# UBC-AWP/vision-sam3-yolo-lameless

Hardware: AMD Instinct MI355X
Metric: frames/sec (whole node) for YOLO+SAM3+DINOv3 feature extraction, 1080p clips (higher is better)
Workload: dtype f16; 1 GPU; BASELINE cfg#5, dense schedule: fused per-frame path on a synthetic 5 s @ 30 fps 1080p clip (150 unique BGR frames resident in HBM): YOLOv8-l detect (letterbox 384x640, NMS, scale_boxes; f16 plan) -> SAM (Hiera-B+ image encoder + FPN at 1024x1024, box-prompted mask decoder, 1080p mask + statistics + contour features) + DINOv3 ViT-L/16 embed (224x224) on EVERY frame; per-frame records packed, gathe; parallelism=one clip per GPU, 1 GPU(s), one gather per step, streams=7

## Files before the change

include/lmx.h:

```cpp
#ifndef LMX_H
#define LMX_H
#include <stdint.h>
#ifdef __cplusplus
extern "C" {
#endif

#define LMX_VERSION 100

#define LMX_OK 0
#define LMX_EINVAL (-1)
#define LMX_EHIP (-2)

typedef void* lmx_stream_t;

int lmx_version(void);
const char* lmx_last_error(void);
int lmx_device_count(void);

enum { LMX_F16 = 0, LMX_F32 = 1 };
enum { LMX_ACT_NONE = 0, LMX_ACT_SILU = 1, LMX_ACT_GELU = 2 , LMX_ACT_RELU = 3 };

typedef struct {
  const void* A;
  const void* W;
  const float* bias;
  const float* scale;
  const void* res;
  void* C;
  int64_t lda, ldc, ldr;
  int32_t M, N, K;
  int32_t act;
  int32_t out_dtype;
  int32_t a_mode;
  int32_t H, W_, Cin, conv_stride, Ho, Wo;
  int32_t res_rows;
  int32_t a_rep;
  int32_t split_k;
  int64_t split_stride;
} lmx_gemm_desc;
int lmx_k_gemm(const lmx_gemm_desc* d, lmx_stream_t stream);
void lmx_dbg_set_gemm2_variant(int v);

int lmx_k_layernorm(const void* x, int in_dtype, int64_t ldx, const float* gamma, const float* beta,
                    void* y, int out_dtype, int64_t ldy, int rows, int D, float eps, int act, lmx_stream_t stream);

int lmx_k_hiera_attn8(const void* h, float* x, int64_t ldx, const float* gamma, const float* beta, float eps, const void* wqkv_p,
                      const float* bqkv_p, const void* wo_p, const float* bo, int n_img, int Gh, int Gw, int D, int heads, float scale,
                      lmx_stream_t stream);

int lmx_k_hiera_attn4(const void* h, float* x, int64_t ldx, const void* w_img, const float* bias, int n_img, int Gh, int Gw, int D,
                      int heads, float scale, lmx_stream_t stream);

int lmx_k_hiera_attn_pool(const void* h, float* out, const void* w_img, const float* bias, int n_img, int Gh, int Gw, int Din, int Dout,
                          int heads, float scale, lmx_stream_t stream);

int lmx_k_ln_mlp(float* x, int64_t ldx, const float* gamma, const float* beta, const void* w1, const float* b1,
                 const void* w2, const float* b2, int64_t rows, int D, float eps, void* workspace, void* x16,
                 const float* gamma_next, const float* beta_next, void* h_next, lmx_stream_t stream);
int lmx_k_ln_mlp_img(float* x, int64_t ldx, const void* w_img, const float* bias, int64_t rows, int D, float eps, void* x16, void* h_next,
                     lmx_stream_t stream);

typedef struct {
  const void* Q; const void* K; const void* V; void* O;
  int64_t ldq, ldk, ldv, ldo;
  int32_t B, H, Tq, Tk, hd;
  float scale;
  int32_t mode;
  int32_t Gh, Gw, ws, q_stride;
  const void* pad_k; const void* pad_v;
  const void* rel; int32_t rel_S;
} lmx_attn_desc;
int lmx_k_attention(const lmx_attn_desc* d, lmx_stream_t stream);
int lmx_k_relpos_tables(const lmx_attn_desc* d, const float* rel_pos_h, const float* rel_pos_w, int S, void* out,
                        lmx_stream_t stream);

int lmx_k_rope(void* x, int64_t ld, int B, int T, int H, int hd, int n_prefix, const float* cos_t,
               const float* sin_t, lmx_stream_t stream);

int lmx_k_pil_resize_h(const uint8_t* src, uint8_t* dst, int n, int sh, int sw, int dw, const int32_t* bounds,
                       const int32_t* kk, int ksize, int swap_rb, lmx_stream_t stream);
int lmx_k_pil_resize_v(const uint8_t* src, uint8_t* dst, int n, int sh, int dh, int w, const int32_t* bounds,
                       const int32_t* kk, int ksize, lmx_stream_t stream);

int lmx_k_patchify_norm(const uint8_t* img, void* out, int n, int ih, int iw, int top, int left, int gh, int gw,
                        int P, int64_t ldo, const float* lut, lmx_stream_t stream);

int lmx_k_assemble_tokens(const void* patch_f16, const float* prefix, const float* pos, float* out, int B, int np,
                          int n_prefix, int D, lmx_stream_t stream);

int lmx_k_token_mean(const void* x, int in_dtype, float* out, int B, int T, int D, lmx_stream_t stream);

int64_t lmx_nms_workspace_bytes(int n, int A);
int lmx_k_nms(const float* pred, int n, int A, int nc, float conf, double iou, int max_det, float max_wh,
              float* boxes, float* scores, int32_t* cls, int32_t* src, int32_t* counts, void* workspace,
              lmx_stream_t stream);

int lmx_k_letterbox(const uint8_t* src, uint8_t* dst, int n, int sh, int sw, int rh, int rw, int top, int left,
                    int oh, int ow, const int32_t* xofs, const int16_t* ialpha, const int32_t* yofs,
                    const int16_t* ibeta, int swap_rb, lmx_stream_t stream);
int lmx_k_stem_conv(const uint8_t* img, const float* w, const float* bias, void* out, int n, int H, int W, int Cout,
                    lmx_stream_t stream);
int lmx_k_maxpool5(const void* src, int64_t lds, void* dst, int64_t ldd, int n, int H, int W, int C,
                   lmx_stream_t stream);
int lmx_k_upsample2(const void* src, int64_t lds, void* dst, int64_t ldd, int n, int H, int W, int C,
                    lmx_stream_t stream);
int lmx_k_detect_decode(const float* head, int64_t ldh, float* pred, int n, int H, int W, int nc, float stride,
                        int a_off, int A, lmx_stream_t stream);
int lmx_k_scale_boxes(float* boxes, int total, float padx, float pady, float gain, float w, float h,
                      lmx_stream_t stream);

int lmx_k_split3(const float* x, int64_t ldx, int act, const void* res3, int64_t ldr, void* out3, int64_t ldo, int64_t rows,
                 int N, int g, int nsum, int64_t sum_stride, lmx_stream_t stream);
int lmx_k_maxpool5_x3(const void* src3, int64_t lds, void* dst3, int64_t ldd, int n, int H, int W, int C, lmx_stream_t stream);
int lmx_k_stem_conv_x3(const uint8_t* img, const float* w, const float* bias, void* out3, int n, int H, int W, int Cout,
                       lmx_stream_t stream);
int lmx_k_attention_f32(const float* q, int64_t ldq, const float* k, int64_t ldk, const float* v, int64_t ldv, float* o,
                        int64_t ldo, int B, int H, int Tq, int Tk, int hd, float scale, lmx_stream_t stream);
int lmx_k_hyper_mask_f32(const float* up, const float* hyper, float* logits, int n, int G, int C, int act, lmx_stream_t stream);

int lmx_k_pose_gather(const float* raw0, const float* raw1, const float* raw2, int64_t ldk, const int32_t* hw,
                      const float* strides, const int32_t* src, const int32_t* counts, int n, int max_det, int K, int ndim,
                      float padx, float pady, float gain, float w, float h, float* out, lmx_stream_t stream);

int lmx_k_im2col_u8(const uint8_t* img, const float* lut, void* out, int n, int rh, int rw, int IH, int IW, int KH,
                    int KW, int stride, int pad, int64_t ldo, lmx_stream_t stream);
int lmx_k_maxpool2(const void* src, int64_t lds, void* dst, int64_t ldd, int dtype, int n, int H, int W, int C,
                   lmx_stream_t stream);
int lmx_k_cast_f32_f16(const float* src, int64_t lds, void* dst, int64_t ldd, int64_t rows, int cols,
                       lmx_stream_t stream);

int lmx_k_add_bcast(const void* a, int a_dtype, int64_t lda, const float* b, int64_t ldb, int b_rows, void* out,
                    int out_dtype, int64_t ldo, int64_t rows, int D, lmx_stream_t stream);
int lmx_k_prompt_box(const float* boxes, int64_t ldb, float* sparse, int n, double sx, double sy, float S,
                     const float* gauss, const float* corner, int F, lmx_stream_t stream);
int lmx_k_hyper_mask(const void* up, const float* hyper, float* logits, int n, int G, int C, lmx_stream_t stream);
int lmx_k_mask_post(const float* logits, int n, int L, int T, int nh, int nw, int h, int w, uint8_t* mask,
                    int64_t* stats, float* workspace, lmx_stream_t stream);
int lmx_k_prompt_points(const float* points, const int32_t* labels, int Np, const float* boxes, int64_t ldb, float* sparse, int n,
                        double sx, double sy, float S, const float* gauss, const float* point_embed, const float* not_a_point,
                        const float* corner, int F, lmx_stream_t stream);
#define LMX_MASK_EMBED_PARAMS 4684
int lmx_k_mask_embed(const float* mask_input, const void* emb, int emb_dtype, int64_t lde, const float* params, float* keys,
                     int64_t ldk, int n, int G, lmx_stream_t stream);
int lmx_k_hyper_mask_multi(const void* up, const float* hyper, float* logits, int n, int M, int G, int C, lmx_stream_t stream);
int lmx_k_hyper_mask_multi_f32(const float* up, const float* hyper, float* logits, int n, int M, int G, int C, int act,
                               lmx_stream_t stream);
int lmx_k_mask_logits(const float* logits, int n, int L, int T, int nh, int nw, int h, int w, float* out, lmx_stream_t stream);
int lmx_k_pack_bits(const uint8_t* src, int64_t rows, int w, uint8_t* dst, lmx_stream_t stream);

int64_t lmx_contour_workspace_bytes(int n, int h, int w);
int lmx_k_contour_features(const uint8_t* mask, int n, int h, int w, int64_t* out, void* workspace, lmx_stream_t stream);

int lmx_h_mask_features(const uint8_t* mask_host, int h, int w, double* out_host);

int lmx_h_iou_matrix(const double* a, int n, const double* b, int m, double* out);
int lmx_h_assign(const double* cost, int n, int m, int* row_to_col, int* col_to_row);

#ifdef __cplusplus
}
#endif
#endif
```

vision-sam3-yolo-lameless_amd/csrc/common.h:

```cpp
#pragma once
#include <hip/hip_runtime.h>
#include <stdint.h>
#include <stdio.h>
#include <stdarg.h>
#include "../../include/lmx.h"

typedef _Float16 half_t;
typedef _Float16 half2_t __attribute__((ext_vector_type(2)));
typedef _Float16 half4_t __attribute__((ext_vector_type(4)));
typedef _Float16 half8_t __attribute__((ext_vector_type(8)));
typedef float f32x4 __attribute__((ext_vector_type(4)));
typedef float f32x16 __attribute__((ext_vector_type(16)));
typedef unsigned int u32x4 __attribute__((ext_vector_type(4)));
typedef unsigned int u32x2 __attribute__((ext_vector_type(2)));

void lmx_set_error(const char* fmt, ...);

#define LMX_REQUIRE(cond, ...)            \
  do {                                    \
    if (!(cond)) {                        \
      lmx_set_error(__VA_ARGS__);         \
      return LMX_EINVAL;                  \
    }                                     \
  } while (0)

#define LMX_HIP(call)                                                                   \
  do {                                                                                  \
    hipError_t e_ = (call);                                                             \
    if (e_ != hipSuccess) {                                                             \
      lmx_set_error("%s failed: %s (%s:%d)", #call, hipGetErrorString(e_), __FILE__, __LINE__); \
      return LMX_EHIP;                                                                  \
    }                                                                                   \
  } while (0)

static inline int lmx_launch_check(const char* what) {
  hipError_t e = hipGetLastError();
  if (e != hipSuccess) {
    lmx_set_error("launch of %s failed: %s", what, hipGetErrorString(e));
    return LMX_EHIP;
  }
  return LMX_OK;
}

typedef float f32x2 __attribute__((ext_vector_type(2)));

__device__ __forceinline__ f32x2 gelu_pk(f32x2 v) {
  f32x2 vc;
  vc[0] = __builtin_amdgcn_fmed3f(v[0], -4.5f, 4.5f);
  vc[1] = __builtin_amdgcn_fmed3f(v[1], -4.5f, 4.5f);
  const f32x2 u = vc * vc;
  f32x2 p = {-1.223331157e-12f, -1.223331157e-12f};
  p = p * u + 1.524351007e-10f;
  p = p * u + -8.481037793e-09f;
  p = p * u + 2.798429583e-07f;
  p = p * u + -6.151207192e-06f;
  p = p * u + 9.615961466e-05f;
  p = p * u + -1.114801972e-03f;
  p = p * u + 9.814679350e-03f;
  p = p * u + -6.632144717e-02f;
  p = p * u + 3.988863025e-01f;
  const f32x2 g = vc * p;
  return v * g + 0.5f * v;
}
__device__ __forceinline__ float gelu_1(float v) {
  const f32x2 r = gelu_pk(f32x2{v, v});
  return r[0];
}

__device__ __forceinline__ float lmx_act(float v, int act) {
  if (act == LMX_ACT_SILU) return v * __builtin_amdgcn_rcpf(1.0f + __builtin_amdgcn_exp2f(-v * 1.44269504088896340736f));
  if (act == LMX_ACT_GELU) return gelu_1(v);
  if (act == LMX_ACT_RELU) return fmaxf(v, 0.0f);
  return v;
}

typedef __attribute__((address_space(3))) void* lds_ptr_t;

__device__ __forceinline__ void lds_dma16(__amdgpu_buffer_rsrc_t rs, char* dst_lds, unsigned voffset, int soffset) {
  __builtin_amdgcn_raw_ptr_buffer_load_lds(rs, (lds_ptr_t)dst_lds, 16, voffset, soffset, 0, 0);
}

#define LMX_WAIT_CASE(n) \
  if constexpr (N == n) asm volatile("s_waitcnt vmcnt(" #n ")" ::: "memory")
template <int N>
__device__ __forceinline__ void wait_vmcnt() {
  static_assert(N == 0 || N == 1 || N == 2 || N == 3 || N == 4 || N == 6 || N == 8 || N == 9 || N == 12 || N == 16 || N == 18 || N == 24 ||
                    N == 32,
                "add the literal for this count");
  LMX_WAIT_CASE(0);
  LMX_WAIT_CASE(1);
  LMX_WAIT_CASE(2);
  LMX_WAIT_CASE(3);
  LMX_WAIT_CASE(4);
  LMX_WAIT_CASE(6);
  LMX_WAIT_CASE(8);
  LMX_WAIT_CASE(9);
  LMX_WAIT_CASE(12);
  LMX_WAIT_CASE(16);
  LMX_WAIT_CASE(18);
  LMX_WAIT_CASE(24);
  LMX_WAIT_CASE(32);
}
#undef LMX_WAIT_CASE
template <int PT>
__device__ __forceinline__ void wait_tiles(int y) {
  if (y >= 4)
    wait_vmcnt<4 * PT>();
  else if (y == 3)
    wait_vmcnt<3 * PT>();
  else if (y == 2)
    wait_vmcnt<2 * PT>();
  else if (y == 1)
    wait_vmcnt<PT>();
  else
    wait_vmcnt<0>();
}

static inline bool aligned16(const void* p) { return (((uintptr_t)p) & 15) == 0; }

__device__ __forceinline__ float wave_sum(float v) {
#pragma unroll
  for (int o = 32; o > 0; o >>= 1) v += __shfl_xor(v, o, 64);
  return v;
}
__device__ __forceinline__ float wave_max(float v) {
#pragma unroll
  for (int o = 32; o > 0; o >>= 1) v = fmaxf(v, __shfl_xor(v, o, 64));
  return v;
}

__device__ __forceinline__ float act_exact(float v, int act) {
  if (act == LMX_ACT_SILU) return v / (1.0f + expf(-v));
  if (act == LMX_ACT_RELU) return fmaxf(v, 0.0f);
  if (act == LMX_ACT_GELU) return 0.5f * v * (1.0f + erff(v * 0.70710678118654752440f));
  return v;
}

__device__ __forceinline__ void bil_idx(float scale, int dst, int in_size, int& i0, int& i1, float& l1) {
  float src = scale * ((float)dst + 0.5f) - 0.5f;
  src = src < 0.f ? 0.f : src;
  i0 = (int)src;
  i1 = i0 + (i0 < in_size - 1 ? 1 : 0);
  l1 = src - (float)i0;
}

__device__ __forceinline__ float sample_mid(const float* __restrict__ lg, int L, int T, float sLT, int Y, int X) {
  int y0, y1, x0, x1;
  float ly, lx;
  bil_idx(sLT, Y, L, y0, y1, ly);
  bil_idx(sLT, X, L, x0, x1, lx);
  const float t0 = (1.f - lx) * lg[y0 * L + x0] + lx * lg[y0 * L + x1];
  const float t1 = (1.f - lx) * lg[y1 * L + x0] + lx * lg[y1 * L + x1];
  return (1.f - ly) * t0 + ly * t1;
}
```

vision-sam3-yolo-lameless_amd/csrc/gemm.hip:

```cpp
#include "common.h"
#include <stdlib.h>

namespace {

constexpr int BK = 64;

template <int BM, int BN, int AMODE, int OUT_DT>
__global__ __launch_bounds__(256, 2) void gemm_kernel(const lmx_gemm_desc p) {
  extern __shared__ __attribute__((aligned(16))) char smem[];
  half_t* As = reinterpret_cast<half_t*>(smem);
  half_t* Ws = As + 2 * BM * BK;
  constexpr int FM = BM / 32;
  constexpr int FN = BN / 32;
  constexpr int AI = BM / 32;
  constexpr int WI = BN / 32;

  const int tid = threadIdx.x;
  const int lane = tid & 63;
  const int wave = tid >> 6;
  const int wm = wave & 1, wn = wave >> 1;

  const int nwg = gridDim.x;
  const int bid = blockIdx.x;
  const int q = nwg >> 3, r = nwg & 7, xcd = bid & 7;
  const int swz = (xcd < r ? xcd * (q + 1) : r * (q + 1) + (xcd - r) * q) + (bid >> 3);
  const int NT = (p.N + BN - 1) / BN;
  const int mt = swz / NT, nt = swz - mt * NT;
  const int m0 = mt * BM, n0 = nt * BN;

  const int c = tid & 7;
  const int r0 = tid >> 3;

  const half_t* A = reinterpret_cast<const half_t*>(p.A);
  const half_t* W = reinterpret_cast<const half_t*>(p.W);

  int64_t a_off[AI];
  int a_iy[AI], a_ix[AI];
  bool a_ok[AI];
#pragma unroll
  for (int i = 0; i < AI; ++i) {
    const int m = m0 + r0 + 32 * i;
    a_ok[i] = m < p.M;
    if (AMODE == 0) {
      a_off[i] = (int64_t)m * p.lda;
      a_iy[i] = a_ix[i] = 0;
    } else {
      const int hw = p.Ho * p.Wo;
      const int img = m / hw;
      const int rem = m - img * hw;
      const int oy = rem / p.Wo;
      const int ox = rem - oy * p.Wo;
      a_off[i] = (int64_t)img * p.H * p.W_ * p.lda;
      a_iy[i] = oy * p.conv_stride - 1;
      a_ix[i] = ox * p.conv_stride - 1;
    }
  }
  int64_t w_off[WI];
  bool w_ok[WI];
#pragma unroll
  for (int i = 0; i < WI; ++i) {
    const int n = n0 + r0 + 32 * i;
    w_ok[i] = n < p.N;
    w_off[i] = (int64_t)n * p.K;
  }

  half8_t a_st[AI], w_st[WI];
  const half8_t zero8 = {0, 0, 0, 0, 0, 0, 0, 0};

  auto load_tile = [&](int kt) {
    const int k = kt * BK + c * 8;
    const bool k_ok = k < p.K;
    if (AMODE == 0) {
#pragma unroll
      for (int i = 0; i < AI; ++i)
        a_st[i] = (a_ok[i] && k_ok) ? *reinterpret_cast<const half8_t*>(A + a_off[i] + k) : zero8;
    } else {
      const int tap = k / p.Cin;
      const int ci = k - tap * p.Cin;
      const int ky = tap / 3;
      const int kx = tap - 3 * ky;
#pragma unroll
      for (int i = 0; i < AI; ++i) {
        const int iy = a_iy[i] + ky, ix = a_ix[i] + kx;
        const bool ok = a_ok[i] && k_ok && (unsigned)iy < (unsigned)p.H && (unsigned)ix < (unsigned)p.W_;
        a_st[i] = ok ? *reinterpret_cast<const half8_t*>(A + a_off[i] + ((int64_t)iy * p.W_ + ix) * p.lda + ci)
                     : zero8;
      }
    }
#pragma unroll
    for (int i = 0; i < WI; ++i)
      w_st[i] = (w_ok[i] && k_ok) ? *reinterpret_cast<const half8_t*>(W + w_off[i] + k) : zero8;
  };
  auto store_tile = [&](int buf) {
    half_t* as = As + buf * BM * BK;
    half_t* ws = Ws + buf * BN * BK;
#pragma unroll
    for (int i = 0; i < AI; ++i) {
      const int row = r0 + 32 * i;
      *reinterpret_cast<half8_t*>(as + row * BK + ((c ^ (row & 7)) << 3)) = a_st[i];
    }
#pragma unroll
    for (int i = 0; i < WI; ++i) {
      const int row = r0 + 32 * i;
      *reinterpret_cast<half8_t*>(ws + row * BK + ((c ^ (row & 7)) << 3)) = w_st[i];
    }
  };

  f32x4 acc[FM][FN];
#pragma unroll
  for (int i = 0; i < FM; ++i)
#pragma unroll
    for (int j = 0; j < FN; ++j) acc[i][j] = f32x4{0.f, 0.f, 0.f, 0.f};

  const int nk = (p.K + BK - 1) / BK;
  load_tile(0);
  store_tile(0);
  __syncthreads();

  const int frow = lane & 15;
  const int fq = lane >> 4;
  for (int kt = 0; kt < nk; ++kt) {
    const int buf = kt & 1;
    if (kt + 1 < nk) load_tile(kt + 1);
    const half_t* as = As + buf * BM * BK + (wm * (BM / 2) + frow) * BK;
    const half_t* ws = Ws + buf * BN * BK + (wn * (BN / 2) + frow) * BK;
#pragma unroll
    for (int ks = 0; ks < 2; ++ks) {
      const int coff = (((ks << 2) + fq) ^ (frow & 7)) << 3;
      half8_t af[FM], wf[FN];
#pragma unroll
      for (int i = 0; i < FM; ++i) af[i] = *reinterpret_cast<const half8_t*>(as + i * 16 * BK + coff);
#pragma unroll
      for (int j = 0; j < FN; ++j) wf[j] = *reinterpret_cast<const half8_t*>(ws + j * 16 * BK + coff);
#pragma unroll
      for (int i = 0; i < FM; ++i)
#pragma unroll
        for (int j = 0; j < FN; ++j)
          acc[i][j] = __builtin_amdgcn_mfma_f32_16x16x32_f16(wf[j], af[i], acc[i][j], 0, 0, 0);
    }
    if (kt + 1 < nk) store_tile(buf ^ 1);
    __syncthreads();
  }

#pragma unroll
  for (int i = 0; i < FM; ++i) {
    const int m = m0 + wm * (BM / 2) + i * 16 + frow;
    if (m >= p.M) continue;
    const int mr = p.res_rows > 0 ? m % p.res_rows : m;
#pragma unroll
    for (int j = 0; j < FN; ++j) {
      const int n = n0 + wn * (BN / 2) + j * 16 + fq * 4;
      if (n >= p.N) continue;
      f32x4 v = acc[i][j];
      if (p.bias) {
        const f32x4 b = *reinterpret_cast<const f32x4*>(p.bias + n);
        v += b;
      }
      if (p.act != LMX_ACT_NONE) {
#pragma unroll
        for (int e = 0; e < 4; ++e) v[e] = lmx_act(v[e], p.act);
      }
      if (p.scale) {
        const f32x4 s = *reinterpret_cast<const f32x4*>(p.scale + n);
#pragma unroll
        for (int e = 0; e < 4; ++e) v[e] = __fmul_rn(v[e], s[e]);
      }
      if (OUT_DT == LMX_F32) {
        float* C = reinterpret_cast<float*>(p.C);
        if (p.res) {
          const f32x4 rr = *reinterpret_cast<const f32x4*>(reinterpret_cast<const float*>(p.res) + (int64_t)mr * p.ldr + n);
#pragma unroll
          for (int e = 0; e < 4; ++e) v[e] = __fadd_rn(v[e], rr[e]);
        }
        *reinterpret_cast<f32x4*>(C + (int64_t)m * p.ldc + n) = v;
      } else {
        half_t* C = reinterpret_cast<half_t*>(p.C);
        if (p.res) {
          const half4_t rr =
              *reinterpret_cast<const half4_t*>(reinterpret_cast<const half_t*>(p.res) + (int64_t)mr * p.ldr + n);
#pragma unroll
          for (int e = 0; e < 4; ++e) v[e] = __fadd_rn((float)(half_t)v[e], (float)rr[e]);
        }
        half4_t o;
#pragma unroll
        for (int e = 0; e < 4; ++e) o[e] = (half_t)v[e];
        *reinterpret_cast<half4_t*>(C + (int64_t)m * p.ldc + n) = o;
      }
    }
  }
}

template <int BM, int BN, int AMODE, int OUT_DT>
int launch(const lmx_gemm_desc& d, hipStream_t st) {
  const int MT = (d.M + BM - 1) / BM, NT = (d.N + BN - 1) / BN;
  const size_t smem = (size_t)2 * (BM + BN) * BK * sizeof(half_t);
  static bool attr_set = false;
  if (!attr_set) {
    LMX_HIP(hipFuncSetAttribute(reinterpret_cast<const void*>(&gemm_kernel<BM, BN, AMODE, OUT_DT>),
                                hipFuncAttributeMaxDynamicSharedMemorySize, (int)smem));
    attr_set = true;
  }
  hipLaunchKernelGGL((gemm_kernel<BM, BN, AMODE, OUT_DT>), dim3(MT * NT), dim3(256), smem, st, d);
  return lmx_launch_check("gemm_kernel");
}

template <int AMODE, int OUT_DT>
int dispatch_tile(const lmx_gemm_desc& d, hipStream_t st) {
  if (d.N <= 64 || (d.N < 128 && d.N % 128 != 0)) return launch<128, 64, AMODE, OUT_DT>(d, st);
  return launch<128, 128, AMODE, OUT_DT>(d, st);
}

}

int lmx_gemm2_launch(const lmx_gemm_desc& d, hipStream_t st);

static bool force_v1() {
  static int v = -1;
  if (v < 0) {
    const char* e = getenv("LMX_GEMM_V1");
    v = (e && e[0] == '1') ? 1 : 0;
  }
  return v == 1;
}

extern "C" int lmx_k_gemm(const lmx_gemm_desc* dp, lmx_stream_t stream) {
  LMX_REQUIRE(dp != nullptr, "lmx_k_gemm: null descriptor");
  const lmx_gemm_desc& d = *dp;
  LMX_REQUIRE(d.A && d.W && d.C, "lmx_k_gemm: null A/W/C");
  LMX_REQUIRE(d.M > 0 && d.N > 0 && d.K > 0, "lmx_k_gemm: empty problem M=%d N=%d K=%d", d.M, d.N, d.K);
  LMX_REQUIRE(d.K % 8 == 0, "lmx_k_gemm: K=%d must be a multiple of 8", d.K);
  LMX_REQUIRE(d.N % 4 == 0, "lmx_k_gemm: N=%d must be a multiple of 4", d.N);
  LMX_REQUIRE(d.lda % 8 == 0, "lmx_k_gemm: lda=%lld must be a multiple of 8", (long long)d.lda);
  LMX_REQUIRE(d.ldc % 4 == 0 && d.ldc >= d.N, "lmx_k_gemm: bad ldc=%lld", (long long)d.ldc);
  LMX_REQUIRE(aligned16(d.A) && aligned16(d.W), "lmx_k_gemm: A/W must be 16-byte aligned");
  LMX_REQUIRE((((uintptr_t)d.C) & 7) == 0, "lmx_k_gemm: C must be 8-byte aligned");
  LMX_REQUIRE(d.out_dtype == LMX_F16 || d.out_dtype == LMX_F32, "lmx_k_gemm: bad out_dtype %d", d.out_dtype);
  LMX_REQUIRE(d.out_dtype == LMX_F16 || aligned16(d.C), "lmx_k_gemm: f32 C must be 16-byte aligned");
  LMX_REQUIRE(d.act >= LMX_ACT_NONE && d.act <= LMX_ACT_RELU, "lmx_k_gemm: bad act %d", d.act);
  if (d.bias) LMX_REQUIRE(aligned16(d.bias), "lmx_k_gemm: bias must be 16-byte aligned");
  if (d.scale) LMX_REQUIRE(aligned16(d.scale), "lmx_k_gemm: scale must be 16-byte aligned");
  if (d.res) LMX_REQUIRE(d.ldr % 4 == 0 && d.ldr >= d.N, "lmx_k_gemm: bad ldr=%lld", (long long)d.ldr);
  LMX_REQUIRE(d.res_rows >= 0, "lmx_k_gemm: res_rows");
  if (d.a_mode == 0) {
    LMX_REQUIRE(d.a_rep > 1 || d.lda >= d.K, "lmx_k_gemm: lda=%lld < K=%d", (long long)d.lda, d.K);
  } else if (d.a_mode == 1) {
    LMX_REQUIRE(d.Cin > 0 && d.Cin % 8 == 0, "lmx_k_gemm: conv Cin=%d must be a multiple of 8", d.Cin);
    LMX_REQUIRE(d.K == 9 * d.Cin, "lmx_k_gemm: conv K=%d != 9*Cin=%d", d.K, 9 * d.Cin);
    LMX_REQUIRE(d.conv_stride == 1 || d.conv_stride == 2, "lmx_k_gemm: conv stride %d", d.conv_stride);
    LMX_REQUIRE(d.H > 0 && d.W_ > 0, "lmx_k_gemm: conv H/W");
    LMX_REQUIRE(d.Ho == (d.H + 2 - 3) / d.conv_stride + 1 && d.Wo == (d.W_ + 2 - 3) / d.conv_stride + 1,
                "lmx_k_gemm: conv Ho/Wo (%d,%d) inconsistent with H/W (%d,%d) stride %d", d.Ho, d.Wo, d.H, d.W_,
                d.conv_stride);
    LMX_REQUIRE(d.M % (d.Ho * d.Wo) == 0, "lmx_k_gemm: conv M=%d not a multiple of Ho*Wo", d.M);
    LMX_REQUIRE(d.lda >= d.Cin, "lmx_k_gemm: conv pixel stride lda=%lld < Cin=%d", (long long)d.lda, d.Cin);
  } else if (d.a_mode == 2) {
    LMX_REQUIRE(d.lda >= d.K, "lmx_k_gemm: lda=%lld < K=%d", (long long)d.lda, d.K);
    LMX_REQUIRE(d.H > 0 && d.W_ > 0 && d.H % 2 == 0 && d.W_ % 2 == 0 && d.M % (d.H * d.W_) == 0,
                "lmx_k_gemm: pooled rows need an even H x W token grid that divides M (H=%d W=%d M=%d)", d.H, d.W_, d.M);
    LMX_REQUIRE(!d.res && !d.scale && d.act == LMX_ACT_NONE, "lmx_k_gemm: pooled rows: no residual / scale / activation");
    LMX_REQUIRE(((int64_t)d.M * d.lda + d.K) * 2 < 0x7fffffffll, "lmx_k_gemm: pooled rows: A must be smaller than 2 GB");
    LMX_REQUIRE(d.M >= 512 && d.N >= 96 && d.N % 8 == 0 && d.ldc % 8 == 0 && aligned16(d.C),
                "lmx_k_gemm: pooled rows are built for the LDS-DMA kernel (M >= 512, N >= 96, N %% 8 == 0): use GEMM + maxpool2 for M=%d N=%d", d.M, d.N);
  } else {
    LMX_REQUIRE(false, "lmx_k_gemm: bad a_mode %d", d.a_mode);
  }
  LMX_REQUIRE(d.a_rep >= 0 && d.a_rep <= 3, "lmx_k_gemm: a_rep=%d (0..3)", d.a_rep);
  LMX_REQUIRE(d.split_k >= 0 && d.split_k <= 64, "lmx_k_gemm: split_k=%d (0..64)", d.split_k);
  if (d.split_k > 1) {
    LMX_REQUIRE(d.out_dtype == LMX_F32 && d.act == LMX_ACT_NONE && d.a_mode != 2 && d.a_rep <= 1, "lmx_k_gemm: split_k needs f32 output, no activation, a_mode 0 or 1");
    LMX_REQUIRE(d.split_stride >= (int64_t)(d.M - 1) * d.ldc + d.N && d.split_stride % 4 == 0, "lmx_k_gemm: split_stride=%lld", (long long)d.split_stride);
    LMX_REQUIRE((d.K + 63) / 64 >= d.split_k, "lmx_k_gemm: split_k=%d exceeds the k-tiles of K=%d", d.split_k, d.K);
    const bool conv_ok2 = d.a_mode == 1 && d.Cin % 32 == 0 && d.H < 32768 && d.W_ < 32768;
    LMX_REQUIRE((d.a_mode == 0 || conv_ok2) && d.N >= 64 && d.N % 8 == 0 && d.ldc % 8 == 0 && (!d.res || d.ldr % 8 == 0) &&
                    aligned16(d.C) && (!d.res || aligned16(d.res)),
                "lmx_k_gemm: split_k is built into the LDS-DMA kernel only (N >= 64, N %% 8 == 0; conv: Cin %% 32 == 0); M=%d N=%d", d.M, d.N);
    return lmx_gemm2_launch(d, reinterpret_cast<hipStream_t>(stream));
  }
  if (d.a_rep > 1) {
    LMX_REQUIRE(d.a_mode == 0 && d.K % d.a_rep == 0 && (d.K / d.a_rep) % 64 == 0, "lmx_k_gemm: a_rep=%d needs a_mode 0 and K / a_rep a multiple of 64 (K=%d)", d.a_rep, d.K);
    LMX_REQUIRE(d.lda >= d.K / d.a_rep, "lmx_k_gemm: lda=%lld < K / a_rep", (long long)d.lda);
    LMX_REQUIRE(d.M >= 512 && d.N >= 96 && d.N % 8 == 0 && d.ldc % 8 == 0 && (!d.res || d.ldr % 8 == 0) && aligned16(d.C) && (!d.res || aligned16(d.res)),
                "lmx_k_gemm: a_rep is built into the LDS-DMA kernel only (M >= 512, N >= 96, N %% 8 == 0); M=%d N=%d", d.M, d.N);
    return lmx_gemm2_launch(d, reinterpret_cast<hipStream_t>(stream));
  }
  hipStream_t st = reinterpret_cast<hipStream_t>(stream);
  const bool conv_ok = d.a_mode == 1 && d.Cin % 32 == 0 && d.H < 32768 && d.W_ < 32768;
  if (d.a_mode == 2) return lmx_gemm2_launch(d, st);
  static int n64 = -1;
  if (n64 < 0) n64 = (getenv("LMX_GEMM_N64") && getenv("LMX_GEMM_N64")[0] == '0') ? 0 : 1;
  const int n_min = (conv_ok && n64 && d.M >= 65536) ? 64 : 96;
  if ((d.a_mode == 0 || conv_ok) && d.M >= 512 && d.N >= n_min && d.N % 8 == 0 && d.ldc % 8 == 0 && (!d.res || d.ldr % 8 == 0) &&
      aligned16(d.C) && (!d.res || aligned16(d.res)) && !force_v1())
    return lmx_gemm2_launch(d, st);
  if (d.a_mode == 0) {
    return d.out_dtype == LMX_F16 ? dispatch_tile<0, LMX_F16>(d, st) : dispatch_tile<0, LMX_F32>(d, st);
  }
  return d.out_dtype == LMX_F16 ? dispatch_tile<1, LMX_F16>(d, st) : dispatch_tile<1, LMX_F32>(d, st);
}
```

vision-sam3-yolo-lameless_amd/csrc/gemm2.hip:

```cpp
#include "common.h"
#include <stdlib.h>
#include <type_traits>

#ifdef LMX_DBG_TIMELINE
__device__ unsigned long long lmx_tl[8 * 16384];
extern "C" int lmx_dbg_get_timeline(void* host, int64_t bytes) { return (int)hipMemcpyFromSymbol(host, HIP_SYMBOL(lmx_tl), bytes); }
#define TL(i, v) if (threadIdx.x == 0 && swz < 16384) lmx_tl[swz * 8 + (i)] = (v)
#else
#define TL(i, v)
#endif
namespace lmx_gemm2 {

__device__ __forceinline__ float act_apply(float v, int act) { return lmx_act(v, act); }

constexpr int smem_bytes(int BM, int BN, int BK, int NSTAGE) { return NSTAGE * (BM + BN) * BK * 2 + 2 * BN * 4; }
constexpr int waves_per_simd(int BM, int BN, int BK, int NSTAGE) {
  const int smem = smem_bytes(BM, BN, BK, NSTAGE), nwave = (BM / 64) * (BN / 64);
  const int wps = (smem <= 80 * 1024 ? 2 : 1) * nwave / 4;
  return wps < 1 ? 1 : wps;
}
template <int OUT_DT, int BM, int BN, int BK, int NSTAGE, int AMODE, int STAG>
__global__ __launch_bounds__(waves_per_simd(BM, BN, BK, NSTAGE) * 256) void gemm2_kernel(const lmx_gemm_desc p, const int ntiles, const int nt_ok) {
  constexpr int NWAVE = (BM / 64) * (BN / 64);
  constexpr int STAGE_BYTES = (BM + BN) * BK * 2;
  constexpr int A_INSTR = BM * BK * 2 / 1024 / NWAVE;
  constexpr int W_INSTR = BN * BK * 2 / 1024 / NWAVE;
  constexpr int ROWS_PER_INSTR = 1024 / (BK * 2);
  constexpr int CHUNKS = BK / 8;
  constexpr int LA = NSTAGE - 1;
  extern __shared__ __attribute__((aligned(16))) char smem[];
  const int tid = threadIdx.x;
  const int lane = tid & 63;
  const int wave = __builtin_amdgcn_readfirstlane(tid >> 6);
  const int wm = wave % (BM / 64), wn = wave / (BM / 64);

  const int bid = blockIdx.x, xcd = bid & 7;
  const int q = ntiles >> 3, r = ntiles & 7;
  const int base = xcd < r ? xcd * (q + 1) : r * (q + 1) + (xcd - r) * q;
  const int cnt = q + (xcd < r ? 1 : 0);
  const int stride = ((int)gridDim.x + 7 - xcd) >> 3;
  const int NT = (p.N + BN - 1) / BN;
  for (int li = bid >> 3; li < cnt; li += stride) {
  const int swz = base + li;
  const int S_ = p.split_k > 1 ? p.split_k : 1;
  const int tile_ = swz / S_, sp_ = swz - tile_ * S_;
  const int mt = tile_ / NT, nt = tile_ - mt * NT;
  const int m0 = mt * BM, n0 = nt * BN;
  TL(0, (unsigned long long)__builtin_amdgcn_s_getreg((31 << 11) | 4));
  TL(1, (unsigned long long)__builtin_amdgcn_s_getreg((31 << 11) | 20));
  TL(2, wall_clock64());
  TL(5, (unsigned long long)bid);

  const int hw_out = (AMODE == 1) ? p.Ho * p.Wo : 1;
  const int img0 = (AMODE == 1) ? m0 / hw_out : 0;
  const char* Ab = reinterpret_cast<const char*>(p.A) +
                   ((AMODE == 1) ? (int64_t)img0 * p.H * p.W_ * p.lda * 2 : (AMODE == 2 ? (int64_t)0 : (int64_t)m0 * p.lda * 2));
  const char* Wb = reinterpret_cast<const char*>(p.W) + (int64_t)n0 * p.K * 2;
  const int Ka = (AMODE == 0 && p.a_rep > 1) ? p.K / p.a_rep : p.K;
  int64_t a_bytes = (AMODE == 1) ? ((int64_t)(p.M / hw_out - img0) * p.H * p.W_ - 1) * p.lda * 2 + (int64_t)p.Cin * 2
                                 : ((int64_t)(p.M - (AMODE == 2 ? 0 : m0) - 1) * p.lda + Ka) * 2;
  int64_t w_bytes = (int64_t)(p.N - n0) * p.K * 2;
  if (a_bytes > 0x7FFFFFF0ll) a_bytes = 0x7FFFFFF0ll;
  if (w_bytes > 0x7FFFFFF0ll) w_bytes = 0x7FFFFFF0ll;
  const __amdgpu_buffer_rsrc_t a_rs = __builtin_amdgcn_make_buffer_rsrc(const_cast<char*>(Ab), 0, (int)a_bytes, 0x00020000);
  const __amdgpu_buffer_rsrc_t w_rs = __builtin_amdgcn_make_buffer_rsrc(const_cast<char*>(Wb), 0, (int)w_bytes, 0x00020000);

  const int lrow = lane / CHUNKS;
  const int lsw = (BK == 64) ? (lrow & 7) : ((-(lrow >> 2)) & 3);
  const int lchunk = (lane % CHUNKS) ^ lsw;
  unsigned a_off[A_INSTR], w_off[W_INSTR];
  int a_yx[A_INSTR];
#pragma unroll
  for (int j = 0; j < A_INSTR; ++j) {
    const int row = (wave * A_INSTR + j) * ROWS_PER_INSTR + lrow;
    if (AMODE == 0) {
      a_off[j] = (unsigned)(row * (int)p.lda * 2 + lchunk * 16);
      a_yx[j] = 0;
    } else if (AMODE == 2) {
      const int m = m0 + row, g = m >> 2, sub = m & 3;
      const int Wq = p.W_ >> 1, gpi = (p.H >> 1) * Wq;
      const int img = g / gpi, rem = g - img * gpi;
      const int gy = rem / Wq, gx = rem - gy * Wq;
      const int tok = (img * p.H + 2 * gy + (sub >> 1)) * p.W_ + 2 * gx + (sub & 1);
      a_off[j] = m < p.M ? (unsigned)(tok * (int)p.lda * 2 + lchunk * 16) : 0x80000000u;
      a_yx[j] = 0;
    } else {
      const int m = m0 + row;
      const int img = m / hw_out, rem = m - img * hw_out;
      const int oy = rem / p.Wo, ox = rem - oy * p.Wo;
      const int iy0 = oy * p.conv_stride - 1, ix0 = ox * p.conv_stride - 1;
      a_off[j] = (unsigned)((((img - img0) * p.H + iy0) * p.W_ + ix0) * (int)p.lda * 2 + lchunk * 16);
      a_yx[j] = (m < p.M) ? ((iy0 << 16) | (ix0 & 0xffff)) : 0x80008000;
    }
  }
#pragma unroll
  for (int j = 0; j < W_INSTR; ++j)
    w_off[j] = (unsigned)(((wave * W_INSTR + j) * ROWS_PER_INSTR + lrow) * p.K * 2 + lchunk * 16);
  const unsigned OOB = 0x80000000u;
  const int nk = (p.K + BK - 1) / BK;
  const int nk64 = (p.K + 63) / 64;
  const int kt0 = (int)((int64_t)sp_ * nk64 / S_) * (64 / BK);
  const int kte = sp_ + 1 == S_ ? nk : (int)((int64_t)(sp_ + 1) * nk64 / S_) * (64 / BK);
  const int nloc = kte - kt0;
  const int nkA = (AMODE == 0 && p.a_rep > 1) ? nk / p.a_rep : nk;
  const bool k_tail_lane = (nk - 1) * BK + lchunk * 8 >= p.K;

  auto issue = [&](int kt, int slot) {
    char* st = smem + slot * STAGE_BYTES;
    const bool kill = (kt == nk - 1) && k_tail_lane;
    const int soff = kt * (BK * 2);
    if (AMODE != 1) {
      const int kta = kt - (kt >= nkA ? nkA : 0) - (kt >= 2 * nkA ? nkA : 0);
      const int soff_a = (AMODE == 0) ? kta * (BK * 2) : soff;
#pragma unroll
      for (int j = 0; j < A_INSTR; ++j) {
        char* dst = st + (wave * A_INSTR + j) * 1024;
        lds_dma16(a_rs, dst, kill ? OOB : a_off[j], soff_a);
      }
    } else {
      const int k0 = kt * BK;
      const int tap = k0 / p.Cin, ci0 = k0 - tap * p.Cin;
      const int ky = tap / 3, kx = tap - 3 * ky;
      const int tap_off = ((ky * p.W_ + kx) * (int)p.lda + ci0) * 2;
#pragma unroll
      for (int j = 0; j < A_INSTR; ++j) {
        char* dst = st + (wave * A_INSTR + j) * 1024;
        const int iy = (a_yx[j] >> 16) + ky, ix = (int)(short)(a_yx[j] & 0xffff) + kx;
        const bool ok = (unsigned)iy < (unsigned)p.H && (unsigned)ix < (unsigned)p.W_;
        lds_dma16(a_rs, dst, ok ? a_off[j] + (unsigned)tap_off : OOB, 0);
      }
    }
#pragma unroll
    for (int j = 0; j < W_INSTR; ++j) {
      char* dst = st + BM * BK * 2 + (wave * W_INSTR + j) * 1024;
      lds_dma16(w_rs, dst, kill ? OOB : w_off[j], soff);
    }
  };

  f32x4 acc[4][4];
#pragma unroll
  for (int i = 0; i < 4; ++i)
#pragma unroll
    for (int j = 0; j < 4; ++j) acc[i][j] = f32x4{0.f, 0.f, 0.f, 0.f};

  float* bl = reinterpret_cast<float*>(smem + NSTAGE * STAGE_BYTES);
  float bias_v = 0.f, scale_v = 1.f;
  if (AMODE != 1 && tid < BN && n0 + tid < p.N) {
    if (p.bias && sp_ == 0) bias_v = p.bias[n0 + tid];
    if (p.scale) scale_v = p.scale[n0 + tid];
  }

#pragma unroll
  for (int t = 0; t < LA; ++t)
    if (t < nloc) issue(kt0 + t, t);

  const int frow = lane & 15, fq = lane >> 4;
  const int fsw = (BK == 64) ? (frow & 7) : ((-(frow >> 2)) & 3);
  constexpr int PT = A_INSTR + W_INSTR;
  if constexpr (STAG == 0) {
  for (int kt = 0; kt < nloc; ++kt) {
    const int left = nloc - 1 - kt;
    wait_tiles<PT>(left < LA - 1 ? left : LA - 1);
    __builtin_amdgcn_s_barrier();
#ifdef LMX_DBG_TIMELINE
    if (kt == 0) { TL(6, wall_clock64()); }
    if (kt == 1) { TL(7, wall_clock64()); }
#endif
    if (kt + LA < nloc) issue(kt0 + kt + LA, (kt + LA) % NSTAGE);
    const char* st = smem + (kt % NSTAGE) * STAGE_BYTES;
    const half_t* as = reinterpret_cast<const half_t*>(st) + (wm * 64 + frow) * BK;
    const half_t* ws = reinterpret_cast<const half_t*>(st + BM * BK * 2) + (wn * 64 + frow) * BK;
#ifdef LMX_DBG_NOMFMA
    if (p.M < 0)
#endif
#pragma unroll
    for (int ks = 0; ks < BK / 32; ++ks) {
      const int coff = (((ks << 2) + fq) ^ fsw) << 3;
      half8_t af[4], wf[4];
#pragma unroll
      for (int j = 0; j < 4; ++j) wf[j] = *reinterpret_cast<const half8_t*>(ws + j * 16 * BK + coff);
#pragma unroll
      for (int i = 0; i < 4; ++i) af[i] = *reinterpret_cast<const half8_t*>(as + i * 16 * BK + coff);
      __builtin_amdgcn_s_setprio(1);
#pragma unroll
      for (int i = 0; i < 4; ++i)
#pragma unroll
        for (int j = 0; j < 4; ++j)
          acc[i][j] = __builtin_amdgcn_mfma_f32_16x16x32_f16(wf[j], af[i], acc[i][j], 0, 0, 0);
      __builtin_amdgcn_s_setprio(0);
    }
  }
  } else {
  const int grp = wave >= NWAVE / 2 ? 1 : 0;
  {
    const int y = nloc - 1 < LA - 1 ? nloc - 1 : LA - 1;
    wait_tiles<PT>(y);
  }
  __builtin_amdgcn_s_barrier();
  if (grp) __builtin_amdgcn_s_barrier();
  for (int kt = 0; kt < nloc; ++kt) {
    const char* st = smem + (kt % NSTAGE) * STAGE_BYTES;
    const half_t* as = reinterpret_cast<const half_t*>(st) + (wm * 64 + frow) * BK;
    const half_t* ws = reinterpret_cast<const half_t*>(st + BM * BK * 2) + (wn * 64 + frow) * BK;
    half8_t af[BK / 32][4], wf[BK / 32][4];
#pragma unroll
    for (int ks = 0; ks < BK / 32; ++ks) {
      const int coff = (((ks << 2) + fq) ^ fsw) << 3;
#pragma unroll
      for (int j = 0; j < 4; ++j) wf[ks][j] = *reinterpret_cast<const half8_t*>(ws + j * 16 * BK + coff);
#pragma unroll
      for (int i = 0; i < 4; ++i) af[ks][i] = *reinterpret_cast<const half8_t*>(as + i * 16 * BK + coff);
    }
    if (kt + 1 < nloc) {
      const int rest = nloc - 2 - kt;
      wait_tiles<PT>(rest < LA - 2 ? (rest < 0 ? 0 : rest) : (LA - 2 < 0 ? 0 : LA - 2));
    }
    if (kt + LA < nloc) issue(kt0 + kt + LA, (kt + LA) % NSTAGE);
    asm volatile("s_waitcnt lgkmcnt(0)" ::: "memory");
    __builtin_amdgcn_s_barrier();
    __builtin_amdgcn_s_setprio(1);
#pragma unroll
    for (int ks = 0; ks < BK / 32; ++ks)
#pragma unroll
      for (int i = 0; i < 4; ++i)
#pragma unroll
        for (int j = 0; j < 4; ++j)
          acc[i][j] = __builtin_amdgcn_mfma_f32_16x16x32_f16(wf[ks][j], af[ks][i], acc[i][j], 0, 0, 0);
    __builtin_amdgcn_s_setprio(0);
    __builtin_amdgcn_s_barrier();
  }
  if (!grp) __builtin_amdgcn_s_barrier();
  }

  if (AMODE == 1 && tid < BN && n0 + tid < p.N) {
    if (p.bias && sp_ == 0) bias_v = p.bias[n0 + tid];
    if (p.scale) scale_v = p.scale[n0 + tid];
  }
  if (tid < BN) {
    bl[tid] = bias_v;
    bl[BN + tid] = scale_v;
  }
  asm volatile("s_waitcnt lgkmcnt(0)" ::: "memory");
  __builtin_amdgcn_s_barrier();
  TL(3, wall_clock64());
#ifdef LMX_DBG_NOEPI
  if (p.M > 0 && acc[0][0][0] != 12345.f) continue;
#endif
  const bool nt_out = nt_ok && OUT_DT == LMX_F16 && ((p.ldc * 2) & 127) == 0 && (int64_t)p.M * p.N >= (16ll << 20);
  char* my = smem + wave * 4608;
  auto epilogue = [&](auto act_c, auto scale_c) {
    constexpr int ACT = decltype(act_c)::value;
    constexpr bool SCALE = decltype(scale_c)::value;
    const float* blj = bl + wn * 64 + fq * 4;
    auto finish = [&](f32x4 v, int j) -> f32x4 {
      v += *reinterpret_cast<const f32x4*>(blj + j * 16);
      if constexpr (ACT == LMX_ACT_GELU) {
        const f32x2 g0 = gelu_pk(f32x2{v[0], v[1]}), g1 = gelu_pk(f32x2{v[2], v[3]});
        v = f32x4{g0[0], g0[1], g1[0], g1[1]};
      } else if constexpr (ACT != LMX_ACT_NONE) {
#pragma unroll
        for (int e = 0; e < 4; ++e) v[e] = act_apply(v[e], ACT);
      }
      if constexpr (SCALE) v *= *reinterpret_cast<const f32x4*>(blj + BN + j * 16);
      return v;
    };
    if constexpr (OUT_DT == LMX_F16 && AMODE == 2) {
#pragma unroll
      for (int pass = 0; pass < 4; ++pass)
#pragma unroll
        for (int j = 0; j < 4; ++j) {
          f32x4 v = finish(acc[pass][j], j);
#pragma unroll
          for (int e = 0; e < 4; ++e) {
            v[e] = fmaxf(v[e], __shfl_xor(v[e], 1, 64));
            v[e] = fmaxf(v[e], __shfl_xor(v[e], 2, 64));
          }
          const int m = m0 + wm * 64 + pass * 16 + frow;
          const int n = n0 + wn * 64 + j * 16 + fq * 4;
          if ((frow & 3) == 0 && m < p.M && n < p.N)
            *reinterpret_cast<half4_t*>(reinterpret_cast<half_t*>(p.C) + (int64_t)(m >> 2) * p.ldc + n) =
                half4_t{(half_t)v[0], (half_t)v[1], (half_t)v[2], (half_t)v[3]};
          __builtin_amdgcn_sched_barrier(0);
        }
    } else if constexpr (OUT_DT == LMX_F16) {
      half_t* t16 = reinterpret_cast<half_t*>(my);
      constexpr int RS = 72;
#pragma unroll
      for (int pass = 0; pass < 2; ++pass) {
#pragma unroll
        for (int ii = 0; ii < 2; ++ii)
#pragma unroll
          for (int j = 0; j < 4; ++j) {
            const f32x4 v = finish(acc[pass * 2 + ii][j], j);
            const half4_t o = {(half_t)v[0], (half_t)v[1], (half_t)v[2], (half_t)v[3]};
            *reinterpret_cast<half4_t*>(t16 + (ii * 16 + frow) * RS + j * 16 + fq * 4) = o;
          }
#pragma unroll
        for (int it = 0; it < 4; ++it) {
          const int row = it * 8 + (lane >> 3), c8 = lane & 7;
          half8_t o = *reinterpret_cast<const half8_t*>(t16 + row * RS + c8 * 8);
          const int m = m0 + wm * 64 + pass * 32 + row;
          const int n = n0 + wn * 64 + c8 * 8;
          if (m < p.M && n < p.N) {
            if (p.res) {
              const int mr = p.res_rows > 0 ? m % p.res_rows : m;
              const half8_t rr = *reinterpret_cast<const half8_t*>(reinterpret_cast<const half_t*>(p.res) + (int64_t)mr * p.ldr + n);
#pragma unroll
              for (int e = 0; e < 8; ++e) o[e] = (half_t)((float)o[e] + (float)rr[e]);
            }
            half8_t* dst = reinterpret_cast<half8_t*>(reinterpret_cast<half_t*>(p.C) + (int64_t)m * p.ldc + n);
            if (nt_out)
              asm volatile("global_store_dwordx4 %0, %1, off nt" ::"v"(dst), "v"(o) : "memory");
            else
              *dst = o;
          }
        }
      }
    } else if constexpr (AMODE == 2) {
#pragma unroll
      for (int pass = 0; pass < 4; ++pass)
#pragma unroll
        for (int j = 0; j < 4; ++j) {
          f32x4 v = finish(acc[pass][j], j);
#pragma unroll
          for (int e = 0; e < 4; ++e) {
            v[e] = fmaxf(v[e], __shfl_xor(v[e], 1, 64));
            v[e] = fmaxf(v[e], __shfl_xor(v[e], 2, 64));
          }
          const int m = m0 + wm * 64 + pass * 16 + frow;
          const int n = n0 + wn * 64 + j * 16 + fq * 4;
          if ((frow & 3) == 0 && m < p.M && n < p.N) *reinterpret_cast<f32x4*>(reinterpret_cast<float*>(p.C) + (int64_t)(m >> 2) * p.ldc + n) = v;
          __builtin_amdgcn_sched_barrier(0);
        }
    } else {
      float* t32 = reinterpret_cast<float*>(my);
      constexpr int RS = 68;
      const int lrow = lane >> 4, c16 = lane & 15;
      const int n = n0 + wn * 64 + c16 * 4;
      const bool has_res = p.res != nullptr && sp_ == 0;
      float* Cs = reinterpret_cast<float*>(p.C) + (int64_t)sp_ * p.split_stride;
      f32x4 rr[4];
      auto load_res = [&](int pass) {
        f32x4* d = rr;
#pragma unroll
        for (int it = 0; it < 4; ++it) {
          const int m = m0 + wm * 64 + pass * 16 + it * 4 + lrow;
          d[it] = f32x4{0.f, 0.f, 0.f, 0.f};
          if (has_res && m < p.M && n < p.N) {
            const int mr = p.res_rows > 0 ? m % p.res_rows : m;
            d[it] = *reinterpret_cast<const f32x4*>(reinterpret_cast<const float*>(p.res) + (int64_t)mr * p.ldr + n);
          }
        }
      };
#pragma unroll
      for (int pass = 0; pass < 4; ++pass) {
        load_res(pass);
#pragma unroll
        for (int j = 0; j < 4; ++j) *reinterpret_cast<f32x4*>(t32 + frow * RS + j * 16 + fq * 4) = finish(acc[pass][j], j);
#pragma unroll
        for (int it = 0; it < 4; ++it) {
          const int row = it * 4 + lrow;
          f32x4 o = *reinterpret_cast<const f32x4*>(t32 + row * RS + c16 * 4);
          const int m = m0 + wm * 64 + pass * 16 + row;
          if (m < p.M && n < p.N) {
            if (has_res) o += rr[it];
            *reinterpret_cast<f32x4*>(Cs + (int64_t)m * p.ldc + n) = o;
          }
        }
      }
    }
  };
  {
    using T = std::true_type;
    using F = std::false_type;
    const int act = p.act;
    if (p.scale) {
      if (act == LMX_ACT_NONE) epilogue(std::integral_constant<int, LMX_ACT_NONE>{}, T{});
      else if (act == LMX_ACT_SILU) epilogue(std::integral_constant<int, LMX_ACT_SILU>{}, T{});
      else if (act == LMX_ACT_GELU) epilogue(std::integral_constant<int, LMX_ACT_GELU>{}, T{});
      else epilogue(std::integral_constant<int, LMX_ACT_RELU>{}, T{});
    } else {
      if (act == LMX_ACT_NONE) epilogue(std::integral_constant<int, LMX_ACT_NONE>{}, F{});
      else if (act == LMX_ACT_SILU) epilogue(std::integral_constant<int, LMX_ACT_SILU>{}, F{});
      else if (act == LMX_ACT_GELU) epilogue(std::integral_constant<int, LMX_ACT_GELU>{}, F{});
      else epilogue(std::integral_constant<int, LMX_ACT_RELU>{}, F{});
    }
  }
  __builtin_amdgcn_s_barrier();
  TL(4, wall_clock64());
  }
}

template <int BM, int BN, int BK, int NSTAGE, int AMODE, int STAG = 0>
int launch2(const lmx_gemm_desc& d, hipStream_t st) {
  const int MT = (d.M + BM - 1) / BM, NT = (d.N + BN - 1) / BN;
  const size_t smem = smem_bytes(BM, BN, BK, NSTAGE);
  static bool attr_set = false;
  if (!attr_set) {
    LMX_HIP(hipFuncSetAttribute(reinterpret_cast<const void*>(&gemm2_kernel<LMX_F16, BM, BN, BK, NSTAGE, AMODE, STAG>),
                                hipFuncAttributeMaxDynamicSharedMemorySize, (int)smem));
    LMX_HIP(hipFuncSetAttribute(reinterpret_cast<const void*>(&gemm2_kernel<LMX_F32, BM, BN, BK, NSTAGE, AMODE, STAG>),
                                hipFuncAttributeMaxDynamicSharedMemorySize, (int)smem));
    attr_set = true;
  }
  const int ntiles = MT * NT * (d.split_k > 1 ? d.split_k : 1);
  int grid = ntiles;
  static int persist = -1, nt_ok = 1;
  if (persist < 0) {
    const char* e = getenv("LMX_GEMM2_PERSIST");
    persist = e ? atoi(e) : 0;
    nt_ok = getenv("LMX_GEMM2_NO_NT") ? 0 : 1;
  }
  if (persist > 0 && grid > 256 * persist) grid = 256 * persist;
  if (d.out_dtype == LMX_F16)
    hipLaunchKernelGGL((gemm2_kernel<LMX_F16, BM, BN, BK, NSTAGE, AMODE, STAG>), dim3(grid), dim3(BM * BN / 64), smem, st, d, ntiles, nt_ok);
  else
    hipLaunchKernelGGL((gemm2_kernel<LMX_F32, BM, BN, BK, NSTAGE, AMODE, STAG>), dim3(grid), dim3(BM * BN / 64), smem, st, d, ntiles, nt_ok);
  return lmx_launch_check("gemm2_kernel");
}

}
using namespace lmx_gemm2;

static int g_variant = -1;
extern "C" void lmx_dbg_set_gemm2_variant(int v) { g_variant = v; }

int lmx_gemm2_launch(const lmx_gemm_desc& d, hipStream_t st) {
  if (g_variant < 0) {
    const char* e = getenv("LMX_GEMM2_VARIANT");
    g_variant = e ? e[0] : 0;
  }
  const int variant = g_variant;
  if (d.a_mode == 2) return launch2<256, 256, 64, 2, 2>(d, st);
  if (d.a_mode == 1) {
    static int conv_small = -1;
    if (conv_small < 0) conv_small = getenv("LMX_GEMM2_CONV_SMALL") ? 1 : 0;
    const int64_t t256 = (int64_t)((d.M + 255) / 256) * ((d.N + 255) / 256);
    const double q256 = (double)t256 / (double)(((t256 + 255) / 256) * 256);
    if (!conv_small && d.N % 256 == 0 && t256 >= 230 && q256 >= 0.75) return launch2<256, 256, 32, 3, 1, 1>(d, st);
    return launch2<256, 128, 32, 3, 1>(d, st);
  }
  switch (variant) {
    case 'A': return launch2<256, 128, 64, 3, 0>(d, st);
    case 'B': return launch2<128, 128, 64, 2, 0>(d, st);
    case 'C': return launch2<256, 128, 32, 3, 0>(d, st);
    case 'D': return launch2<256, 128, 32, 2, 0>(d, st);
    case 'E': return launch2<256, 256, 32, 3, 0>(d, st);
    case 'F': return launch2<256, 256, 32, 4, 0>(d, st);
    case 'H': return launch2<128, 128, 32, 2, 0>(d, st);
    case 'I': return launch2<128, 128, 32, 3, 0>(d, st);
    case 'S': return launch2<256, 128, 32, 6, 0, 1>(d, st);
    case 'T': return launch2<256, 128, 64, 3, 0, 1>(d, st);
    case 'U': return launch2<256, 128, 32, 3, 0, 1>(d, st);
    case 'V': return launch2<256, 128, 32, 4, 0, 1>(d, st);
    case 'W': return launch2<256, 256, 32, 4, 0, 1>(d, st);
    case 'Y': return launch2<256, 256, 32, 3, 0, 1>(d, st);
    case 'Z': return launch2<256, 256, 64, 2, 0>(d, st);
    default: {
      const int64_t nt256 = (d.N + 255) / 256, tiles256 = (int64_t)((d.M + 255) / 256) * nt256;
      const double nfrac = (double)d.N / (double)(nt256 * 256);
      const double q256 = (double)tiles256 / (double)(((tiles256 + 255) / 256) * 256);
      if (d.K >= 448 && tiles256 >= 200 && q256 >= 0.75 && nfrac >= 0.85) {
        return launch2<256, 256, 64, 2, 0>(d, st);
      }
      if (d.K < 448 && d.N >= 224 && d.N <= 1536 && d.N % 256 != 0 && nfrac >= 0.85 && tiles256 >= 200 && q256 >= 0.75)
        return d.K > 128 ? launch2<256, 256, 32, 3, 0>(d, st) : launch2<256, 256, 64, 2, 0>(d, st);
      const int64_t tiles = (int64_t)((d.M + 255) / 256) * ((d.N + 127) / 128);
      return (d.K >= 1792 || tiles <= 256) ? launch2<256, 128, 64, 3, 0, 1>(d, st) : launch2<256, 128, 32, 3, 0>(d, st);
    }
  }
}
```

vision-sam3-yolo-lameless_amd/csrc/norm.hip:

```cpp
#include "common.h"
#include <stdlib.h>

namespace {

template <int LPR>
__device__ __forceinline__ float group_sum(float v) {
#pragma unroll
  for (int o = LPR / 2; o > 0; o >>= 1) v += __shfl_xor(v, o, 64);
  return v;
}

template <int IN_DT, int OUT_DT>
__global__ __launch_bounds__(256) void layernorm_narrow_kernel(const void* __restrict__ xv, int64_t ldx,
                                                               const float* __restrict__ gamma,
                                                               const float* __restrict__ beta, void* __restrict__ yv,
                                                               int64_t ldy, int rows, int D, float eps, int act) {
  const int l = threadIdx.x & 31;
  const int row = blockIdx.x * 8 + (threadIdx.x >> 5);
  const bool live = row < rows;
  const int c = l * 4;
  const bool ok = live && c < D;
  f32x4 v = {0.f, 0.f, 0.f, 0.f};
  if (ok) {
    if (IN_DT == LMX_F32) {
      v = *reinterpret_cast<const f32x4*>(reinterpret_cast<const float*>(xv) + (int64_t)row * ldx + c);
    } else {
      const half4_t hv = *reinterpret_cast<const half4_t*>(reinterpret_cast<const half_t*>(xv) + (int64_t)row * ldx + c);
      v = f32x4{(float)hv[0], (float)hv[1], (float)hv[2], (float)hv[3]};
    }
  }
  const float mean = group_sum<32>((v[0] + v[1]) + (v[2] + v[3])) / (float)D;
  const f32x4 dl = ok ? v - mean : f32x4{0.f, 0.f, 0.f, 0.f};
  const float var = group_sum<32>((dl[0] * dl[0] + dl[1] * dl[1]) + (dl[2] * dl[2] + dl[3] * dl[3])) / (float)D;
  const float rstd = 1.0f / sqrtf(var + eps);
  if (!ok) return;
  f32x4 o = dl * rstd * *reinterpret_cast<const f32x4*>(gamma + c) + *reinterpret_cast<const f32x4*>(beta + c);
  if (act == LMX_ACT_GELU) {
#pragma unroll
    for (int e = 0; e < 4; ++e) o[e] = 0.5f * o[e] * (1.0f + erff(o[e] * 0.70710678118654752440f));
  }
  if (OUT_DT == LMX_F32) {
    *reinterpret_cast<f32x4*>(reinterpret_cast<float*>(yv) + (int64_t)row * ldy + c) = o;
  } else {
    half4_t h = {(half_t)o[0], (half_t)o[1], (half_t)o[2], (half_t)o[3]};
    *reinterpret_cast<half4_t*>(reinterpret_cast<half_t*>(yv) + (int64_t)row * ldy + c) = h;
  }
}

template <int IN_DT, int OUT_DT, int ITERS>
__global__ __launch_bounds__(256) void layernorm_kernel(const void* __restrict__ xv, int64_t ldx,
                                                        const float* __restrict__ gamma,
                                                        const float* __restrict__ beta, void* __restrict__ yv,
                                                        int64_t ldy, int rows, int D, float eps, int act) {
  const int lane = threadIdx.x & 63;
  const int row = blockIdx.x * 4 + (threadIdx.x >> 6);
  if (row >= rows) return;
  f32x4 v[ITERS];
  float s = 0.f;
#pragma unroll
  for (int i = 0; i < ITERS; ++i) {
    const int c = (i * 64 + lane) * 4;
    if (c < D) {
      if (IN_DT == LMX_F32) {
        v[i] = *reinterpret_cast<const f32x4*>(reinterpret_cast<const float*>(xv) + (int64_t)row * ldx + c);
      } else {
        const half4_t hv = *reinterpret_cast<const half4_t*>(reinterpret_cast<const half_t*>(xv) + (int64_t)row * ldx + c);
        v[i] = f32x4{(float)hv[0], (float)hv[1], (float)hv[2], (float)hv[3]};
      }
      s += (v[i][0] + v[i][1]) + (v[i][2] + v[i][3]);
    }
  }
  const float mean = wave_sum(s) / (float)D;
  float q = 0.f;
#pragma unroll
  for (int i = 0; i < ITERS; ++i) {
    const int c = (i * 64 + lane) * 4;
    if (c < D) {
      const f32x4 dlt = v[i] - mean;
      q += (dlt[0] * dlt[0] + dlt[1] * dlt[1]) + (dlt[2] * dlt[2] + dlt[3] * dlt[3]);
    }
  }
  const float rstd = 1.0f / sqrtf(wave_sum(q) / (float)D + eps);
#pragma unroll
  for (int i = 0; i < ITERS; ++i) {
    const int c = (i * 64 + lane) * 4;
    if (c < D) {
      const f32x4 g = *reinterpret_cast<const f32x4*>(gamma + c);
      const f32x4 b = *reinterpret_cast<const f32x4*>(beta + c);
      f32x4 o = (v[i] - mean) * rstd * g + b;
      if (act == LMX_ACT_GELU) {
#pragma unroll
        for (int e = 0; e < 4; ++e) o[e] = 0.5f * o[e] * (1.0f + erff(o[e] * 0.70710678118654752440f));
      }
      if (OUT_DT == LMX_F32) {
        *reinterpret_cast<f32x4*>(reinterpret_cast<float*>(yv) + (int64_t)row * ldy + c) = o;
      } else {
        half4_t h = {(half_t)o[0], (half_t)o[1], (half_t)o[2], (half_t)o[3]};
        *reinterpret_cast<half4_t*>(reinterpret_cast<half_t*>(yv) + (int64_t)row * ldy + c) = h;
      }
    }
  }
}

template <int IN_DT, int OUT_DT, int ITERS>
__global__ __launch_bounds__(256) void layernorm_rows_kernel(const void* __restrict__ xv, int64_t ldx, const float* __restrict__ gamma,
                                                             const float* __restrict__ beta, void* __restrict__ yv, int64_t ldy, int rows,
                                                             int D, float eps) {
  const int lane = threadIdx.x & 63;
  const int nw = gridDim.x * 4;
  int row = blockIdx.x * 4 + (threadIdx.x >> 6);
  if (row >= rows) return;
  f32x4 g[ITERS], b[ITERS];
#pragma unroll
  for (int i = 0; i < ITERS; ++i) {
    const int c = (i * 64 + lane) * 4;
    g[i] = c < D ? *reinterpret_cast<const f32x4*>(gamma + c) : f32x4{0.f, 0.f, 0.f, 0.f};
    b[i] = c < D ? *reinterpret_cast<const f32x4*>(beta + c) : f32x4{0.f, 0.f, 0.f, 0.f};
  }
  auto load = [&](int r, f32x4* v) {
#pragma unroll
    for (int i = 0; i < ITERS; ++i) {
      const int c = (i * 64 + lane) * 4;
      v[i] = f32x4{0.f, 0.f, 0.f, 0.f};
      if (c < D) {
        if (IN_DT == LMX_F32) {
          v[i] = *reinterpret_cast<const f32x4*>(reinterpret_cast<const float*>(xv) + (int64_t)r * ldx + c);
        } else {
          const half4_t hv = *reinterpret_cast<const half4_t*>(reinterpret_cast<const half_t*>(xv) + (int64_t)r * ldx + c);
          v[i] = f32x4{(float)hv[0], (float)hv[1], (float)hv[2], (float)hv[3]};
        }
      }
    }
  };
  f32x4 v[ITERS], vn[ITERS];
  load(row, v);
  while (row < rows) {
    const int nrow = row + nw;
    if (nrow < rows) load(nrow, vn);
    float s = 0.f;
#pragma unroll
    for (int i = 0; i < ITERS; ++i)
      if ((i * 64 + lane) * 4 < D) s += (v[i][0] + v[i][1]) + (v[i][2] + v[i][3]);
    const float mean = wave_sum(s) / (float)D;
    float q = 0.f;
#pragma unroll
    for (int i = 0; i < ITERS; ++i)
      if ((i * 64 + lane) * 4 < D) {
        const f32x4 dlt = v[i] - mean;
        q += (dlt[0] * dlt[0] + dlt[1] * dlt[1]) + (dlt[2] * dlt[2] + dlt[3] * dlt[3]);
      }
    const float rstd = 1.0f / sqrtf(wave_sum(q) / (float)D + eps);
#pragma unroll
    for (int i = 0; i < ITERS; ++i) {
      const int c = (i * 64 + lane) * 4;
      if (c < D) {
        const f32x4 o = (v[i] - mean) * rstd * g[i] + b[i];
        if (OUT_DT == LMX_F32) {
          *reinterpret_cast<f32x4*>(reinterpret_cast<float*>(yv) + (int64_t)row * ldy + c) = o;
        } else {
          const half4_t h = {(half_t)o[0], (half_t)o[1], (half_t)o[2], (half_t)o[3]};
          *reinterpret_cast<half4_t*>(reinterpret_cast<half_t*>(yv) + (int64_t)row * ldy + c) = h;
        }
      }
    }
#pragma unroll
    for (int i = 0; i < ITERS; ++i) v[i] = vn[i];
    row = nrow;
  }
}


__global__ __launch_bounds__(256) void assemble_tokens_kernel(const half_t* __restrict__ patch,
                                                              const float* __restrict__ prefix,
                                                              const float* __restrict__ pos, float* __restrict__ out,
                                                              int B, int np, int n_prefix, int D) {
  const int T = np + n_prefix;
  const int64_t total = (int64_t)B * T * (D / 4);
  for (int64_t i = (int64_t)blockIdx.x * blockDim.x + threadIdx.x; i < total; i += (int64_t)gridDim.x * blockDim.x) {
    const int c = (int)(i % (D / 4)) * 4;
    const int64_t bt = i / (D / 4);
    const int t = (int)(bt % T);
    const int b = (int)(bt / T);
    f32x4 v;
    if (t < n_prefix) {
      v = *reinterpret_cast<const f32x4*>(prefix + (int64_t)t * D + c);
    } else {
      const half4_t h = *reinterpret_cast<const half4_t*>(patch + ((int64_t)b * np + (t - n_prefix)) * D + c);
      v = f32x4{(float)h[0], (float)h[1], (float)h[2], (float)h[3]};
    }
    if (pos) v += *reinterpret_cast<const f32x4*>(pos + (int64_t)t * D + c);
    *reinterpret_cast<f32x4*>(out + bt * D + c) = v;
  }
}

template <int IN_DT>
__global__ __launch_bounds__(64) void token_mean_kernel(const void* __restrict__ xv, float* __restrict__ out, int B,
                                                        int T, int D) {
  const int b = blockIdx.y;
  const int c = (blockIdx.x * 64 + threadIdx.x) * 4;
  if (c >= D) return;
  f32x4 acc = {0.f, 0.f, 0.f, 0.f};
  for (int t = 0; t < T; ++t) {
    const int64_t off = ((int64_t)b * T + t) * D + c;
    if (IN_DT == LMX_F32) {
      acc += *reinterpret_cast<const f32x4*>(reinterpret_cast<const float*>(xv) + off);
    } else {
      const half4_t h = *reinterpret_cast<const half4_t*>(reinterpret_cast<const half_t*>(xv) + off);
      acc += f32x4{(float)h[0], (float)h[1], (float)h[2], (float)h[3]};
    }
  }
  acc /= (float)T;
  *reinterpret_cast<f32x4*>(out + (int64_t)b * D + c) = acc;
}

__global__ __launch_bounds__(256) void rope_kernel(half_t* __restrict__ x, int64_t ld, int B, int T, int H, int hd,
                                                   int n_prefix, const float* __restrict__ cos_t,
                                                   const float* __restrict__ sin_t) {
  const int half = hd / 2;
  const int per_tok = H * (half / 4);
  const int np = T - n_prefix;
  const int64_t total = (int64_t)B * np * per_tok;
  for (int64_t i = (int64_t)blockIdx.x * blockDim.x + threadIdx.x; i < total; i += (int64_t)gridDim.x * blockDim.x) {
    const int w = (int)(i % per_tok);
    const int64_t bp = i / per_tok;
    const int pidx = (int)(bp % np);
    const int b = (int)(bp / np);
    const int h = w / (half / 4);
    const int d = (w - h * (half / 4)) * 4;
    half_t* base = x + ((int64_t)b * T + n_prefix + pidx) * ld + (int64_t)h * hd;
    const half4_t lo = *reinterpret_cast<const half4_t*>(base + d);
    const half4_t hi = *reinterpret_cast<const half4_t*>(base + d + half);
    const f32x4 c_lo = *reinterpret_cast<const f32x4*>(cos_t + (int64_t)pidx * hd + d);
    const f32x4 c_hi = *reinterpret_cast<const f32x4*>(cos_t + (int64_t)pidx * hd + d + half);
    const f32x4 s_lo = *reinterpret_cast<const f32x4*>(sin_t + (int64_t)pidx * hd + d);
    const f32x4 s_hi = *reinterpret_cast<const f32x4*>(sin_t + (int64_t)pidx * hd + d + half);
    half4_t olo, ohi;
#pragma unroll
    for (int e = 0; e < 4; ++e) {
      const float a = (float)lo[e], bb = (float)hi[e];
      olo[e] = (half_t)(a * c_lo[e] - bb * s_lo[e]);
      ohi[e] = (half_t)(bb * c_hi[e] + a * s_hi[e]);
    }
    *reinterpret_cast<half4_t*>(base + d) = olo;
    *reinterpret_cast<half4_t*>(base + d + half) = ohi;
  }
}

inline int grid_for(int64_t total, int block = 256) {
  int64_t g = (total + block - 1) / block;
  if (g > 256 * 8) g = 256 * 8;
  if (g < 1) g = 1;
  return (int)g;
}

}

extern "C" int lmx_k_layernorm(const void* x, int in_dtype, int64_t ldx, const float* gamma, const float* beta,
                               void* y, int out_dtype, int64_t ldy, int rows, int D, float eps, int act, lmx_stream_t stream) {
  LMX_REQUIRE(x && y && gamma && beta, "lmx_k_layernorm: null pointer");
  LMX_REQUIRE(rows > 0 && D > 0 && D % 4 == 0 && D <= 4096, "lmx_k_layernorm: rows=%d D=%d (need D%%4==0, D<=4096)", rows, D);
  LMX_REQUIRE(ldx % 4 == 0 && ldy % 4 == 0 && ldx >= D && ldy >= D, "lmx_k_layernorm: strides");
  LMX_REQUIRE(act == LMX_ACT_NONE || act == LMX_ACT_GELU, "lmx_k_layernorm: act %d", act);
  LMX_REQUIRE(aligned16(gamma) && aligned16(beta), "lmx_k_layernorm: gamma/beta alignment");
  LMX_REQUIRE((((uintptr_t)x) & (in_dtype == LMX_F32 ? 15 : 7)) == 0, "lmx_k_layernorm: x alignment");
  LMX_REQUIRE((((uintptr_t)y) & (out_dtype == LMX_F32 ? 15 : 7)) == 0, "lmx_k_layernorm: y alignment");
  hipStream_t st = reinterpret_cast<hipStream_t>(stream);
  if (D <= 128) {
    dim3 g8((rows + 7) / 8), b256(256);
    if (in_dtype == LMX_F32 && out_dtype == LMX_F16)
      hipLaunchKernelGGL((layernorm_narrow_kernel<LMX_F32, LMX_F16>), g8, b256, 0, st, x, ldx, gamma, beta, y, ldy, rows, D, eps, act);
    else if (in_dtype == LMX_F32 && out_dtype == LMX_F32)
      hipLaunchKernelGGL((layernorm_narrow_kernel<LMX_F32, LMX_F32>), g8, b256, 0, st, x, ldx, gamma, beta, y, ldy, rows, D, eps, act);
    else if (in_dtype == LMX_F16 && out_dtype == LMX_F16)
      hipLaunchKernelGGL((layernorm_narrow_kernel<LMX_F16, LMX_F16>), g8, b256, 0, st, x, ldx, gamma, beta, y, ldy, rows, D, eps, act);
    else if (in_dtype == LMX_F16 && out_dtype == LMX_F32)
      hipLaunchKernelGGL((layernorm_narrow_kernel<LMX_F16, LMX_F32>), g8, b256, 0, st, x, ldx, gamma, beta, y, ldy, rows, D, eps, act);
    else
      LMX_REQUIRE(false, "lmx_k_layernorm: bad dtypes %d -> %d", in_dtype, out_dtype);
    return lmx_launch_check("layernorm_narrow_kernel");
  }
  dim3 grid((rows + 3) / 4), block(256);
  static int one_row = -1;
  if (one_row < 0) one_row = getenv("LMX_LN_ONE_ROW") ? 1 : 0;
  if (!one_row && rows >= 16384 && act == LMX_ACT_NONE && in_dtype == LMX_F32 && out_dtype == LMX_F16 && D <= 1024) {
    dim3 g2(256 * 8);
    if (D <= 512)
      hipLaunchKernelGGL((layernorm_rows_kernel<LMX_F32, LMX_F16, 2>), g2, block, 0, st, x, ldx, gamma, beta, y, ldy, rows, D, eps);
    else
      hipLaunchKernelGGL((layernorm_rows_kernel<LMX_F32, LMX_F16, 4>), g2, block, 0, st, x, ldx, gamma, beta, y, ldy, rows, D, eps);
    return lmx_launch_check("layernorm_rows_kernel");
  }
#define LMX_LN(IN, OUT, IT) \
  hipLaunchKernelGGL((layernorm_kernel<IN, OUT, IT>), grid, block, 0, st, x, ldx, gamma, beta, y, ldy, rows, D, eps, act)
#define LMX_LN_IT(IN, OUT)        \
  do {                            \
    if (D <= 512)                 \
      LMX_LN(IN, OUT, 2);         \
    else if (D <= 1024)           \
      LMX_LN(IN, OUT, 4);         \
    else                          \
      LMX_LN(IN, OUT, 16);        \
  } while (0)
  if (in_dtype == LMX_F32 && out_dtype == LMX_F16)
    LMX_LN_IT(LMX_F32, LMX_F16);
  else if (in_dtype == LMX_F32 && out_dtype == LMX_F32)
    LMX_LN_IT(LMX_F32, LMX_F32);
  else if (in_dtype == LMX_F16 && out_dtype == LMX_F16)
    LMX_LN_IT(LMX_F16, LMX_F16);
  else if (in_dtype == LMX_F16 && out_dtype == LMX_F32)
    LMX_LN_IT(LMX_F16, LMX_F32);
  else
    LMX_REQUIRE(false, "lmx_k_layernorm: bad dtypes %d -> %d", in_dtype, out_dtype);
#undef LMX_LN_IT
#undef LMX_LN
  return lmx_launch_check("layernorm_kernel");
}

extern "C" int lmx_k_assemble_tokens(const void* patch_f16, const float* prefix, const float* pos, float* out, int B,
                                     int np, int n_prefix, int D, lmx_stream_t stream) {
  LMX_REQUIRE(patch_f16 && out && (prefix || n_prefix == 0), "lmx_k_assemble_tokens: null pointer");
  LMX_REQUIRE(B > 0 && np > 0 && n_prefix >= 0 && D > 0 && D % 4 == 0, "lmx_k_assemble_tokens: shape");
  LMX_REQUIRE(aligned16(out) && ((((uintptr_t)patch_f16) & 7) == 0), "lmx_k_assemble_tokens: alignment");
  const int64_t total = (int64_t)B * (np + n_prefix) * (D / 4);
  hipLaunchKernelGGL(assemble_tokens_kernel, dim3(grid_for(total)), dim3(256), 0, reinterpret_cast<hipStream_t>(stream),
                     reinterpret_cast<const half_t*>(patch_f16), prefix, pos, out, B, np, n_prefix, D);
  return lmx_launch_check("assemble_tokens_kernel");
}

extern "C" int lmx_k_token_mean(const void* x, int in_dtype, float* out, int B, int T, int D, lmx_stream_t stream) {
  LMX_REQUIRE(x && out, "lmx_k_token_mean: null pointer");
  LMX_REQUIRE(B > 0 && T > 0 && D > 0 && D % 4 == 0, "lmx_k_token_mean: shape");
  LMX_REQUIRE(aligned16(out), "lmx_k_token_mean: alignment");
  dim3 grid((D / 4 + 63) / 64, B), block(64);
  hipStream_t st = reinterpret_cast<hipStream_t>(stream);
  if (in_dtype == LMX_F32)
    hipLaunchKernelGGL((token_mean_kernel<LMX_F32>), grid, block, 0, st, x, out, B, T, D);
  else if (in_dtype == LMX_F16)
    hipLaunchKernelGGL((token_mean_kernel<LMX_F16>), grid, block, 0, st, x, out, B, T, D);
  else
    LMX_REQUIRE(false, "lmx_k_token_mean: bad dtype %d", in_dtype);
  return lmx_launch_check("token_mean_kernel");
}

extern "C" int lmx_k_rope(void* x, int64_t ld, int B, int T, int H, int hd, int n_prefix, const float* cos_t,
                          const float* sin_t, lmx_stream_t stream) {
  LMX_REQUIRE(x && cos_t && sin_t, "lmx_k_rope: null pointer");
  LMX_REQUIRE(B > 0 && T > n_prefix && n_prefix >= 0 && H > 0 && hd % 8 == 0, "lmx_k_rope: shape");
  LMX_REQUIRE(ld % 4 == 0 && ((((uintptr_t)x) & 7) == 0) && aligned16(cos_t) && aligned16(sin_t), "lmx_k_rope: alignment");
  const int64_t total = (int64_t)B * (T - n_prefix) * H * (hd / 8);
  hipLaunchKernelGGL(rope_kernel, dim3(grid_for(total)), dim3(256), 0, reinterpret_cast<hipStream_t>(stream),
                     reinterpret_cast<half_t*>(x), ld, B, T, H, hd, n_prefix, cos_t, sin_t);
  return lmx_launch_check("rope_kernel");
}
```

vision-sam3-yolo-lameless_amd/lmx/_lib.py:

```python
import ctypes as C
import os

_HERE = os.path.dirname(os.path.abspath(__file__))
LIB_PATH = os.environ.get("LMX_LIB") or os.path.join(_HERE, "liblmx.so")


class LmxError(RuntimeError):
    pass


class GemmDesc(C.Structure):
    _fields_ = [
        ("A", C.c_void_p), ("W", C.c_void_p), ("bias", C.c_void_p), ("scale", C.c_void_p), ("res", C.c_void_p),
        ("C", C.c_void_p),
        ("lda", C.c_int64), ("ldc", C.c_int64), ("ldr", C.c_int64),
        ("M", C.c_int32), ("N", C.c_int32), ("K", C.c_int32),
        ("act", C.c_int32), ("out_dtype", C.c_int32), ("a_mode", C.c_int32),
        ("H", C.c_int32), ("W_", C.c_int32), ("Cin", C.c_int32), ("conv_stride", C.c_int32),
        ("Ho", C.c_int32), ("Wo", C.c_int32), ("res_rows", C.c_int32), ("a_rep", C.c_int32), ("split_k", C.c_int32), ("split_stride", C.c_int64),
    ]


class AttnDesc(C.Structure):
    _fields_ = [
        ("Q", C.c_void_p), ("K", C.c_void_p), ("V", C.c_void_p), ("O", C.c_void_p),
        ("ldq", C.c_int64), ("ldk", C.c_int64), ("ldv", C.c_int64), ("ldo", C.c_int64),
        ("B", C.c_int32), ("H", C.c_int32), ("Tq", C.c_int32), ("Tk", C.c_int32), ("hd", C.c_int32),
        ("scale", C.c_float), ("mode", C.c_int32),
        ("Gh", C.c_int32), ("Gw", C.c_int32), ("ws", C.c_int32), ("q_stride", C.c_int32),
        ("pad_k", C.c_void_p), ("pad_v", C.c_void_p),
        ("rel", C.c_void_p), ("rel_S", C.c_int32),
    ]


_VP, _I, _I64, _F, _D = C.c_void_p, C.c_int, C.c_int64, C.c_float, C.c_double
SIGNATURES = {
    "lmx_version": (_I, []),
    "lmx_last_error": (C.c_char_p, []),
    "lmx_device_count": (_I, []),
    "lmx_k_gemm": (_I, [C.POINTER(GemmDesc), _VP]),
    "lmx_dbg_set_gemm2_variant": (None, [_I]),
    "lmx_k_pose_gather": (_I, [_VP, _VP, _VP, _I64, _VP, _VP, _VP, _VP, _I, _I, _I, _I, _F, _F, _F, _F, _F, _VP, _VP]),
    "lmx_k_pack_bits": (_I, [_VP, _I64, _I, _VP, _VP]),
    "lmx_k_ln_mlp": (_I, [_VP, _I64, _VP, _VP, _VP, _VP, _VP, _VP, _I64, _I, _F, _VP, _VP, _VP, _VP, _VP, _VP]),
    "lmx_k_hiera_attn8": (_I, [_VP, _VP, _I64, _VP, _VP, _F, _VP, _VP, _VP, _VP, _I, _I, _I, _I, _I, _F, _VP]),
    "lmx_k_hiera_attn4": (_I, [_VP, _VP, _I64, _VP, _VP, _I, _I, _I, _I, _I, _F, _VP]),
    "lmx_k_hiera_attn_pool": (_I, [_VP, _VP, _VP, _VP, _I, _I, _I, _I, _I, _I, _F, _VP]),
    "lmx_k_ln_mlp_img": (_I, [_VP, _I64, _VP, _VP, _I64, _I, _F, _VP, _VP, _VP]),
    "lmx_k_layernorm": (_I, [_VP, _I, _I64, _VP, _VP, _VP, _I, _I64, _I, _I, _F, _I, _VP]),
    "lmx_k_attention": (_I, [C.POINTER(AttnDesc), _VP]),
    "lmx_k_relpos_tables": (_I, [C.POINTER(AttnDesc), _VP, _VP, _I, _VP, _VP]),
    "lmx_k_rope": (_I, [_VP, _I64, _I, _I, _I, _I, _I, _VP, _VP, _VP]),
    "lmx_k_pil_resize_h": (_I, [_VP, _VP, _I, _I, _I, _I, _VP, _VP, _I, _I, _VP]),
    "lmx_k_pil_resize_v": (_I, [_VP, _VP, _I, _I, _I, _I, _VP, _VP, _I, _VP]),
    "lmx_k_patchify_norm": (_I, [_VP, _VP, _I, _I, _I, _I, _I, _I, _I, _I, _I64, _VP, _VP]),
    "lmx_k_assemble_tokens": (_I, [_VP, _VP, _VP, _VP, _I, _I, _I, _I, _VP]),
    "lmx_k_token_mean": (_I, [_VP, _I, _VP, _I, _I, _I, _VP]),
    "lmx_nms_workspace_bytes": (_I64, [_I, _I]),
    "lmx_k_nms": (_I, [_VP, _I, _I, _I, _F, _D, _I, _F, _VP, _VP, _VP, _VP, _VP, _VP, _VP]),
    "lmx_k_letterbox": (_I, [_VP, _VP, _I, _I, _I, _I, _I, _I, _I, _I, _I, _VP, _VP, _VP, _VP, _I, _VP]),
    "lmx_k_stem_conv": (_I, [_VP, _VP, _VP, _VP, _I, _I, _I, _I, _VP]),
    "lmx_k_split3": (_I, [_VP, _I64, _I, _VP, _I64, _VP, _I64, _I64, _I, _I, _I, _I64, _VP]),
    "lmx_k_maxpool5_x3": (_I, [_VP, _I64, _VP, _I64, _I, _I, _I, _I, _VP]),
    "lmx_k_stem_conv_x3": (_I, [_VP, _VP, _VP, _VP, _I, _I, _I, _I, _VP]),
    "lmx_k_attention_f32": (_I, [_VP, _I64, _VP, _I64, _VP, _I64, _VP, _I64, _I, _I, _I, _I, _I, _F, _VP]),
    "lmx_k_hyper_mask_f32": (_I, [_VP, _VP, _VP, _I, _I, _I, _I, _VP]),
    "lmx_k_maxpool5": (_I, [_VP, _I64, _VP, _I64, _I, _I, _I, _I, _VP]),
    "lmx_k_upsample2": (_I, [_VP, _I64, _VP, _I64, _I, _I, _I, _I, _VP]),
    "lmx_k_detect_decode": (_I, [_VP, _I64, _VP, _I, _I, _I, _I, _F, _I, _I, _VP]),
    "lmx_k_scale_boxes": (_I, [_VP, _I, _F, _F, _F, _F, _F, _VP]),
    "lmx_k_im2col_u8": (_I, [_VP, _VP, _VP, _I, _I, _I, _I, _I, _I, _I, _I, _I, _I64, _VP]),
    "lmx_k_maxpool2": (_I, [_VP, _I64, _VP, _I64, _I, _I, _I, _I, _I, _VP]),
    "lmx_k_cast_f32_f16": (_I, [_VP, _I64, _VP, _I64, _I64, _I, _VP]),
    "lmx_k_add_bcast": (_I, [_VP, _I, _I64, _VP, _I64, _I, _VP, _I, _I64, _I64, _I, _VP]),
    "lmx_h_mask_features": (_I, [_VP, _I, _I, _VP]),
    "lmx_h_iou_matrix": (_I, [_VP, _I, _VP, _I, _VP]),
    "lmx_h_assign": (_I, [_VP, _I, _I, _VP, _VP]),
    "lmx_contour_workspace_bytes": (_I64, [_I, _I, _I]),
    "lmx_k_contour_features": (_I, [_VP, _I, _I, _I, _VP, _VP, _VP]),
    "lmx_k_prompt_box": (_I, [_VP, _I64, _VP, _I, _D, _D, _F, _VP, _VP, _I, _VP]),
    "lmx_k_hyper_mask": (_I, [_VP, _VP, _VP, _I, _I, _I, _VP]),
    "lmx_k_mask_post": (_I, [_VP, _I, _I, _I, _I, _I, _I, _I, _VP, _VP, _VP, _VP]),
    "lmx_k_prompt_points": (_I, [_VP, _VP, _I, _VP, _I64, _VP, _I, _D, _D, _F, _VP, _VP, _VP, _VP, _I, _VP]),
    "lmx_k_mask_embed": (_I, [_VP, _VP, _I, _I64, _VP, _VP, _I64, _I, _I, _VP]),
    "lmx_k_hyper_mask_multi": (_I, [_VP, _VP, _VP, _I, _I, _I, _I, _VP]),
    "lmx_k_hyper_mask_multi_f32": (_I, [_VP, _VP, _VP, _I, _I, _I, _I, _I, _VP]),
    "lmx_k_mask_logits": (_I, [_VP, _I, _I, _I, _I, _I, _I, _I, _VP, _VP]),
}

_lib = None


def load():
    global _lib
    if _lib is not None:
        return _lib
    if not os.path.exists(LIB_PATH):
        raise ImportError(
            f"{LIB_PATH} not found: build it with `python -c 'import __graft_entry__ as g; g.build()'` "
            "(hipcc --offload-arch=gfx950).  lmx has no CPU fallback.")
    import torch

    lib = C.CDLL(LIB_PATH, mode=os.RTLD_NOW)
    for name, (res, args) in SIGNATURES.items():
        fn = getattr(lib, name)
        fn.restype = res
        fn.argtypes = args
    _lib = lib
    return lib


def check(rc, what):
    if rc != 0:
        msg = load().lmx_last_error().decode("utf-8", "replace")
        raise LmxError(f"{what} failed (rc={rc}): {msg}")
```

vision-sam3-yolo-lameless_amd/lmx/kernels.py:

```python
import ctypes as C
import os
import threading

import torch

from . import _lib
from ._lib import AttnDesc, GemmDesc, LmxError, check

F16, F32 = 0, 1
ACT_NONE, ACT_SILU, ACT_GELU, ACT_RELU = 0, 1, 2, 3
_DT = {torch.float16: F16, torch.float32: F32}


_tls = threading.local()


def _stream(dev):
    _tls.dev = dev
    return C.c_void_p(torch.cuda.current_stream(dev).cuda_stream)


def _ptr(t):
    return C.c_void_p(t.data_ptr()) if t is not None else C.c_void_p(0)


def _dev(*ts):
    dev = None
    for t in ts:
        if t is None:
            continue
        if not t.is_cuda:
            raise LmxError("lmx kernels take device (HBM) tensors only; got a CPU tensor")
        if dev is None:
            dev = t.device
        elif t.device != dev:
            raise LmxError(f"lmx kernels: operands on different devices ({dev} and {t.device})")
    if dev is None:
        raise LmxError("lmx kernels: no device operand")
    return dev


def _rows(t, what):
    if t.dim() != 2 or t.stride(1) != 1:
        raise LmxError(f"{what}: expected a 2-D tensor with contiguous last dim, got shape {tuple(t.shape)} "
                       f"strides {t.stride()}")
    return t.shape[0], t.shape[1], t.stride(0)


def pooled_gemm_ok(M, N):
    return M >= 512 and N >= 96 and N % 8 == 0


def gemm(a, w, bias=None, act=ACT_NONE, scale=None, res=None, out=None, out_dtype=torch.float16, res_rows=0, pool_hw=None, a_rep=1):
    dev = _dev(a, w, bias, scale, res, out)
    M, K, lda = _rows(a, "gemm A")
    N, K2, ldw = _rows(w, "gemm W")
    if K2 != a_rep * K or ldw != K2:
        raise LmxError(f"gemm: W must be contiguous [N,{a_rep}*K]; A K={K}, W shape {tuple(w.shape)}")
    if a.dtype != torch.float16 or w.dtype != torch.float16:
        raise LmxError("gemm: A and W must be float16")
    Mout = M // 4 if pool_hw else M
    if out is None:
        out = torch.empty((Mout, N), dtype=out_dtype, device=a.device)
    Mo, No, ldc = _rows(out, "gemm C")
    if (Mo, No) != (Mout, N):
        raise LmxError(f"gemm: out shape {tuple(out.shape)} != ({Mout},{N})")
    d = GemmDesc()
    d.A, d.W, d.C = a.data_ptr(), w.data_ptr(), out.data_ptr()
    d.bias = bias.data_ptr() if bias is not None else None
    d.scale = scale.data_ptr() if scale is not None else None
    d.lda, d.ldc, d.ldr = lda, ldc, 0
    if bias is not None and (bias.dtype != torch.float32 or bias.numel() != N):
        raise LmxError("gemm: bias must be float32 [N]")
    if scale is not None and (scale.dtype != torch.float32 or scale.numel() != N):
        raise LmxError("gemm: scale must be float32 [N]")
    if res is not None:
        Mr, Nr, ldr = _rows(res, "gemm res")
        if (Mr, Nr) != ((res_rows or M), N) or res.dtype != out.dtype:
            raise LmxError("gemm: residual must match out's shape and dtype")
        d.res, d.ldr = res.data_ptr(), ldr
    d.res_rows = res_rows
    d.M, d.N, d.K = M, N, a_rep * K
    d.act, d.out_dtype, d.a_mode, d.a_rep = act, _DT[out.dtype], 0, a_rep
    if pool_hw:
        d.a_mode, d.H, d.W_ = 2, int(pool_hw[0]), int(pool_hw[1])
    check(_lib.load().lmx_k_gemm(C.byref(d), _stream(dev)), "lmx_k_gemm")
    return out


def im2col_u8(img, lut, IH, IW, KH, KW, stride, pad, ldo):
    dev = _dev(img, lut)
    n, rh, rw, c = img.shape
    if c != 3 or img.dtype != torch.uint8 or not img.is_contiguous():
        raise LmxError("im2col_u8: img must be contiguous uint8 [n,h,w,3]")
    OH, OW = (IH + 2 * pad - KH) // stride + 1, (IW + 2 * pad - KW) // stride + 1
    out = torch.empty((n * OH * OW, ldo), dtype=torch.float16, device=img.device)
    check(_lib.load().lmx_k_im2col_u8(_ptr(img), _ptr(lut), _ptr(out), n, rh, rw, IH, IW, KH, KW, stride, pad, ldo,
                                      _stream(dev)), "lmx_k_im2col_u8")
    return out


def maxpool2(x, out):
    dev = _dev(x, out)
    n, H, W, Cc, ps = _nhwc(x, "maxpool2 x")
    no, Ho, Wo, Co, pso = _nhwc(out, "maxpool2 out")
    if (no, Ho, Wo, Co) != (n, H // 2, W // 2, Cc) or x.dtype != out.dtype:
        raise LmxError("maxpool2: shape/dtype mismatch")
    check(_lib.load().lmx_k_maxpool2(_ptr(x), ps, _ptr(out), pso, _DT[x.dtype], n, H, W, Cc, _stream(dev)), "lmx_k_maxpool2")
    return out


def cast_f16(x, out=None):
    dev = _dev(x, out)
    rows, cols, lds = _rows(x, "cast src")
    if out is None:
        out = torch.empty((rows, cols), dtype=torch.float16, device=x.device)
    check(_lib.load().lmx_k_cast_f32_f16(_ptr(x), lds, _ptr(out), out.stride(0), rows, cols, _stream(dev)),
          "lmx_k_cast_f32_f16")
    return out


def _nhwc(t, what):
    if t.dim() != 4 or t.stride(3) != 1:
        raise LmxError(f"{what}: expected NHWC with contiguous channels, got {tuple(t.shape)} / {t.stride()}")
    n, H, W, Cc = t.shape
    ps = t.stride(2)
    if t.stride(1) != W * ps or (n > 1 and t.stride(0) != H * W * ps):
        raise LmxError(f"{what}: not a channel slice of a dense NHWC buffer: strides {t.stride()}")
    return n, H, W, Cc, ps


def split_k_for(px_per_frame, N, K, cin):
    if N < 64 or N % 8 or cin % 32:
        return 1
    tiles1 = -(-px_per_frame // 256) * -(-N // 256)
    nk = K // 64
    s = min(8, nk // 8, 32 // tiles1)
    return s if s >= 2 else 1


def conv3x3(x, w, bias=None, act=ACT_SILU, stride=1, res=None, out=None, scale=None, out_dtype=torch.float16, split_k=1):
    dev = _dev(x, w, bias, res, out, scale)
    n, H, W, Cin, ps = _nhwc(x, "conv3x3 x")
    Cout = w.shape[0]
    if w.dim() != 2 or w.shape[1] != 9 * Cin or not w.is_contiguous():
        raise LmxError(f"conv3x3: W must be contiguous [Cout, 9*Cin={9 * Cin}], got {tuple(w.shape)}")
    Ho, Wo = (H + 2 - 3) // stride + 1, (W + 2 - 3) // stride + 1
    parts = None
    if split_k > 1:
        if out is not None or res is not None or act != ACT_NONE or out_dtype != torch.float32:
            raise LmxError("conv3x3: split_k needs a fresh f32 output, no residual, no activation")
        parts = torch.empty((split_k, n, Ho, Wo, Cout), dtype=torch.float32, device=x.device)
        out = parts[0]
    if out is None:
        out = torch.empty((n, Ho, Wo, Cout), dtype=out_dtype, device=x.device)
    no, Ho2, Wo2, Co2, pso = _nhwc(out, "conv3x3 out")
    if (no, Ho2, Wo2, Co2) != (n, Ho, Wo, Cout):
        raise LmxError(f"conv3x3: out shape {tuple(out.shape)} != {(n, Ho, Wo, Cout)}")
    d = GemmDesc()
    d.A, d.W, d.C = x.data_ptr(), w.data_ptr(), out.data_ptr()
    d.bias = bias.data_ptr() if bias is not None else None
    if scale is not None and (scale.dtype != torch.float32 or scale.numel() != Cout):
        raise LmxError("conv3x3: scale must be float32 [Cout]")
    d.scale = scale.data_ptr() if scale is not None else None
    d.lda, d.ldc, d.ldr = ps, pso, 0
    if res is not None:
        nr, Hr, Wr, Cr, psr = _nhwc(res, "conv3x3 res")
        if (nr, Hr, Wr, Cr) != (n, Ho, Wo, Cout) or res.dtype != out.dtype:
            raise LmxError("conv3x3: residual must match out")
        d.res, d.ldr = res.data_ptr(), psr
    d.M, d.N, d.K = n * Ho * Wo, Cout, 9 * Cin
    d.act, d.out_dtype, d.a_mode = act, _DT[out.dtype], 1
    d.H, d.W_, d.Cin, d.conv_stride, d.Ho, d.Wo = H, W, Cin, stride, Ho, Wo
    if parts is not None:
        d.split_k, d.split_stride = split_k, parts.stride(0)
    check(_lib.load().lmx_k_gemm(C.byref(d), _stream(dev)), "lmx_k_gemm(conv3x3)")
    return out if parts is None else parts


def conv1x1(x, w, bias=None, act=ACT_SILU, res=None, out=None, out_dtype=torch.float16, scale=None):
    n, H, W, Cin, ps = _nhwc(x, "conv1x1 x")
    a = x.as_strided((n * H * W, Cin), (ps, 1))
    Cout = w.shape[0]
    if out is None:
        out = torch.empty((n, H, W, Cout), dtype=out_dtype, device=x.device)
    no, Ho, Wo, Co, pso = _nhwc(out, "conv1x1 out")
    o2 = out.as_strided((n * H * W, Cout), (pso, 1))
    r2 = None
    if res is not None:
        nr, Hr, Wr, Cr, psr = _nhwc(res, "conv1x1 res")
        r2 = res.as_strided((n * H * W, Cout), (psr, 1))
    gemm(a, w, bias=bias, act=act, res=r2, out=o2, scale=scale)
    return out


def layernorm(x, gamma, beta, eps, out=None, out_dtype=torch.float16, act=ACT_NONE):
    dev = _dev(x, gamma, beta, out)
    rows, D, ldx = _rows(x, "layernorm x")
    if out is None:
        out = torch.empty((rows, D), dtype=out_dtype, device=x.device)
    r2, D2, ldy = _rows(out, "layernorm y")
    if (r2, D2) != (rows, D):
        raise LmxError("layernorm: out shape mismatch")
    check(_lib.load().lmx_k_layernorm(_ptr(x), _DT[x.dtype], ldx, _ptr(gamma), _ptr(beta), _ptr(out), _DT[out.dtype],
                                      ldy, rows, D, float(eps), act, _stream(dev)), "lmx_k_layernorm")
    return out


def pack_bits(mask):
    dev = _dev(mask)
    if mask.dtype not in (torch.uint8, torch.bool) or not mask.is_contiguous():
        raise LmxError("pack_bits: contiguous uint8 / bool tensor expected")
    w = mask.shape[-1]
    rows = mask.numel() // w
    out = torch.empty(tuple(mask.shape[:-1]) + ((w + 7) // 8,), dtype=torch.uint8, device=mask.device)
    check(_lib.load().lmx_k_pack_bits(_ptr(mask), rows, w, _ptr(out), _stream(dev)), "lmx_k_pack_bits")
    return out


FUSED_MLP_WIDTHS = (112, 224)
if os.environ.get("LMX_MLP448"):
    FUSED_MLP_WIDTHS = (112, 224, 448)


def ln_mlp(x, gamma, beta, w1, b1, w2, b2, eps, x16=None, next_ln=None):
    dev = _dev(x, gamma, beta, w1, b1, w2, b2, x16, *(next_ln or ()))
    rows, D, ldx = _rows(x, "ln_mlp x")
    if x.dtype != torch.float32 or w1.dtype != torch.float16 or w2.dtype != torch.float16:
        raise LmxError("ln_mlp: x must be f32 and the weights f16")
    if tuple(w1.shape) != (4 * D, D) or tuple(w2.shape) != (D, 4 * D) or not (w1.is_contiguous() and w2.is_contiguous()):
        raise LmxError("ln_mlp: weight shapes must be [4D, D] and [D, 4D], contiguous")
    if x16 is not None and (x16.dtype != torch.float16 or tuple(x16.shape) != (rows, D) or not x16.is_contiguous()):
        raise LmxError("ln_mlp: x16 must be contiguous float16 [rows, D]")
    gn, bn, hn = next_ln if next_ln else (None, None, None)
    if hn is not None and (hn.dtype != torch.float16 or tuple(hn.shape) != (rows, D) or not hn.is_contiguous() or gn.numel() != D or bn.numel() != D):
        raise LmxError("ln_mlp: next_ln = (gamma [D], beta [D], contiguous float16 [rows, D])")
    ws = torch.empty((rows, D), dtype=torch.float16, device=x.device)
    check(_lib.load().lmx_k_ln_mlp(_ptr(x), ldx, _ptr(gamma), _ptr(beta), _ptr(w1), _ptr(b1), _ptr(w2), _ptr(b2), rows, D,
                                   float(eps), _ptr(ws), _ptr(x16), _ptr(gn), _ptr(bn), _ptr(hn), _stream(dev)), "lmx_k_ln_mlp")
    return x


def hiera_attn8_ok(D, heads, win, Gh, Gw, q_stride):
    return D == 112 and heads == 2 and win == 8 and not q_stride and Gh % 8 == 0 and Gw % 8 == 0 and os.environ.get("LMX_HIERA_ATTN8", "1") != "0"


def hiera_attn8(x, packed, n_img, Gh, Gw, heads, h=None, ln=None):
    wq, bq, wo, bo = packed
    if (h is None) == (ln is None):
        raise LmxError("hiera_attn8: give either h or ln=(gamma, beta, eps)")
    gamma, beta, eps = ln if ln is not None else (None, None, 0.0)
    dev = _dev(x, h, gamma, beta, wq, bq, wo, bo)
    rows, D, ldx = _rows(x, "hiera_attn8 x")
    if x.dtype != torch.float32 or rows != n_img * Gh * Gw:
        raise LmxError("hiera_attn8: x must be float32 [n*Gh*Gw, D]")
    if h is not None and (h.dtype != torch.float16 or tuple(h.shape) != (rows, D) or not h.is_contiguous()):
        raise LmxError("hiera_attn8: h must be contiguous float16 [rows, D]")
    if ln is not None and (gamma.numel() != D or beta.numel() != D or gamma.dtype != torch.float32 or beta.dtype != torch.float32):
        raise LmxError("hiera_attn8: gamma / beta must be float32 [D]")
    if tuple(wq.shape) != (3 * heads * 64, 128) or tuple(wo.shape) != (D, heads * 64) or wq.dtype != torch.float16 or wo.dtype != torch.float16 \
            or not (wq.is_contiguous() and wo.is_contiguous()) or bq.numel() != 3 * heads * 64 or bo.numel() != D:
        raise LmxError("hiera_attn8: packed operands have the wrong shapes (lmx.sam.pack_hiera_attn)")
    check(_lib.load().lmx_k_hiera_attn8(_ptr(h), _ptr(x), ldx, _ptr(gamma), _ptr(beta), float(eps), _ptr(wq), _ptr(bq), _ptr(wo), _ptr(bo),
                                        n_img, Gh, Gw, D, heads, float((D // heads) ** -0.5), _stream(dev)), "lmx_k_hiera_attn8")
    return x


def hiera_attn4_ok(D, heads, win, Gh, Gw, q_stride):
    return D == 224 and heads == 4 and win == 4 and not q_stride and Gh % 4 == 0 and Gw % 4 == 0 and os.environ.get("LMX_HIERA_ATTN4", "1") != "0"


def hiera_attn4(h, x, packed, n_img, Gh, Gw, heads):
    img, bias = packed
    dev = _dev(h, x, img, bias)
    rows, D, ldx = _rows(x, "hiera_attn4 x")
    if x.dtype != torch.float32 or h.dtype != torch.float16 or tuple(h.shape) != (rows, D) or not h.is_contiguous() or rows != n_img * Gh * Gw:
        raise LmxError("hiera_attn4: h must be contiguous float16 [n*Gh*Gw, D] and x float32 rows of the same count")
    if tuple(img.shape) != (4 * heads, 16384) or img.dtype != torch.float16 or not img.is_contiguous() or bias.numel() != heads * 192 + D \
            or bias.dtype != torch.float32:
        raise LmxError("hiera_attn4: packed operands have the wrong shapes (lmx.sam.pack_hiera_attn4)")
    check(_lib.load().lmx_k_hiera_attn4(_ptr(h), _ptr(x), ldx, _ptr(img), _ptr(bias), n_img, Gh, Gw, D, heads, float((D // heads) ** -0.5),
                                        _stream(dev)), "lmx_k_hiera_attn4")
    return x


def hiera_attn_pool_ok(Din, Dout, heads, win, Gh, Gw, q_stride):
    if not q_stride or os.environ.get("LMX_HIERA_ATTN_POOL", "1") == "0":
        return False
    if (Din, Dout, heads, win) == (112, 224, 4, 8):
        return Gh % 8 == 0 and Gw % 8 == 0
    if (Din, Dout, heads, win) == (224, 448, 8, 4):
        return Gh % 4 == 0 and Gw % 4 == 0 and os.environ.get("LMX_HIERA_ATTN_POOL3", "1") != "0"
    return False


def hiera_attn_pool(h, packed, n_img, Gh, Gw, heads, Dout):
    img, bias = packed
    dev = _dev(h, img, bias)
    if h.dtype != torch.float16 or h.dim() != 2 or not h.is_contiguous() or h.shape[0] != n_img * Gh * Gw:
        raise LmxError("hiera_attn_pool: h must be contiguous float16 [n*Gh*Gw, Din]")
    Din = h.shape[1]
    nimg, nb = (47, Dout + heads * 192) if Din > 128 else (14, 2 * Dout + heads * 192)
    if tuple(img.shape) != (nimg, 16384) or img.dtype != torch.float16 or not img.is_contiguous() or bias.numel() != nb or bias.dtype != torch.float32:
        raise LmxError("hiera_attn_pool: packed operands have the wrong shapes (lmx.sam.pack_hiera_attn_pool)")
    out = torch.empty((n_img * (Gh // 2) * (Gw // 2), Dout), dtype=torch.float32, device=h.device)
    check(_lib.load().lmx_k_hiera_attn_pool(_ptr(h), _ptr(out), _ptr(img), _ptr(bias), n_img, Gh, Gw, Din, Dout, heads,
                                            float((Dout // heads) ** -0.5), _stream(dev)), "lmx_k_hiera_attn_pool")
    return out


def ln_mlp_img_ok(D, rows):
    return D in (112, 224) and os.environ.get("LMX_MLP_IMG", "1") != "0"


def ln_mlp_img(x, packed, eps, x16=None, h_next=None):
    img, bias = packed
    dev = _dev(x, img, bias, x16, h_next)
    rows, D, ldx = _rows(x, "ln_mlp_img x")
    nimg = 7 if D == 112 else 28
    if x.dtype != torch.float32 or tuple(img.shape) != (nimg, 16384) or img.dtype != torch.float16 or not img.is_contiguous() \
            or bias.numel() != 9 * D or bias.dtype != torch.float32:
        raise LmxError("ln_mlp_img: x must be f32 [rows, D] and the packed operands those of lmx.sam.pack_ln_mlp")
    for t, name in ((x16, "x16"), (h_next, "h_next")):
        if t is not None and (t.dtype != torch.float16 or tuple(t.shape) != (rows, D) or not t.is_contiguous()):
            raise LmxError(f"ln_mlp_img: {name} must be contiguous float16 [rows, D]")
    check(_lib.load().lmx_k_ln_mlp_img(_ptr(x), ldx, _ptr(img), _ptr(bias), rows, D, float(eps), _ptr(x16), _ptr(h_next), _stream(dev)),
          "lmx_k_ln_mlp_img")
    return x


def _attn_desc(q, k, v, out, B, H, Tq, Tk, hd, scale, window, pad_k, pad_v):
    d = AttnDesc()
    d.Q, d.K, d.V, d.O = q.data_ptr(), k.data_ptr(), v.data_ptr(), out.data_ptr()
    d.ldq, d.ldk, d.ldv, d.ldo = q.stride(0), k.stride(0), v.stride(0), out.stride(0)
    for t in (q, k, v, out):
        if t.dtype != torch.float16 or t.stride(-1) != 1:
            raise LmxError("attention: q/k/v/out must be float16 with contiguous last dim")
    d.B, d.H, d.Tq, d.Tk, d.hd = B, H, Tq, Tk, hd
    d.scale = float(scale)
    if window is None:
        d.mode = 0
    else:
        d.mode = 1
        d.Gh, d.Gw, d.ws, d.q_stride = window["Gh"], window["Gw"], window["ws"], window.get("q_stride", 1)
        d.pad_k = pad_k.data_ptr() if pad_k is not None else None
        d.pad_v = pad_v.data_ptr() if pad_v is not None else None
    return d


def attention(q, k, v, out, B, H, Tq, Tk, hd, scale, window=None, pad_k=None, pad_v=None, rel_pos=None):
    dev = _dev(q, k, v, out, pad_k, pad_v)
    d = _attn_desc(q, k, v, out, B, H, Tq, Tk, hd, scale, window, pad_k, pad_v)
    keep = None
    if rel_pos is not None:
        rh, rw = rel_pos
        _dev(rh, rw, q)
        S = (rh.shape[0] + 1) // 2
        if S * S != Tk or Tq != Tk or rh.dtype != torch.float32 or tuple(rh.shape) != (2 * S - 1, hd) or rh.shape != rw.shape:
            raise LmxError("attention: rel_pos tables must be float32 [2S-1, hd] with S*S == Tq == Tk")
        keep = torch.empty((B * H * Tq, 2 * S), dtype=torch.float16, device=q.device)
        check(_lib.load().lmx_k_relpos_tables(C.byref(d), _ptr(rh), _ptr(rw), S, _ptr(keep), _stream(dev)), "lmx_k_relpos_tables")
        d.rel, d.rel_S = keep.data_ptr(), S
    check(_lib.load().lmx_k_attention(C.byref(d), _stream(dev)), "lmx_k_attention")
    return out


def rope(x, B, T, H, hd, n_prefix, cos_t, sin_t):
    dev = _dev(x, cos_t, sin_t)
    check(_lib.load().lmx_k_rope(_ptr(x), x.stride(0), B, T, H, hd, n_prefix, _ptr(cos_t), _ptr(sin_t), _stream(dev)),
          "lmx_k_rope")
    return x


def pil_resize(src, dw, dh, tab_h, tab_v, swap_rb=False):
    dev = _dev(src)
    n, sh, sw, c = src.shape
    if c != 3 or src.dtype != torch.uint8 or not src.is_contiguous():
        raise LmxError("pil_resize: src must be contiguous uint8 [n,h,w,3]")
    lib = _lib.load()
    cur = src
    if tab_h is not None:
        bounds, kk, ksize = tab_h
        tmp = torch.empty((n, sh, dw, 3), dtype=torch.uint8, device=src.device)
        check(lib.lmx_k_pil_resize_h(_ptr(cur), _ptr(tmp), n, sh, sw, dw, _ptr(bounds), _ptr(kk), ksize,
                                     1 if swap_rb else 0, _stream(dev)), "lmx_k_pil_resize_h")
        cur = tmp
    elif swap_rb:
        raise LmxError("pil_resize: swap_rb needs the horizontal pass")
    if tab_v is not None:
        bounds, kk, ksize = tab_v
        w = cur.shape[2]
        dst = torch.empty((n, dh, w, 3), dtype=torch.uint8, device=src.device)
        check(lib.lmx_k_pil_resize_v(_ptr(cur), _ptr(dst), n, cur.shape[1], dh, w, _ptr(bounds), _ptr(kk), ksize,
                                     _stream(dev)), "lmx_k_pil_resize_v")
        cur = dst
    return cur


def patchify_norm(img, top, left, gh, gw, P, lut, k_pad=None):
    dev = _dev(img, lut)
    n, ih, iw, c = img.shape
    if c != 3 or img.dtype != torch.uint8 or not img.is_contiguous():
        raise LmxError("patchify_norm: img must be contiguous uint8 [n,h,w,3]")
    K = P * P * 3
    ldo = k_pad or K
    alloc = torch.zeros if ldo != K else torch.empty
    out = alloc((n * gh * gw, ldo), dtype=torch.float16, device=img.device)
    check(_lib.load().lmx_k_patchify_norm(_ptr(img), _ptr(out), n, ih, iw, top, left, gh, gw, P, ldo, _ptr(lut),
                                          _stream(dev)), "lmx_k_patchify_norm")
    return out


def assemble_tokens(patch, prefix, pos, B, np_, n_prefix, D):
    dev = _dev(patch, prefix, pos)
    out = torch.empty((B * (np_ + n_prefix), D), dtype=torch.float32, device=patch.device)
    check(_lib.load().lmx_k_assemble_tokens(_ptr(patch), _ptr(prefix), _ptr(pos), _ptr(out), B, np_, n_prefix, D,
                                            _stream(dev)), "lmx_k_assemble_tokens")
    return out


def token_mean(x, B, T, D):
    dev = _dev(x)
    out = torch.empty((B, D), dtype=torch.float32, device=x.device)
    check(_lib.load().lmx_k_token_mean(_ptr(x), _DT[x.dtype], _ptr(out), B, T, D, _stream(dev)), "lmx_k_token_mean")
    return out


def nms(pred, conf, iou=0.7, max_det=300, max_wh=7680.0):
    dev = _dev(pred)
    if pred.dtype != torch.float32 or pred.dim() != 3 or not pred.is_contiguous():
        raise LmxError("nms: pred must be contiguous float32 [n,A,4+nc]")
    n, A, row = pred.shape
    lib = _lib.load()
    ws = torch.empty((int(lib.lmx_nms_workspace_bytes(n, A)),), dtype=torch.uint8, device=pred.device)
    boxes = torch.zeros((n, max_det, 4), dtype=torch.float32, device=pred.device)
    scores = torch.zeros((n, max_det), dtype=torch.float32, device=pred.device)
    cls = torch.zeros((n, max_det), dtype=torch.int32, device=pred.device)
    src = torch.full((n, max_det), -1, dtype=torch.int32, device=pred.device)
    counts = torch.zeros((n,), dtype=torch.int32, device=pred.device)
    check(lib.lmx_k_nms(_ptr(pred), n, A, row - 4, float(conf), float(iou), max_det, float(max_wh), _ptr(boxes),
                        _ptr(scores), _ptr(cls), _ptr(src), _ptr(counts), _ptr(ws), _stream(dev)), "lmx_k_nms")
    return boxes, scores, cls, src, counts


def letterbox(frames, geo, tables, swap_rb=True):
    dev = _dev(frames)
    n, sh, sw, c = frames.shape
    if c != 3 or frames.dtype != torch.uint8 or not frames.is_contiguous():
        raise LmxError("letterbox: frames must be contiguous uint8 [n,h,w,3]")
    out = torch.empty((n, geo.oh, geo.ow, 3), dtype=torch.uint8, device=frames.device)
    xo, ia, yo, ib = tables if tables is not None else (None, None, None, None)
    check(_lib.load().lmx_k_letterbox(_ptr(frames), _ptr(out), n, sh, sw, geo.rh, geo.rw, geo.top, geo.left, geo.oh, geo.ow,
                                      _ptr(xo), _ptr(ia), _ptr(yo), _ptr(ib), 1 if swap_rb else 0, _stream(dev)),
          "lmx_k_letterbox")
    return out


def stem_conv(img_u8, w, bias, out=None):
    dev = _dev(img_u8, w, bias, out)
    n, H, W, _ = img_u8.shape
    Cout = bias.numel()
    Ho, Wo = (H - 1) // 2 + 1, (W - 1) // 2 + 1
    if out is None:
        out = torch.empty((n, Ho, Wo, Cout), dtype=torch.float16, device=img_u8.device)
    if not out.is_contiguous() or tuple(out.shape) != (n, Ho, Wo, Cout):
        raise LmxError("stem_conv: out must be a dense NHWC tensor")
    check(_lib.load().lmx_k_stem_conv(_ptr(img_u8), _ptr(w), _ptr(bias), _ptr(out), n, H, W, Cout, _stream(dev)),
          "lmx_k_stem_conv")
    return out


def maxpool5(x, out):
    dev = _dev(x, out)
    n, H, W, Cc, ps = _nhwc(x, "maxpool5 x")
    no, Ho, Wo, Co, pso = _nhwc(out, "maxpool5 out")
    if (no, Ho, Wo, Co) != (n, H, W, Cc):
        raise LmxError("maxpool5: shape mismatch")
    check(_lib.load().lmx_k_maxpool5(_ptr(x), ps, _ptr(out), pso, n, H, W, Cc, _stream(dev)), "lmx_k_maxpool5")
    return out


def upsample2(x, out):
    dev = _dev(x, out)
    n, H, W, Cc, ps = _nhwc(x, "upsample2 x")
    no, Ho, Wo, Co, pso = _nhwc(out, "upsample2 out")
    if (no, Ho, Wo, Co) != (n, 2 * H, 2 * W, Cc):
        raise LmxError("upsample2: shape mismatch")
    check(_lib.load().lmx_k_upsample2(_ptr(x), ps, _ptr(out), pso, n, H, W, Cc, _stream(dev)), "lmx_k_upsample2")
    return out


def split3(x, act, out3, g=None, res3=None):
    dev = _dev(x, out3, res3)
    nsum, sstride = 1, 0
    if x.dim() == 5:
        nsum, sstride = x.shape[0], x.stride(0)
        x = x[0]
    n, H, W, N, ps = _nhwc(x, "split3 x")
    no, Ho, Wo, C3, pso = _nhwc(out3, "split3 out")
    g = g or N
    if x.dtype != torch.float32 or out3.dtype != torch.float16 or (no, Ho, Wo, C3) != (n, H, W, 3 * N):
        raise LmxError(f"split3: x f32 {tuple(x.shape)} -> out3 f16 {tuple(out3.shape)} (3x the channels) expected")
    ldr = 0
    if res3 is not None:
        nr, Hr, Wr, Cr, ldr = _nhwc(res3, "split3 res")
        if (nr, Hr, Wr, Cr) != (n, H, W, 3 * N) or res3.dtype != torch.float16:
            raise LmxError("split3: residual must be an x3 tensor of the output's shape")
    check(_lib.load().lmx_k_split3(_ptr(x), ps, act, _ptr(res3), ldr, _ptr(out3), pso, n * H * W, N, g, nsum, sstride, _stream(dev)),
          "lmx_k_split3")
    return out3


def maxpool5_x3(x3, out3):
    dev = _dev(x3, out3)
    n, H, W, C3, ps = _nhwc(x3, "maxpool5_x3 x")
    no, Ho, Wo, Co, pso = _nhwc(out3, "maxpool5_x3 out")
    if (no, Ho, Wo, Co) != (n, H, W, C3) or C3 % 3:
        raise LmxError("maxpool5_x3: shape mismatch")
    check(_lib.load().lmx_k_maxpool5_x3(_ptr(x3), ps, _ptr(out3), pso, n, H, W, C3 // 3, _stream(dev)), "lmx_k_maxpool5_x3")
    return out3


def stem_conv_x3(img_u8, w, bias):
    dev = _dev(img_u8, w, bias)
    n, H, W, _ = img_u8.shape
    Cout = bias.numel()
    out = torch.empty((n, (H - 1) // 2 + 1, (W - 1) // 2 + 1, 3 * Cout), dtype=torch.float16, device=img_u8.device)
    check(_lib.load().lmx_k_stem_conv_x3(_ptr(img_u8), _ptr(w), _ptr(bias), _ptr(out), n, H, W, Cout, _stream(dev)),
          "lmx_k_stem_conv_x3")
    return out


def detect_decode(head, pred, nc, stride, a_off):
    dev = _dev(head, pred)
    n, H, W, ldh = head.shape
    A = pred.shape[1]
    if not head.is_contiguous() or not pred.is_contiguous() or pred.shape[2] != 4 + nc:
        raise LmxError("detect_decode: head/pred must be dense")
    check(_lib.load().lmx_k_detect_decode(_ptr(head), ldh, _ptr(pred), n, H, W, nc, float(stride), a_off, A, _stream(dev)),
          "lmx_k_detect_decode")
    return pred


def scale_boxes(boxes, padx, pady, gain, w, h):
    dev = _dev(boxes)
    if boxes.dtype != torch.float32 or not boxes.is_contiguous() or boxes.shape[-1] != 4:
        raise LmxError("scale_boxes: boxes must be dense float32 [...,4]")
    check(_lib.load().lmx_k_scale_boxes(_ptr(boxes), boxes.numel() // 4, float(padx), float(pady), float(gain), float(w),
                                        float(h), _stream(dev)), "lmx_k_scale_boxes")
    return boxes


def pose_gather(raws, strides, src, counts, kpt_shape, padx, pady, gain, w, h):
    dev = _dev(*raws, src, counts)
    K_, ndim = kpt_shape
    ldk = raws[0].shape[-1]
    for r in raws:
        if r.dtype != torch.float32 or not r.is_contiguous() or r.dim() != 4 or r.shape[-1] != ldk:
            raise LmxError("pose_gather: levels must be dense float32 [n,h,w,ldk]")
    if src.dtype != torch.int32 or counts.dtype != torch.int32 or not src.is_contiguous():
        raise LmxError("pose_gather: src / counts must be int32")
    n, max_det = src.shape
    hw = (C.c_int32 * 6)(*[v for r in raws for v in (r.shape[1], r.shape[2])])
    st = (C.c_float * 3)(*[float(v) for v in strides])
    out = torch.empty((n, max_det, K_, ndim), dtype=torch.float32, device=src.device)
    check(_lib.load().lmx_k_pose_gather(_ptr(raws[0]), _ptr(raws[1]), _ptr(raws[2]), ldk, C.cast(hw, C.c_void_p),
                                        C.cast(st, C.c_void_p), _ptr(src), _ptr(counts), n, max_det, K_, ndim, float(padx),
                                        float(pady), float(gain), float(w), float(h), _ptr(out), _stream(dev)), "lmx_k_pose_gather")
    return out


def add_bcast(a, b, out=None, out_dtype=torch.float32):
    dev = _dev(a, b, out)
    rows, D_, lda = _rows(a, "add_bcast a")
    b_rows, Db, ldb = _rows(b, "add_bcast b")
    if Db != D_ or a.dtype not in _DT or b.dtype != torch.float32:
        raise LmxError("add_bcast: a must be float16/float32, b float32, equal width")
    if out is None:
        out = torch.empty((rows, D_), dtype=out_dtype, device=a.device)
    check(_lib.load().lmx_k_add_bcast(_ptr(a), _DT[a.dtype], lda, _ptr(b), ldb, b_rows, _ptr(out), _DT[out.dtype], out.stride(0),
                                      rows, D_, _stream(dev)), "lmx_k_add_bcast")
    return out


def attention_f32(q, k, v, B, H, Tq, Tk, hd, scale):
    dev = _dev(q, k, v)
    for t in (q, k, v):
        if t.dtype != torch.float32 or t.dim() != 2 or t.stride(1) != 1:
            raise LmxError("attention_f32: q/k/v must be float32 2-D row views")
    out = torch.empty((B * Tq, H * hd), dtype=torch.float32, device=q.device)
    check(_lib.load().lmx_k_attention_f32(_ptr(q), q.stride(0), _ptr(k), k.stride(0), _ptr(v), v.stride(0), _ptr(out), out.stride(0),
                                          B, H, Tq, Tk, hd, float(scale), _stream(dev)), "lmx_k_attention_f32")
    return out


def hyper_mask_f32(up, hyper, n, G, C_, act=ACT_NONE):
    dev = _dev(up, hyper)
    if up.dtype != torch.float32 or not up.is_contiguous():
        raise LmxError("hyper_mask_f32: up must be contiguous float32")
    logits = torch.empty((n, 4 * G, 4 * G), dtype=torch.float32, device=up.device)
    check(_lib.load().lmx_k_hyper_mask_f32(_ptr(up), _ptr(hyper), _ptr(logits), n, G, C_, act, _stream(dev)), "lmx_k_hyper_mask_f32")
    return logits


def split3_rows(x, act=ACT_NONE):
    dev = _dev(x)
    rows, N, ldx = _rows(x, "split3_rows x")
    if x.dtype != torch.float32 or N % 8:
        raise LmxError("split3_rows: float32 rows with N % 8 == 0 expected")
    out = torch.empty((rows, 3 * N), dtype=torch.float16, device=x.device)
    check(_lib.load().lmx_k_split3(_ptr(x), ldx, act, None, 0, _ptr(out), 3 * N, rows, N, N, 1, 0, _stream(dev)), "lmx_k_split3")
    return out


def prompt_box(boxes, sx, sy, S, gauss, corner):
    dev = _dev(boxes, gauss, corner)
    n = boxes.shape[0]
    Fq = gauss.shape[1]
    out = torch.empty((n, 2, 2 * Fq), dtype=torch.float32, device=boxes.device)
    check(_lib.load().lmx_k_prompt_box(_ptr(boxes), boxes.stride(0), _ptr(out), n, float(sx), float(sy), float(S), _ptr(gauss),
                                       _ptr(corner), Fq, _stream(dev)), "lmx_k_prompt_box")
    return out


def hyper_mask(up, hyper, n, G, C_):
    dev = _dev(up, hyper)
    logits = torch.empty((n, 4 * G, 4 * G), dtype=torch.float32, device=up.device)
    check(_lib.load().lmx_k_hyper_mask(_ptr(up), _ptr(hyper), _ptr(logits), n, G, C_, _stream(dev)), "lmx_k_hyper_mask")
    return logits


def mask_post(logits, T, nh, nw, h, w):
    dev = _dev(logits)
    n, L, _ = logits.shape
    mask = torch.empty((n, h, w), dtype=torch.uint8, device=logits.device)
    stats = torch.empty((n, 8), dtype=torch.int64, device=logits.device)
    ws = torch.empty((n, nh, nw), dtype=torch.float32, device=logits.device)
    check(_lib.load().lmx_k_mask_post(_ptr(logits), n, L, T, nh, nw, h, w, _ptr(mask), _ptr(stats), _ptr(ws), _stream(dev)),
          "lmx_k_mask_post")
    return mask, stats


def prompt_points(points, labels, boxes, sx, sy, S, gauss, point_embed, not_a_point, corner):
    dev = _dev(points, labels, boxes, gauss)
    Np = 0 if points is None else points.shape[1]
    if Np:
        if (points.dtype != torch.float32 or labels.dtype != torch.int32 or not points.is_contiguous() or not labels.is_contiguous()
                or points.dim() != 3 or points.shape[2] != 2 or tuple(labels.shape) != tuple(points.shape[:2])):
            raise LmxError("prompt_points: points must be contiguous f32 [n,Np,2], labels contiguous int32 [n,Np]")
    if boxes is not None and (boxes.dtype != torch.float32 or boxes.dim() != 2 or boxes.shape[1] < 4 or boxes.stride(1) != 1):
        raise LmxError("prompt_points: boxes must be f32 [n,>=4] rows")
    n = points.shape[0] if Np else boxes.shape[0]
    if boxes is not None and boxes.shape[0] != n:
        raise LmxError("prompt_points: points and boxes disagree on n")
    Fq = gauss.shape[1]
    ldb = 0 if boxes is None else (boxes.stride(0) if n > 1 else boxes.shape[1])
    out = torch.empty((n, Np + (2 if boxes is not None else 1), 2 * Fq), dtype=torch.float32, device=dev)
    check(_lib.load().lmx_k_prompt_points(_ptr(points if Np else None), _ptr(labels if Np else None), Np, _ptr(boxes), ldb,
                                          _ptr(out), n, float(sx), float(sy), float(S),
                                          _ptr(gauss), _ptr(point_embed), _ptr(not_a_point), _ptr(corner), Fq, _stream(dev)),
          "lmx_k_prompt_points")
    return out


MASK_EMBED_PARAMS = 4684


def mask_embed(mask_input, emb, params, G=64):
    dev = _dev(mask_input, emb, params)
    rows, D_, lde = _rows(emb, "mask_embed emb")
    n = mask_input.shape[0]
    if (mask_input.dtype != torch.float32 or not mask_input.is_contiguous() or tuple(mask_input.shape[1:]) != (4 * G, 4 * G)
            or D_ != 256 or rows != n * G * G or emb.dtype not in _DT):
        raise LmxError(f"mask_embed: mask_input f32 [n,{4 * G},{4 * G}] and emb [n*{G * G},256] expected")
    if params.dtype != torch.float32 or params.numel() != MASK_EMBED_PARAMS or not params.is_contiguous():
        raise LmxError("mask_embed: params must be contiguous f32 [%d]" % MASK_EMBED_PARAMS)
    keys = torch.empty((rows, 256), dtype=torch.float32, device=dev)
    check(_lib.load().lmx_k_mask_embed(_ptr(mask_input), _ptr(emb), _DT[emb.dtype], lde, _ptr(params), _ptr(keys), 256, n, G,
                                       _stream(dev)), "lmx_k_mask_embed")
    return keys


def hyper_mask_multi(up, hyper, n, G, C_):
    dev = _dev(up, hyper)
    if hyper.dtype != torch.float32 or not hyper.is_contiguous() or hyper.dim() != 3 or hyper.shape[0] != n or hyper.shape[2] != C_:
        raise LmxError("hyper_mask_multi: hyper must be contiguous f32 [n,M,C]")
    M = hyper.shape[1]
    logits = torch.empty((n, M, 4 * G, 4 * G), dtype=torch.float32, device=up.device)
    check(_lib.load().lmx_k_hyper_mask_multi(_ptr(up), _ptr(hyper), _ptr(logits), n, M, G, C_, _stream(dev)), "lmx_k_hyper_mask_multi")
    return logits


def hyper_mask_multi_f32(up, hyper, n, G, C_, act=ACT_NONE):
    dev = _dev(up, hyper)
    if up.dtype != torch.float32 or not up.is_contiguous():
        raise LmxError("hyper_mask_multi_f32: up must be contiguous float32")
    if hyper.dtype != torch.float32 or not hyper.is_contiguous() or hyper.dim() != 3 or hyper.shape[0] != n or hyper.shape[2] != C_:
        raise LmxError("hyper_mask_multi_f32: hyper must be contiguous f32 [n,M,C]")
    M = hyper.shape[1]
    logits = torch.empty((n, M, 4 * G, 4 * G), dtype=torch.float32, device=up.device)
    check(_lib.load().lmx_k_hyper_mask_multi_f32(_ptr(up), _ptr(hyper), _ptr(logits), n, M, G, C_, act, _stream(dev)),
          "lmx_k_hyper_mask_multi_f32")
    return logits


def mask_logits(logits, T, nh, nw, h, w):
    dev = _dev(logits)
    if logits.dtype != torch.float32 or not logits.is_contiguous() or logits.dim() != 3:
        raise LmxError("mask_logits: logits must be contiguous f32 [n,L,L]")
    n, L, _ = logits.shape
    out = torch.empty((n, h, w), dtype=torch.float32, device=logits.device)
    check(_lib.load().lmx_k_mask_logits(_ptr(logits), n, L, T, nh, nw, h, w, _ptr(out), _stream(dev)), "lmx_k_mask_logits")
    return out


def contour_features(mask):
    dev = _dev(mask)
    if mask.dtype != torch.uint8 or mask.dim() != 3 or not mask.is_contiguous():
        raise LmxError("contour_features: mask must be contiguous uint8 [n,h,w]")
    n, h, w = mask.shape
    lib = _lib.load()
    ws = torch.empty((int(lib.lmx_contour_workspace_bytes(n, h, w)),), dtype=torch.uint8, device=mask.device)
    out = torch.empty((n, 8), dtype=torch.int64, device=mask.device)
    check(lib.lmx_k_contour_features(_ptr(mask), n, h, w, _ptr(out), _ptr(ws), _stream(dev)), "lmx_k_contour_features")
    return out


LAUNCH_TRACE = None
_raw_lib = None
RIDGE_FLOP_PER_BYTE = 2500e12 / 8e12


def _work(name, args):
    if name == "lmx_k_gemm":
        d = args[0]._obj
        M, N, Kd = d.M, d.N, d.K
        osz = 4 if d.out_dtype == F32 else 2
        a_bytes = 2 * M * (Kd // max(d.a_rep, 1))
        if d.a_mode == 1:
            a_bytes = 2 * (M // max(d.Ho * d.Wo, 1)) * d.H * d.W_ * d.Cin
        by = a_bytes + 2 * N * Kd + osz * (M // 4 if d.a_mode == 2 else M) * N + (osz * (d.res_rows or M) * N if d.res else 0)
        fl = 2.0 * M * N * Kd
        key = f"gemm M={M} N={N} K={Kd} out={'f32' if osz == 4 else 'f16'} conv3x3={d.a_mode} act={d.act} res={int(bool(d.res))}"
        return ("gemm/mfma-bound" if fl / by >= RIDGE_FLOP_PER_BYTE else "gemm/hbm-bound"), fl, by, key
    if name == "lmx_k_attention":
        d = args[0]._obj
        fl = 4.0 * d.B * d.H * d.Tq * d.Tk * d.hd
        by = 2 * d.H * d.hd * d.B * (2 * d.Tq + 2 * d.Tk)
        key = f"attention B={d.B} H={d.H} Tq={d.Tq} Tk={d.Tk} hd={d.hd} mode={d.mode} ws={d.ws} qs={d.q_stride} rel={int(bool(d.rel))}"
        return ("attention/mfma-bound" if fl / by >= RIDGE_FLOP_PER_BYTE else "attention/hbm-bound"), fl, by, key
    if name == "lmx_k_layernorm":
        in_dt, out_dt, rows, D = args[1], args[6], args[8], args[9]
        return "layernorm", 0.0, rows * D * ((4 if in_dt == F32 else 2) + (4 if out_dt == F32 else 2)), f"layernorm rows={rows} D={D} in={in_dt} out={out_dt}"
    if name == "lmx_k_ln_mlp_img":
        rows, D = args[4], args[5]
        return "fused ln+mlp", 16.0 * D * D * rows, (8 + (2 if args[7] else 0) + (2 if args[8] else 0)) * D * rows, f"ln_mlp_img rows={rows} D={D}"
    if name == "lmx_k_ln_mlp":
        rows, D = args[8], args[9]
        return "fused ln+mlp", 16.0 * D * D * rows, (16 + (2 if args[12] else 0) + (2 if args[15] else 0)) * D * rows, f"ln_mlp rows={rows} D={D}"
    if name == "lmx_k_hiera_attn8":
        n_, Gh, Gw, D = args[10], args[11], args[12], args[13]
        rows = n_ * Gh * Gw
        return "fused attention half", rows * (8.0 * D * D + 256.0 * D), rows * D * (8 + (2 if args[0] else 0)), f"hiera_attn8 rows={rows} D={D} ln_inside={int(not args[0])}"
    if name == "lmx_k_hiera_attn4":
        n_, Gh, Gw, D = args[5], args[6], args[7], args[8]
        rows = n_ * Gh * Gw
        return "fused attention half", rows * (8.0 * D * D + 64.0 * D), rows * D * 10, f"hiera_attn4 rows={rows} D={D}"
    if name == "lmx_k_hiera_attn_pool":
        n_, Gh, Gw, Di, Do = args[4], args[5], args[6], args[7], args[8]
        rows = n_ * Gh * Gw
        keys = 64 if Di == 112 else 16
        return "fused attention half", rows * (8.0 * Di * Do + keys * Do + 0.5 * Do * Do), rows * (2 * Di + Do), f"hiera_attn_pool rows={rows} {Di}->{Do}"
    if name == "lmx_k_cast_f32_f16":
        rows, cols = args[4], args[5]
        return "streaming glue", 0.0, 6 * rows * cols, f"cast_f32_f16 rows={rows} cols={cols}"
    if name == "lmx_k_maxpool2":
        dt, n_, H, W, C_ = args[4], args[5], args[6], args[7], args[8]
        esz = 4 if dt == F32 else 2
        return "streaming glue", 0.0, esz * n_ * H * W * C_ * 5 // 4, f"maxpool2 n={n_} H={H} W={W} C={C_} dtype={dt}"
    if name == "lmx_k_upsample2":
        n_, H, W, C_ = args[4], args[5], args[6], args[7]
        return "streaming glue", 0.0, 2 * n_ * H * W * C_ * 5, f"upsample2 n={n_} H={H} W={W} C={C_}"
    if name == "lmx_k_add_bcast":
        a_dt, o_dt, rows, D = args[1], args[7], args[9], args[10]
        return "streaming glue", 0.0, rows * D * ((4 if a_dt == F32 else 2) + (4 if o_dt == F32 else 2)), f"add_bcast rows={rows} D={D}"
    if name == "lmx_k_rope":
        B, T, H, hd = args[2], args[3], args[4], args[5]
        return "streaming glue", 0.0, 2 * 2 * 2 * B * T * H * hd, f"rope B={B} T={T} H={H} hd={hd}"
    return "pre/post-processing and glue", 0.0, None, name


def _install_trace():
    global _raw_lib
    if _raw_lib is not None:
        return
    lib = _raw_lib = _lib.load()

    def make(name, fn):
        def traced(*args):
            if LAUNCH_TRACE is None:
                return fn(*args)
            cls, fl, by, key = _work(name, args)
            st = torch.cuda.current_stream(_tls.dev)
            e0, e1 = torch.cuda.Event(enable_timing=True), torch.cuda.Event(enable_timing=True)
            e0.record(st)
            rc = fn(*args)
            e1.record(st)
            LAUNCH_TRACE.append((cls, key, fl, by, e0, e1))
            return rc

        return traced

    class _Proxy:
        def __getattr__(self, name):
            fn = getattr(lib, name)
            if name.startswith("lmx_k_"):
                fn = make(name, fn)
            setattr(self, name, fn)
            return fn

    _lib._lib = _Proxy()


def start_launch_trace():
    global LAUNCH_TRACE
    _install_trace()
    LAUNCH_TRACE = []


def stop_launch_trace(by_shape=False):
    global LAUNCH_TRACE
    tr, LAUNCH_TRACE = LAUNCH_TRACE or [], None
    torch.cuda.synchronize()
    out, shapes = {}, {}
    for cls, key, fl, by, e0, e1 in tr:
        dt = e0.elapsed_time(e1) * 1e-3
        for table, k in ((out, cls), (shapes, (cls, key))):
            r = table.setdefault(k, dict(launches=0, seconds=0.0, flops=0.0, bytes=0.0, modelled=by is not None))
            r["launches"] += 1
            r["seconds"] += dt
            r["flops"] += fl
            r["bytes"] += by or 0.0
    return (out, shapes) if by_shape else out
```

vision-sam3-yolo-lameless_amd/lmx/sam.py:

```python
import math
import os
from dataclasses import dataclass

import numpy as np
import torch

from . import kernels as K
from . import resample

SAM_PIXEL_MEAN = (123.675, 116.28, 103.53)
SAM_PIXEL_STD = (58.395, 57.12, 57.375)


@dataclass
class HieraConfig:
    hidden: int = 112
    blocks: tuple = (2, 3, 16, 3)
    dims: tuple = (112, 224, 448, 896)
    heads: tuple = (2, 4, 8, 16)
    windows: tuple = (8, 4, 14, 7)
    global_blocks: tuple = (12, 16, 20)
    pos_bkg: tuple = (14, 14)
    q_pool_stages: int = 3
    fpn_dim: int = 256
    fpn_top_down: tuple = (2, 3)
    eps: float = 1e-6
    image: int = 1024

    def block_plan(self):
        plan, t = [], 0
        for s, nb in enumerate(self.blocks):
            for b in range(nb):
                first = s > 0 and b == 0
                dim = self.dims[s - 1] if first else self.dims[s]
                win = self.windows[s - 1] if first else self.windows[s]
                if t in self.global_blocks:
                    win = 0
                qs = 2 if (0 < s <= self.q_pool_stages and b == 0) else 0
                plan.append((dim, self.dims[s], self.heads[s], win, qs))
                t += 1
        return plan


def hiera_b_plus():
    return HieraConfig()


def param_spec(cfg):
    s = {}
    s["backbone.pos_embed"] = ((1, cfg.hidden) + tuple(cfg.pos_bkg), "tok")
    s["backbone.pos_embed_window"] = ((1, cfg.hidden, cfg.windows[0], cfg.windows[0]), "tok")
    s["backbone.patch_embed.projection.weight"] = ((cfg.hidden, 3, 7, 7), "w")
    s["backbone.patch_embed.projection.bias"] = ((cfg.hidden,), "b")
    for i, (dim, dim_out, heads, win, qs) in enumerate(cfg.block_plan()):
        p = f"backbone.blocks.{i}."
        s[p + "layer_norm1.weight"] = ((dim,), "g")
        s[p + "layer_norm1.bias"] = ((dim,), "b")
        s[p + "attn.qkv.weight"] = ((3 * dim_out, dim), "w")
        s[p + "attn.qkv.bias"] = ((3 * dim_out,), "b")
        s[p + "attn.proj.weight"] = ((dim_out, dim_out), "w")
        s[p + "attn.proj.bias"] = ((dim_out,), "b")
        s[p + "layer_norm2.weight"] = ((dim_out,), "g")
        s[p + "layer_norm2.bias"] = ((dim_out,), "b")
        s[p + "mlp.proj_in.weight"] = ((4 * dim_out, dim_out), "w")
        s[p + "mlp.proj_in.bias"] = ((4 * dim_out,), "b")
        s[p + "mlp.proj_out.weight"] = ((dim_out, 4 * dim_out), "w")
        s[p + "mlp.proj_out.bias"] = ((dim_out,), "b")
        if dim != dim_out:
            s[p + "proj.weight"] = ((dim_out, dim), "w")
            s[p + "proj.bias"] = ((dim_out,), "b")
    for j, c in enumerate(reversed(cfg.dims)):
        s[f"neck.convs.{j}.weight"] = ((cfg.fpn_dim, c, 1, 1), "w")
        s[f"neck.convs.{j}.bias"] = ((cfg.fpn_dim,), "b")
    return s


def resize_longest_side(h, w, target=1024):
    scale = target * 1.0 / max(h, w)
    return int(h * scale + 0.5), int(w * scale + 0.5)


def sam_norm_lut():
    u = np.arange(256, dtype=np.float32)
    m = np.array(SAM_PIXEL_MEAN, np.float32)
    s = np.array(SAM_PIXEL_STD, np.float32)
    return ((u[None, :] - m[:, None]) / s[:, None]).astype(np.float32)


def pack_hiera_attn(wqkv, bqkv, wo, bo, heads, ln_inside=False):
    D = wo.shape[0]
    hd = D // heads
    if hd > 63 or D > 128:
        raise ValueError("pack_hiera_attn: head dim <= 63 and D <= 128")
    wq = np.zeros((3 * heads * 64, 128), np.float32)
    bq = np.zeros((3 * heads * 64,), np.float32)
    pos = np.array([32 * s_ + 8 * g + 4 * hb + i for s_ in range(4) for hb in range(2) for g in range(4) for i in range(4)])
    pos = pos[:D] if ln_inside else np.arange(D)
    for sec in range(3):
        for hh in range(heads):
            r0 = sec * heads * 64 + hh * 64
            wq[r0:r0 + hd, pos] = wqkv[sec * D + hh * hd: sec * D + (hh + 1) * hd]
            bq[r0:r0 + hd] = bqkv[sec * D + hh * hd: sec * D + (hh + 1) * hd]
            if sec == 2:
                bq[r0 + 63] = 1.0
    wop = np.zeros((D, heads * 64), np.float32)
    for hh in range(heads):
        for s_ in range(2):
            for g in range(4):
                for hb in range(2):
                    for i in range(4):
                        d = 16 * (2 * s_ + hb) + 4 * g + i
                        if d < hd:
                            wop[:, 64 * hh + 32 * s_ + 8 * g + 4 * hb + i] = wo[:, hh * hd + d]
    return wq.astype(np.float16), bq, wop.astype(np.float16), np.ascontiguousarray(bo, dtype=np.float32)


def pack_hiera_attn4(wqkv, bqkv, wo, bo, heads):
    D = wo.shape[0]
    hd = D // heads
    img = np.zeros((4 * heads, 16384), np.float16)
    bias = np.zeros((heads * 192 + D,), np.float32)
    for hh in range(heads):
        for sec in range(3):
            m = np.zeros((64, 256), np.float16)
            m[:hd, :D] = wqkv[sec * D + hh * hd: sec * D + (hh + 1) * hd].astype(np.float16)
            ch = m.reshape(64, 32, 8)
            out = np.zeros_like(ch)
            for r in range(64):
                out[r, np.arange(32) ^ (r & 15)] = ch[r]
            img[4 * hh + sec] = out.reshape(-1)
            bias[hh * 192 + sec * 64: hh * 192 + sec * 64 + hd] = bqkv[sec * D + hh * hd: sec * D + (hh + 1) * hd]
        bias[hh * 192 + 128 + 63] = 1.0
        m = np.zeros((256, 64), np.float16)
        for s_ in range(2):
            for g in range(4):
                for hb in range(2):
                    for i in range(4):
                        d = 16 * (2 * s_ + hb) + 4 * g + i
                        if d < hd:
                            m[:D, 32 * s_ + 8 * g + 4 * hb + i] = wo[:, hh * hd + d].astype(np.float16)
        ch = m.reshape(256, 8, 8)
        out = np.zeros_like(ch)
        for r in range(256):
            out[r, np.arange(8) ^ ((r >> 1) & 7)] = ch[r]
        img[4 * hh + 3] = out.reshape(-1)
    bias[heads * 192:] = bo
    return img, bias


def _lds_image(m, key):
    rows, cols = m.shape
    ch = m.reshape(rows, cols // 8, 8)
    out = np.zeros_like(ch)
    for r in range(rows):
        out[r, np.arange(cols // 8) ^ key(r)] = ch[r]
    img = np.zeros((16384,), np.float16)
    img[:rows * cols] = out.reshape(-1)
    return img


def pack_hiera_attn_pool(wsc, bsc, wqkv, bqkv, wo, bo, heads):
    Dout, Din = wsc.shape
    hd = Dout // heads
    wide = Din > 128
    cols = 256 if wide else 128
    k15, k7 = (lambda r: r & 15), (lambda r: (r >> 1) & 7)

    def rows_img(w, nrows):
        m = np.zeros((nrows, cols), np.float16)
        m[:w.shape[0], :Din] = w.astype(np.float16)
        return _lds_image(m, k15)

    if wide:
        imgs = [rows_img(wsc[64 * j: 64 * j + 64], 64) for j in range(7)]
    else:
        imgs = [rows_img(wsc[:128], 128), rows_img(wsc[128:], 128)]
    bias = np.zeros((Dout + heads * 192 + (0 if wide else Dout),), np.float32)
    bias[:Dout] = bsc + bo
    for hh in range(heads):
        sec = []
        for s_ in range(3):
            sec.append(wqkv[s_ * Dout + hh * hd: s_ * Dout + (hh + 1) * hd])
            bias[Dout + hh * 192 + s_ * 64: Dout + hh * 192 + s_ * 64 + hd] = bqkv[s_ * Dout + hh * hd: s_ * Dout + (hh + 1) * hd]
        bias[Dout + hh * 192 + 128 + 63] = 1.0
        if wide:
            imgs += [rows_img(sec[0], 64), rows_img(sec[1], 64), rows_img(sec[2], 64)]
        else:
            qk = np.zeros((128, Din), np.float32)
            qk[:hd], qk[64:64 + hd] = sec[0], sec[1]
            imgs += [rows_img(qk, 128), rows_img(sec[2], 64)]
        m = np.zeros((512 if wide else 256, 64), np.float16)
        for s_ in range(2):
            for g in range(4):
                for hb in range(2):
                    for i in range(4):
                        d = 16 * (2 * s_ + hb) + 4 * g + i
                        if d < hd:
                            m[:Dout, 32 * s_ + 8 * g + 4 * hb + i] = wo[:, hh * hd + d].astype(np.float16)
        if wide:
            for half in range(2):
                mm = np.zeros((256, 64), np.float16)
                mm[:224] = m[224 * half: 224 * half + 224]
                imgs.append(_lds_image(mm, k7))
        else:
            imgs.append(_lds_image(m, k7))
    return np.stack(imgs), bias


def pack_ln_mlp(w1, b1, w2, b2, g2, e2, gn=None, en=None):
    D = w2.shape[0]
    cols = 128 if D <= 128 else 256
    nks = cols // 32
    kslot = np.array([16 * (2 * s_ + hb) + 4 * g + i for s_ in range(nks) for g in range(4) for hb in range(2) for i in range(4)])
    k15, k7 = (lambda r: r & 15), (lambda r: (r >> 1) & 7)
    imgs = []
    for ch in range(4 * D // 64):
        m1 = np.zeros((64, cols), np.float16)
        ok = kslot < D
        m1[:, ok] = w1[64 * ch: 64 * ch + 64][:, kslot[ok]].astype(np.float16)
        m2 = np.zeros((D, 64), np.float16)
        m2[:, :] = w2[:, 64 * ch + kslot[:64]].astype(np.float16)
        i1, i2 = _lds_image(m1, k15), _lds_image(m2, k7)
        if D <= 128:
            both = i1.copy()
            both[8192:8192 + D * 64] = i2[:D * 64]
            imgs.append(both)
        else:
            imgs += [i1, i2]
    z = np.zeros((D,), np.float32)
    bias = np.concatenate([b1, b2, g2, e2, gn if gn is not None else z, en if en is not None else z]).astype(np.float32)
    return np.stack(imgs), bias


class HieraEncoder:

    def __init__(self, cfg, state_dict, device="cuda", fused_mlp=True):
        self.cfg = cfg
        self.device = torch.device(device)
        self.fused_mlp = fused_mlp and not os.environ.get("LMX_NO_FUSED_MLP")
        dev = self.device
        sd = state_dict

        def t32(a):
            return torch.from_numpy(np.ascontiguousarray(a, dtype=np.float32)).to(dev)

        def t16(a):
            return t32(a).to(torch.float16).contiguous()

        w = np.transpose(sd["backbone.patch_embed.projection.weight"], (0, 2, 3, 1)).reshape(cfg.hidden, 147)
        self.k_pad = 152
        self.pe_w = t16(np.concatenate([w, np.zeros((cfg.hidden, self.k_pad - 147), np.float32)], 1))
        self.pe_b = t32(sd["backbone.patch_embed.projection.bias"])
        g = cfg.image // 4
        pe = torch.nn.functional.interpolate(torch.from_numpy(sd["backbone.pos_embed"]), size=(g, g), mode="bicubic")
        win = torch.from_numpy(sd["backbone.pos_embed_window"])
        pe = pe + win.tile([x // y for x, y in zip(pe.shape, win.shape)])
        self.pos = pe.permute(0, 2, 3, 1).reshape(g * g, cfg.hidden).contiguous().to(dev)
        self.grid0 = g
        self.blocks = []
        for i, (dim, dim_out, heads, win_, qs) in enumerate(cfg.block_plan()):
            p = f"backbone.blocks.{i}."
            qkv_b = sd[p + "attn.qkv.bias"]
            blk = dict(dim=dim, dim_out=dim_out, heads=heads, win=win_, qs=qs,
                       g1=t32(sd[p + "layer_norm1.weight"]), b1=t32(sd[p + "layer_norm1.bias"]),
                       wqkv=t16(sd[p + "attn.qkv.weight"]), bqkv=t32(qkv_b),
                       padkv=t16(qkv_b),
                       wo=t16(sd[p + "attn.proj.weight"]), bo=t32(sd[p + "attn.proj.bias"]),
                       g2=t32(sd[p + "layer_norm2.weight"]), b2=t32(sd[p + "layer_norm2.bias"]),
                       w1=t16(sd[p + "mlp.proj_in.weight"]), bb1=t32(sd[p + "mlp.proj_in.bias"]),
                       w2=t16(sd[p + "mlp.proj_out.weight"]), bb2=t32(sd[p + "mlp.proj_out.bias"]))
            if dim != dim_out:
                blk["wp"], blk["bp"] = t16(sd[p + "proj.weight"]), t32(sd[p + "proj.bias"])
            if dim == dim_out == 112 and heads == 2 and win_ == 8 and not qs:
                blk["attn8_ln"] = i == 0 or not (self.fused_mlp and dim in K.FUSED_MLP_WIDTHS)
                blk["attn8"] = tuple(torch.from_numpy(a).to(dev) for a in pack_hiera_attn(
                    np.asarray(sd[p + "attn.qkv.weight"], np.float32), np.asarray(qkv_b, np.float32),
                    np.asarray(sd[p + "attn.proj.weight"], np.float32), np.asarray(sd[p + "attn.proj.bias"], np.float32), heads,
                    ln_inside=blk["attn8_ln"]))
            if dim == dim_out == 224 and heads == 4 and win_ == 4 and not qs:
                blk["attn4"] = tuple(torch.from_numpy(a).to(dev) for a in pack_hiera_attn4(
                    np.asarray(sd[p + "attn.qkv.weight"], np.float32), np.asarray(qkv_b, np.float32),
                    np.asarray(sd[p + "attn.proj.weight"], np.float32), np.asarray(sd[p + "attn.proj.bias"], np.float32), heads))
            if qs and ((dim, dim_out, heads, win_) in ((112, 224, 4, 8), (224, 448, 8, 4))):
                blk["attnp"] = tuple(torch.from_numpy(a).to(dev) for a in pack_hiera_attn_pool(
                    np.asarray(sd[p + "proj.weight"], np.float32), np.asarray(sd[p + "proj.bias"], np.float32),
                    np.asarray(sd[p + "attn.qkv.weight"], np.float32), np.asarray(qkv_b, np.float32),
                    np.asarray(sd[p + "attn.proj.weight"], np.float32), np.asarray(sd[p + "attn.proj.bias"], np.float32), heads))
            self.blocks.append(blk)
        for i, blk in enumerate(self.blocks):
            if blk["dim_out"] in (112, 224) and self.fused_mlp:
                p = f"backbone.blocks.{i}."
                nx = f"backbone.blocks.{i + 1}." if i + 1 < len(self.blocks) else None
                f32 = lambda k: np.asarray(sd[k], np.float32)
                blk["mlp_img"] = tuple(torch.from_numpy(a).to(dev) for a in pack_ln_mlp(
                    f32(p + "mlp.proj_in.weight"), f32(p + "mlp.proj_in.bias"), f32(p + "mlp.proj_out.weight"), f32(p + "mlp.proj_out.bias"),
                    f32(p + "layer_norm2.weight"), f32(p + "layer_norm2.bias"),
                    f32(nx + "layer_norm1.weight") if nx else None, f32(nx + "layer_norm1.bias") if nx else None))
        n = len(cfg.dims) - 1
        self.neck = [(t16(sd[f"neck.convs.{n - i}.weight"][:, :, 0, 0]), t32(sd[f"neck.convs.{n - i}.bias"])) for i in range(n + 1)]
        self.lut = t32(sam_norm_lut())
        self._tabs = {}

    def _tables(self, h, w):
        key = (h, w)
        if key not in self._tabs:
            nh, nw = resize_longest_side(h, w, self.cfg.image)
            dev = self.device

            def up(tab):
                b, k, ks = tab
                return (torch.from_numpy(b).to(dev), torch.from_numpy(k).to(dev), ks)

            th = up(resample.coeff_tables(w, nw, resample.BILINEAR)) if nw != w else None
            tv = up(resample.coeff_tables(h, nh, resample.BILINEAR)) if nh != h else None
            self._tabs[key] = (nh, nw, th, tv)
        return self._tabs[key]

    def preprocess(self, frames):
        n, h, w, _ = frames.shape
        nh, nw, th, tv = self._tables(h, w)
        img = K.pil_resize(frames, nw, nh, th, tv, swap_rb=False)
        S = self.cfg.image
        return img, K.im2col_u8(img, self.lut, S, S, 7, 7, 4, 3, self.k_pad)

    def trunk(self, patches, n):
        cfg = self.cfg
        g = self.grid0
        x = K.gemm(patches, self.pe_w, bias=self.pe_b, res=self.pos, res_rows=g * g, out_dtype=torch.float32)
        H = W = g
        stage_ends = set(int(v) for v in np.cumsum(cfg.blocks) - 1)
        stages, stages16 = [], []
        dev = x.device
        h_next = None
        for i, B in enumerate(self.blocks):
            dim, D, heads, qs = B["dim"], B["dim_out"], B["heads"], B["qs"]
            rows = n * H * W
            if self._attn8(i, H, W):
                if B["attn8_ln"]:
                    K.hiera_attn8(x, B["attn8"], n, H, W, heads, ln=(B["g1"], B["b1"], cfg.eps))
                else:
                    K.hiera_attn8(x, B["attn8"], n, H, W, heads, h=h_next if h_next is not None else K.layernorm(x, B["g1"], B["b1"], cfg.eps))
            elif "attnp" in B and K.hiera_attn_pool_ok(dim, D, heads, B["win"], H, W, qs):
                x = K.hiera_attn_pool(h_next if h_next is not None else K.layernorm(x, B["g1"], B["b1"], cfg.eps), B["attnp"], n, H, W, heads, D)
                H, W = H // 2, W // 2
            elif "attn4" in B and K.hiera_attn4_ok(D, heads, B["win"], H, W, qs):
                K.hiera_attn4(h_next if h_next is not None else K.layernorm(x, B["g1"], B["b1"], cfg.eps), x, B["attn4"], n, H, W, heads)
            else:
                h = h_next if h_next is not None else K.layernorm(x, B["g1"], B["b1"], cfg.eps)
                if dim != D:
                    if qs and K.pooled_gemm_ok(rows, D):
                        sc = K.gemm(h, B["wp"], bias=B["bp"], out_dtype=torch.float32, pool_hw=(H, W))
                    else:
                        sc = K.gemm(h, B["wp"], bias=B["bp"], out_dtype=torch.float32)
                        if qs:
                            pooled = torch.empty((n, H // 2, W // 2, D), dtype=torch.float32, device=dev)
                            K.maxpool2(sc.view(n, H, W, D), pooled)
                            sc = pooled.view(-1, D)
                    res = sc
                else:
                    res = x
                x, H, W = self._attention_half(B, h, x, res, n, H, W)
            h_next = None
            x16 = None
            if D in K.FUSED_MLP_WIDTHS and self.fused_mlp:
                if i in stage_ends:
                    x16 = torch.empty((n * H * W, D), dtype=torch.float16, device=dev)
                nxt = None
                if i + 1 < len(self.blocks) and not (self._attn8(i + 1, H, W) and self.blocks[i + 1]["attn8_ln"]):
                    h_next = torch.empty((n * H * W, D), dtype=torch.float16, device=dev)
                    nxt = (self.blocks[i + 1]["g1"], self.blocks[i + 1]["b1"], h_next)
                if "mlp_img" in B and K.ln_mlp_img_ok(D, n * H * W):
                    K.ln_mlp_img(x, B["mlp_img"], cfg.eps, x16=x16, h_next=h_next)
                else:
                    K.ln_mlp(x, B["g2"], B["b2"], B["w1"], B["bb1"], B["w2"], B["bb2"], cfg.eps, x16=x16, next_ln=nxt)
            else:
                h2 = K.layernorm(x, B["g2"], B["b2"], cfg.eps)
                u = K.gemm(h2, B["w1"], bias=B["bb1"], act=K.ACT_GELU)
                K.gemm(u, B["w2"], bias=B["bb2"], res=x, out=x)
            if i in stage_ends:
                stages.append(x.view(n, H, W, D))
                stages16.append(x16)
                if i != len(self.blocks) - 1 and self.blocks[i + 1]["dim"] == self.blocks[i + 1]["dim_out"]:
                    x = x.clone()
        return stages, stages16

    def _attn8(self, i, H, W):
        B = self.blocks[i]
        return "attn8" in B and B["dim"] == B["dim_out"] and K.hiera_attn8_ok(B["dim_out"], B["heads"], B["win"], H, W, B["qs"])

    def _attention_half(self, B, h, x, res, n, H, W):
        D, heads, win, qs = B["dim_out"], B["heads"], B["win"], B["qs"]
        hd = D // heads
        rows = n * H * W
        dev = h.device
        Hq, Wq = H, W
        if qs and K.pooled_gemm_ok(rows, D):
            Hq, Wq = H // 2, W // 2
            q = K.gemm(h, B["wqkv"][:D], bias=B["bqkv"][:D], pool_hw=(H, W))
            kv = K.gemm(h, B["wqkv"][D:], bias=B["bqkv"][D:])
            k, v = kv[:, :D], kv[:, D:]
        else:
            qkv = K.gemm(h, B["wqkv"], bias=B["bqkv"])
            q, k, v = qkv[:, :D], qkv[:, D:2 * D], qkv[:, 2 * D:]
            if qs:
                Hq, Wq = H // 2, W // 2
                qp = torch.empty((n, Hq, Wq, D), dtype=torch.float16, device=dev)
                K.maxpool2(qkv.view(n, H, W, 3 * D)[..., :D], qp)
                q = qp.view(-1, D)
        a = torch.empty((n * Hq * Wq, D), dtype=torch.float16, device=dev)
        if win > 0:
            nW = -(-H // win) * -(-W // win)
            wq = win // 2 if qs else win
            K.attention(q, k, v, a, n * nW, heads, wq * wq, win * win, hd, hd ** -0.5,
                        window=dict(Gh=H, Gw=W, ws=win, q_stride=2 if qs else 1),
                        pad_k=B["padkv"][D:2 * D], pad_v=B["padkv"][2 * D:])
        else:
            K.attention(q, k, v, a, n, heads, Hq * Wq, H * W, hd, hd ** -0.5)
        xo = torch.empty((n * Hq * Wq, D), dtype=torch.float32, device=dev) if res is not x else x
        K.gemm(a, B["wo"], bias=B["bo"], res=res, out=xo)
        return xo, Hq, Wq

    def fpn(self, stages, stages16=None):
        cfg = self.cfg
        nlev = len(stages) - 1
        feats, prev = [], None
        for i in range(nlev, -1, -1):
            s = stages[i]
            n, H, W, C = s.shape
            a = stages16[i] if stages16 and stages16[i] is not None else K.cast_f16(s.view(-1, C))
            w, b = self.neck[i]
            out = torch.empty((n, H, W, cfg.fpn_dim), dtype=torch.float16, device=s.device)
            if i not in cfg.fpn_top_down or i == nlev:
                K.gemm(a, w, bias=b, out=out.view(-1, cfg.fpn_dim))
            else:
                up = torch.empty((n, H, W, cfg.fpn_dim), dtype=torch.float16, device=s.device)
                K.upsample2(prev, up)
                K.gemm(a, w, bias=b, res=up.view(-1, cfg.fpn_dim), out=out.view(-1, cfg.fpn_dim))
            prev = out
            feats.append(out)
        return feats[-3:][::-1]

    def encode_patches(self, patches, n):
        stages, stages16 = self.trunk(patches, n)
        return dict(fpn=self.fpn(stages, stages16), stages=stages)

    def encode(self, frames, precision=None):
        img, patches = self.preprocess(frames)
        out = self.encode_patches(patches, frames.shape[0])
        out["resized"] = img
        return out


@dataclass
class SamVitConfig:
    hidden: int = 768
    layers: int = 12
    heads: int = 12
    mlp: int = 3072
    global_idx: tuple = (2, 5, 8, 11)
    window: int = 14
    patch: int = 16
    image: int = 1024
    out_ch: int = 256
    eps: float = 1e-6

    @property
    def grid(self):
        return self.image // self.patch


def sam_vit_b():
    return SamVitConfig()


def sam_vit_l():
    return SamVitConfig(hidden=1024, layers=24, heads=16, mlp=4096, global_idx=(5, 11, 17, 23))


def sam_vit_h():
    return SamVitConfig(hidden=1280, layers=32, heads=16, mlp=5120, global_idx=(7, 15, 23, 31))


def vit_param_spec(cfg):
    D, hd, g = cfg.hidden, cfg.hidden // cfg.heads, cfg.grid
    s = {"vision_encoder.pos_embed": ((1, g, g, D), "tok"),
         "vision_encoder.patch_embed.projection.weight": ((D, 3, cfg.patch, cfg.patch), "w"),
         "vision_encoder.patch_embed.projection.bias": ((D,), "b")}
    for i in range(cfg.layers):
        p = f"vision_encoder.layers.{i}."
        S = g if i in cfg.global_idx else cfg.window
        s[p + "layer_norm1.weight"] = ((D,), "g")
        s[p + "layer_norm1.bias"] = ((D,), "b")
        s[p + "attn.rel_pos_h"] = ((2 * S - 1, hd), "b")
        s[p + "attn.rel_pos_w"] = ((2 * S - 1, hd), "b")
        s[p + "attn.qkv.weight"] = ((3 * D, D), "w")
        s[p + "attn.qkv.bias"] = ((3 * D,), "b")
        s[p + "attn.proj.weight"] = ((D, D), "w")
        s[p + "attn.proj.bias"] = ((D,), "b")
        s[p + "layer_norm2.weight"] = ((D,), "g")
        s[p + "layer_norm2.bias"] = ((D,), "b")
        s[p + "mlp.lin1.weight"] = ((cfg.mlp, D), "w")
        s[p + "mlp.lin1.bias"] = ((cfg.mlp,), "b")
        s[p + "mlp.lin2.weight"] = ((D, cfg.mlp), "w")
        s[p + "mlp.lin2.bias"] = ((D,), "b")
    s["vision_encoder.neck.conv1.weight"] = ((cfg.out_ch, D, 1, 1), "w")
    s["vision_encoder.neck.layer_norm1.weight"] = ((cfg.out_ch,), "g")
    s["vision_encoder.neck.layer_norm1.bias"] = ((cfg.out_ch,), "b")
    s["vision_encoder.neck.conv2.weight"] = ((cfg.out_ch, cfg.out_ch, 3, 3), "w")
    s["vision_encoder.neck.layer_norm2.weight"] = ((cfg.out_ch,), "g")
    s["vision_encoder.neck.layer_norm2.bias"] = ((cfg.out_ch,), "b")
    return s


class SamVitEncoder:

    def __init__(self, cfg, state_dict, device="cuda", precision="exact"):
        if precision not in ("exact", "f16"):
            raise ValueError(f"precision {precision!r}: expected 'exact' or 'f16'")
        self.precision = precision
        self.cfg = cfg
        self.device = torch.device(device)
        dev = self.device
        sd = state_dict
        D, P = cfg.hidden, cfg.patch
        self._w32, self._w2 = {}, {}

        def t32(a):
            return torch.from_numpy(np.ascontiguousarray(a, dtype=np.float32)).to(dev)

        def t16(a, key=None):
            if key is not None:
                self._w32[key] = np.ascontiguousarray(a, dtype=np.float32)
            return t32(a).to(torch.float16).contiguous()

        w = np.transpose(sd["vision_encoder.patch_embed.projection.weight"], (0, 2, 3, 1)).reshape(D, P * P * 3)
        self._w32["pe"] = np.ascontiguousarray(w, dtype=np.float32)
        self.k_pad = P * P * 3
        self.pe_w, self.pe_b = t16(w), t32(sd["vision_encoder.patch_embed.projection.bias"])
        self.pos = t32(sd["vision_encoder.pos_embed"].reshape(cfg.grid * cfg.grid, D))
        self.layers = []
        for i in range(cfg.layers):
            p = f"vision_encoder.layers.{i}."
            qb = sd[p + "attn.qkv.bias"]
            self.layers.append(dict(
                glob=i in cfg.global_idx,
                g1=t32(sd[p + "layer_norm1.weight"]), b1=t32(sd[p + "layer_norm1.bias"]),
                wqkv=t16(sd[p + "attn.qkv.weight"], f"{i}.qkv"), bqkv=t32(qb), padkv=t16(qb),
                rh=t32(sd[p + "attn.rel_pos_h"]), rw=t32(sd[p + "attn.rel_pos_w"]),
                wo=t16(sd[p + "attn.proj.weight"], f"{i}.proj"), bo=t32(sd[p + "attn.proj.bias"]),
                g2=t32(sd[p + "layer_norm2.weight"]), b2=t32(sd[p + "layer_norm2.bias"]),
                w1=t16(sd[p + "mlp.lin1.weight"], f"{i}.fc1"), bb1=t32(sd[p + "mlp.lin1.bias"]),
                w2=t16(sd[p + "mlp.lin2.weight"], f"{i}.fc2"), bb2=t32(sd[p + "mlp.lin2.bias"])))
        self.n1_w = t16(sd["vision_encoder.neck.conv1.weight"][:, :, 0, 0], "n1")
        self.n1_ln = (t32(sd["vision_encoder.neck.layer_norm1.weight"]), t32(sd["vision_encoder.neck.layer_norm1.bias"]))
        c2 = sd["vision_encoder.neck.conv2.weight"]
        self.n2_w = t16(np.transpose(c2, (0, 2, 3, 1)).reshape(c2.shape[0], -1), "n2")
        self.n2_ln = (t32(sd["vision_encoder.neck.layer_norm2.weight"]), t32(sd["vision_encoder.neck.layer_norm2.bias"]))
        self.lut = t32(sam_norm_lut())
        self._tabs = {}

    _tables = HieraEncoder._tables

    def preprocess(self, frames):
        n, h, w, _ = frames.shape
        nh, nw, th, tv = self._tables(h, w)
        img = K.pil_resize(frames, nw, nh, th, tv, swap_rb=False)
        S, P = self.cfg.image, self.cfg.patch
        return img, K.im2col_u8(img, self.lut, S, S, P, P, P, 0, self.k_pad)

    def _split2(self, key):
        if key not in self._w2:
            w = self._w32[key]
            hi = w.astype(np.float16)
            lo = (w - hi.astype(np.float32)).astype(np.float16)
            self._w2[key] = torch.from_numpy(np.ascontiguousarray(np.concatenate([hi, lo], 1))).to(self.device)
        return self._w2[key]

    def embed(self, patches, n, precision=None):
        cfg = self.cfg
        precision = precision or self.precision
        if precision not in ("exact", "f16"):
            raise ValueError(f"precision {precision!r}: expected 'exact' or 'f16'")
        exact = precision == "exact"
        g, D, H = cfg.grid, cfg.hidden, cfg.heads
        hd = D // H
        rows = n * g * g

        def lin(a, w16, key, **kw):
            if exact:
                w2 = self._split2(key)
                if a.shape[1] % 64 == 0 and a.shape[0] >= 512 and w2.shape[0] >= 96 and w2.shape[0] % 8 == 0:
                    return K.gemm(a, w2, a_rep=2, **kw)
                return K.gemm(torch.cat([a, a], 1), w2, **kw)
            return K.gemm(a, w16, **kw)

        x = lin(patches, self.pe_w, "pe", bias=self.pe_b, res=self.pos, res_rows=g * g, out_dtype=torch.float32)
        for i, L in enumerate(self.layers):
            h = K.layernorm(x, L["g1"], L["b1"], cfg.eps)
            qkv = lin(h, L["wqkv"], f"{i}.qkv", bias=L["bqkv"])
            q, k, v = qkv[:, :D], qkv[:, D:2 * D], qkv[:, 2 * D:]
            a = torch.empty((rows, D), dtype=torch.float16, device=x.device)
            if L["glob"]:
                K.attention(q, k, v, a, n, H, g * g, g * g, hd, hd ** -0.5, rel_pos=(L["rh"], L["rw"]))
            else:
                ws = cfg.window
                nW = (-(-g // ws)) ** 2
                K.attention(q, k, v, a, n * nW, H, ws * ws, ws * ws, hd, hd ** -0.5, window=dict(Gh=g, Gw=g, ws=ws, q_stride=1),
                            pad_k=L["padkv"][D:2 * D], pad_v=L["padkv"][2 * D:], rel_pos=(L["rh"], L["rw"]))
            lin(a, L["wo"], f"{i}.proj", bias=L["bo"], res=x, out=x)
            h2 = K.layernorm(x, L["g2"], L["b2"], cfg.eps)
            u = lin(h2, L["w1"], f"{i}.fc1", bias=L["bb1"], act=K.ACT_GELU)
            lin(u, L["w2"], f"{i}.fc2", bias=L["bb2"], res=x, out=x)
        y = lin(K.cast_f16(x), self.n1_w, "n1", out_dtype=torch.float32)
        y = K.layernorm(y, *self.n1_ln, 1e-6)
        y4 = y.view(n, g, g, cfg.out_ch)
        if exact:
            if "n2.hi" not in self._w2:
                w2 = self._split2("n2")
                Kc = w2.shape[1] // 2
                self._w2["n2.hi"], self._w2["n2.lo"] = w2[:, :Kc].contiguous(), w2[:, Kc:].contiguous()
            acc = K.conv3x3(y4, self._w2["n2.hi"], bias=None, act=K.ACT_NONE, out_dtype=torch.float32)
            acc = K.conv3x3(y4, self._w2["n2.lo"], bias=None, act=K.ACT_NONE, res=acc, out=acc)
            y = K.layernorm(acc.view(rows, cfg.out_ch), *self.n2_ln, 1e-6, out_dtype=torch.float32)
        else:
            y = K.conv3x3(y4, self.n2_w, bias=None, act=K.ACT_NONE)
            y = K.layernorm(y.view(rows, cfg.out_ch), *self.n2_ln, 1e-6)
        return y.view(n, g, g, cfg.out_ch)

    def encode(self, frames, precision=None):
        img, patches = self.preprocess(frames)
        return dict(fpn=[None, None, self.embed(patches, frames.shape[0], precision)], resized=img)
```

Measured before the change: 663.6 frames/s.

## Fuse LayerNorm into GEMM epilogue for width-448 Hiera blocks

Adds a GEMM variant with a row-complete 128x448 tile whose epilogue adds the residual, writes the f32 output, then computes LayerNorm per row from LDS and emits the f16 normalized activations (and optionally an f16 copy). The Hiera blocks of width 448 use it after the attention output projection and after the MLP down projection, so the separate layernorm kernels and their re-read of the f32 residual stream go away. The new tile uses a two-stage ring with an uneven DMA split and a single wide tile per workgroup, which may lower GEMM efficiency or occupancy compared with the tuned generic kernel. The LayerNorm statistics code is also factored into shared helpers.

Measured after the change: 670.3 frames/s (median of 6 runs). 1.01x the previous value.

```diff
diff --git a/include/lmx.h b/include/lmx.h
--- a/include/lmx.h
+++ b/include/lmx.h
@@ -39,6 +39,8 @@
   int64_t split_stride;
 } lmx_gemm_desc;
 int lmx_k_gemm(const lmx_gemm_desc* d, lmx_stream_t stream);
+int lmx_k_gemm_ln(const lmx_gemm_desc* d, const float* gamma, const float* beta, float eps, void* y16, int64_t ldy, void* x16,
+                  int64_t ldx16, lmx_stream_t stream);
 void lmx_dbg_set_gemm2_variant(int v);
 
 int lmx_k_layernorm(const void* x, int in_dtype, int64_t ldx, const float* gamma, const float* beta,
diff --git a/vision-sam3-yolo-lameless_amd/csrc/common.h b/vision-sam3-yolo-lameless_amd/csrc/common.h
--- a/vision-sam3-yolo-lameless_amd/csrc/common.h
+++ b/vision-sam3-yolo-lameless_amd/csrc/common.h
@@ -123,6 +123,24 @@
   for (int o = 32; o > 0; o >>= 1) v += __shfl_xor(v, o, 64);
   return v;
 }
+template <int ITERS>
+__device__ __forceinline__ void ln_stats(const f32x4 (&v)[ITERS], int lane, int D, float eps, float& mean, float& rstd) {
+  float s = 0.f;
+#pragma unroll
+  for (int i = 0; i < ITERS; ++i)
+    if ((i * 64 + lane) * 4 < D) s += (v[i][0] + v[i][1]) + (v[i][2] + v[i][3]);
+  mean = wave_sum(s) / (float)D;
+  float q = 0.f;
+#pragma unroll
+  for (int i = 0; i < ITERS; ++i)
+    if ((i * 64 + lane) * 4 < D) {
+      const f32x4 dlt = v[i] - mean;
+      q += (dlt[0] * dlt[0] + dlt[1] * dlt[1]) + (dlt[2] * dlt[2] + dlt[3] * dlt[3]);
+    }
+  rstd = 1.0f / sqrtf(wave_sum(q) / (float)D + eps);
+}
+__device__ __forceinline__ f32x4 ln_apply(f32x4 v, float mean, float rstd, f32x4 g, f32x4 b) { return (v - mean) * rstd * g + b; }
+
 __device__ __forceinline__ float wave_max(float v) {
 #pragma unroll
   for (int o = 32; o > 0; o >>= 1) v = fmaxf(v, __shfl_xor(v, o, 64));
diff --git a/vision-sam3-yolo-lameless_amd/csrc/gemm.hip b/vision-sam3-yolo-lameless_amd/csrc/gemm.hip
--- a/vision-sam3-yolo-lameless_amd/csrc/gemm.hip
+++ b/vision-sam3-yolo-lameless_amd/csrc/gemm.hip
@@ -214,7 +214,7 @@
 
 int lmx_gemm2_launch(const lmx_gemm_desc& d, hipStream_t st);
 
-static bool force_v1() {
+bool lmx_gemm_v1_forced() {
   static int v = -1;
   if (v < 0) {
     const char* e = getenv("LMX_GEMM_V1");
@@ -223,9 +223,7 @@
   return v == 1;
 }
 
-extern "C" int lmx_k_gemm(const lmx_gemm_desc* dp, lmx_stream_t stream) {
-  LMX_REQUIRE(dp != nullptr, "lmx_k_gemm: null descriptor");
-  const lmx_gemm_desc& d = *dp;
+int lmx_gemm_check(const lmx_gemm_desc& d) {
   LMX_REQUIRE(d.A && d.W && d.C, "lmx_k_gemm: null A/W/C");
   LMX_REQUIRE(d.M > 0 && d.N > 0 && d.K > 0, "lmx_k_gemm: empty problem M=%d N=%d K=%d", d.M, d.N, d.K);
   LMX_REQUIRE(d.K % 8 == 0, "lmx_k_gemm: K=%d must be a multiple of 8", d.K);
@@ -270,6 +268,20 @@
     LMX_REQUIRE(d.out_dtype == LMX_F32 && d.act == LMX_ACT_NONE && d.a_mode != 2 && d.a_rep <= 1, "lmx_k_gemm: split_k needs f32 output, no activation, a_mode 0 or 1");
     LMX_REQUIRE(d.split_stride >= (int64_t)(d.M - 1) * d.ldc + d.N && d.split_stride % 4 == 0, "lmx_k_gemm: split_stride=%lld", (long long)d.split_stride);
     LMX_REQUIRE((d.K + 63) / 64 >= d.split_k, "lmx_k_gemm: split_k=%d exceeds the k-tiles of K=%d", d.split_k, d.K);
+  }
+  if (d.a_rep > 1) {
+    LMX_REQUIRE(d.a_mode == 0 && d.K % d.a_rep == 0 && (d.K / d.a_rep) % 64 == 0, "lmx_k_gemm: a_rep=%d needs a_mode 0 and K / a_rep a multiple of 64 (K=%d)", d.a_rep, d.K);
+    LMX_REQUIRE(d.lda >= d.K / d.a_rep, "lmx_k_gemm: lda=%lld < K / a_rep", (long long)d.lda);
+  }
+  return LMX_OK;
+}
+
+extern "C" int lmx_k_gemm(const lmx_gemm_desc* dp, lmx_stream_t stream) {
+  LMX_REQUIRE(dp != nullptr, "lmx_k_gemm: null descriptor");
+  const lmx_gemm_desc& d = *dp;
+  const int rc = lmx_gemm_check(d);
+  if (rc != LMX_OK) return rc;
+  if (d.split_k > 1) {
     const bool conv_ok2 = d.a_mode == 1 && d.Cin % 32 == 0 && d.H < 32768 && d.W_ < 32768;
     LMX_REQUIRE((d.a_mode == 0 || conv_ok2) && d.N >= 64 && d.N % 8 == 0 && d.ldc % 8 == 0 && (!d.res || d.ldr % 8 == 0) &&
                     aligned16(d.C) && (!d.res || aligned16(d.res)),
@@ -277,8 +289,6 @@
     return lmx_gemm2_launch(d, reinterpret_cast<hipStream_t>(stream));
   }
   if (d.a_rep > 1) {
-    LMX_REQUIRE(d.a_mode == 0 && d.K % d.a_rep == 0 && (d.K / d.a_rep) % 64 == 0, "lmx_k_gemm: a_rep=%d needs a_mode 0 and K / a_rep a multiple of 64 (K=%d)", d.a_rep, d.K);
-    LMX_REQUIRE(d.lda >= d.K / d.a_rep, "lmx_k_gemm: lda=%lld < K / a_rep", (long long)d.lda);
     LMX_REQUIRE(d.M >= 512 && d.N >= 96 && d.N % 8 == 0 && d.ldc % 8 == 0 && (!d.res || d.ldr % 8 == 0) && aligned16(d.C) && (!d.res || aligned16(d.res)),
                 "lmx_k_gemm: a_rep is built into the LDS-DMA kernel only (M >= 512, N >= 96, N %% 8 == 0); M=%d N=%d", d.M, d.N);
     return lmx_gemm2_launch(d, reinterpret_cast<hipStream_t>(stream));
@@ -290,7 +300,7 @@
   if (n64 < 0) n64 = (getenv("LMX_GEMM_N64") && getenv("LMX_GEMM_N64")[0] == '0') ? 0 : 1;
   const int n_min = (conv_ok && n64 && d.M >= 65536) ? 64 : 96;
   if ((d.a_mode == 0 || conv_ok) && d.M >= 512 && d.N >= n_min && d.N % 8 == 0 && d.ldc % 8 == 0 && (!d.res || d.ldr % 8 == 0) &&
-      aligned16(d.C) && (!d.res || aligned16(d.res)) && !force_v1())
+      aligned16(d.C) && (!d.res || aligned16(d.res)) && !lmx_gemm_v1_forced())
     return lmx_gemm2_launch(d, st);
   if (d.a_mode == 0) {
     return d.out_dtype == LMX_F16 ? dispatch_tile<0, LMX_F16>(d, st) : dispatch_tile<0, LMX_F32>(d, st);
diff --git a/vision-sam3-yolo-lameless_amd/csrc/gemm2.hip b/vision-sam3-yolo-lameless_amd/csrc/gemm2.hip
--- a/vision-sam3-yolo-lameless_amd/csrc/gemm2.hip
+++ b/vision-sam3-yolo-lameless_amd/csrc/gemm2.hip
@@ -16,15 +16,29 @@
 constexpr int smem_bytes(int BM, int BN, int BK, int NSTAGE) { return NSTAGE * (BM + BN) * BK * 2 + 2 * BN * 4; }
 constexpr int waves_per_simd(int BM, int BN, int BK, int NSTAGE) {
   const int smem = smem_bytes(BM, BN, BK, NSTAGE), nwave = (BM / 64) * (BN / 64);
-  const int wps = (smem <= 80 * 1024 ? 2 : 1) * nwave / 4;
+  const int wps = ((smem <= 80 * 1024 ? 2 : 1) * nwave + 3) / 4;
   return wps < 1 ? 1 : wps;
 }
-template <int OUT_DT, int BM, int BN, int BK, int NSTAGE, int AMODE, int STAG>
-__global__ __launch_bounds__(waves_per_simd(BM, BN, BK, NSTAGE) * 256) void gemm2_kernel(const lmx_gemm_desc p, const int ntiles, const int nt_ok) {
+struct ln_epi {
+  const float* gamma;
+  const float* beta;
+  half_t* y;
+  half_t* x16;
+  int64_t ldy, ldx;
+  float eps;
+};
+template <int OUT_DT, int BM, int BN, int BK, int NSTAGE, int AMODE, int STAG, int LN = 0>
+__global__ __launch_bounds__(waves_per_simd(BM, BN, BK, NSTAGE) * 256) void gemm2_kernel(const lmx_gemm_desc p, const int ntiles, const int nt_ok,
+                                                                                       const ln_epi e) {
   constexpr int NWAVE = (BM / 64) * (BN / 64);
   constexpr int STAGE_BYTES = (BM + BN) * BK * 2;
-  constexpr int A_INSTR = BM * BK * 2 / 1024 / NWAVE;
-  constexpr int W_INSTR = BN * BK * 2 / 1024 / NWAVE;
+  constexpr int A_TOT = BM * BK * 2 / 1024, W_TOT = BN * BK * 2 / 1024;
+  constexpr bool EVEN = A_TOT % NWAVE == 0 && W_TOT % NWAVE == 0;
+  constexpr int A_U = (A_TOT + NWAVE - 1) / NWAVE, W_U = (W_TOT + NWAVE - 1) / NWAVE;
+  static_assert(EVEN || (NSTAGE == 2 && STAG == 0 && AMODE == 0 && LN != 0), "an uneven DMA split: the two-slot ring, BN == N");
+  static_assert(LN == 0 || (OUT_DT == LMX_F32 && AMODE == 0 && BM == 128), "the LayerNorm epilogue: f32 rows, 64-row halves");
+  constexpr int A_INSTR = A_TOT / NWAVE;
+  constexpr int W_INSTR = W_TOT / NWAVE;
   constexpr int ROWS_PER_INSTR = 1024 / (BK * 2);
   constexpr int CHUNKS = BK / 8;
   constexpr int LA = NSTAGE - 1;
@@ -96,6 +110,10 @@
 #pragma unroll
   for (int j = 0; j < W_INSTR; ++j)
     w_off[j] = (unsigned)(((wave * W_INSTR + j) * ROWS_PER_INSTR + lrow) * p.K * 2 + lchunk * 16);
+  unsigned ua_off[A_U], uw_off = 0;
+#pragma unroll
+  for (int j = 0; j < (EVEN ? 0 : A_U); ++j) ua_off[j] = (unsigned)(((j * NWAVE + wave) * ROWS_PER_INSTR + lrow) * (int)p.lda * 2 + lchunk * 16);
+  if (!EVEN) uw_off = (unsigned)((wave * ROWS_PER_INSTR + lrow) * p.K * 2 + lchunk * 16);
   const unsigned OOB = 0x80000000u;
   const int nk = (p.K + BK - 1) / BK;
   const int nk64 = (p.K + 63) / 64;
@@ -109,6 +127,17 @@
     char* st = smem + slot * STAGE_BYTES;
     const bool kill = (kt == nk - 1) && k_tail_lane;
     const int soff = kt * (BK * 2);
+    if constexpr (!EVEN) {
+      const int kta = kt - (kt >= nkA ? nkA : 0) - (kt >= 2 * nkA ? nkA : 0);
+#pragma unroll
+      for (int j = 0; j < A_U; ++j)
+        if (A_TOT % NWAVE == 0 || j * NWAVE + wave < A_TOT) lds_dma16(a_rs, st + (j * NWAVE + wave) * 1024, kill ? OOB : ua_off[j], kta * (BK * 2));
+#pragma unroll
+      for (int j = 0; j < W_U; ++j)
+        if (W_TOT % NWAVE == 0 || j * NWAVE + wave < W_TOT)
+          lds_dma16(w_rs, st + BM * BK * 2 + (j * NWAVE + wave) * 1024, kill ? OOB : uw_off, soff + j * NWAVE * ROWS_PER_INSTR * p.K * 2);
+      return;
+    }
     if (AMODE != 1) {
       const int kta = kt - (kt >= nkA ? nkA : 0) - (kt >= 2 * nkA ? nkA : 0);
       const int soff_a = (AMODE == 0) ? kta * (BK * 2) : soff;
@@ -144,8 +173,9 @@
     for (int j = 0; j < 4; ++j) acc[i][j] = f32x4{0.f, 0.f, 0.f, 0.f};
 
   float* bl = reinterpret_cast<float*>(smem + NSTAGE * STAGE_BYTES);
+  constexpr bool LATE_BIAS = AMODE == 1 || LN != 0;
   float bias_v = 0.f, scale_v = 1.f;
-  if (AMODE != 1 && tid < BN && n0 + tid < p.N) {
+  if (!LATE_BIAS && tid < BN && n0 + tid < p.N) {
     if (p.bias && sp_ == 0) bias_v = p.bias[n0 + tid];
     if (p.scale) scale_v = p.scale[n0 + tid];
   }
@@ -156,7 +186,7 @@
 
   const int frow = lane & 15, fq = lane >> 4;
   const int fsw = (BK == 64) ? (frow & 7) : ((-(frow >> 2)) & 3);
-  constexpr int PT = A_INSTR + W_INSTR;
+  constexpr int PT = EVEN ? A_INSTR + W_INSTR : 1;
   if constexpr (STAG == 0) {
   for (int kt = 0; kt < nloc; ++kt) {
     const int left = nloc - 1 - kt;
@@ -232,7 +262,7 @@
   if (!grp) __builtin_amdgcn_s_barrier();
   }
 
-  if (AMODE == 1 && tid < BN && n0 + tid < p.N) {
+  if (LATE_BIAS && tid < BN && n0 + tid < p.N) {
     if (p.bias && sp_ == 0) bias_v = p.bias[n0 + tid];
     if (p.scale) scale_v = p.scale[n0 + tid];
   }
@@ -332,6 +362,67 @@
           if ((frow & 3) == 0 && m < p.M && n < p.N) *reinterpret_cast<f32x4*>(reinterpret_cast<float*>(p.C) + (int64_t)(m >> 2) * p.ldc + n) = v;
           __builtin_amdgcn_sched_barrier(0);
         }
+    } else if constexpr (LN != 0) {
+      constexpr int RSL = BN + 4;
+      constexpr int LIT = (BN + 255) / 256;
+      float* img = reinterpret_cast<float*>(smem);
+      const int lrow = lane >> 4, c16 = lane & 15;
+      const int n = n0 + wn * 64 + c16 * 4;
+      const bool has_res = p.res != nullptr;
+      f32x4 rr[4];
+#pragma unroll
+      for (int h = 0; h < 2; ++h) {
+#pragma unroll
+        for (int pp = 0; pp < 2; ++pp) {
+          const int pass = 2 * h + pp;
+#pragma unroll
+          for (int it = 0; it < 4; ++it) {
+            const int m = m0 + wm * 64 + pass * 16 + it * 4 + lrow;
+            rr[it] = f32x4{0.f, 0.f, 0.f, 0.f};
+            if (has_res && m < p.M && n < p.N)
+              rr[it] = *reinterpret_cast<const f32x4*>(reinterpret_cast<const float*>(p.res) + (int64_t)m * p.ldr + n);
+          }
+          float* t = img + (wm * 32 + pp * 16) * RSL + wn * 64;
+#pragma unroll
+          for (int j = 0; j < 4; ++j) *reinterpret_cast<f32x4*>(t + frow * RSL + j * 16 + fq * 4) = finish(acc[pass][j], j);
+#pragma unroll
+          for (int it = 0; it < 4; ++it) {
+            const int row = it * 4 + lrow;
+            f32x4 o = *reinterpret_cast<const f32x4*>(t + row * RSL + c16 * 4);
+            const int m = m0 + wm * 64 + pass * 16 + row;
+            if (m < p.M && n < p.N) {
+              if (has_res) o += rr[it];
+              *reinterpret_cast<f32x4*>(reinterpret_cast<float*>(p.C) + (int64_t)m * p.ldc + n) = o;
+            }
+            *reinterpret_cast<f32x4*>(t + row * RSL + c16 * 4) = o;
+          }
+        }
+        asm volatile("s_waitcnt lgkmcnt(0)" ::: "memory");
+        __builtin_amdgcn_s_barrier();
+        for (int r = wave; r < 64; r += NWAVE) {
+          const int m = m0 + (r >> 5) * 64 + h * 32 + (r & 31);
+          if (m >= p.M) continue;
+          f32x4 v[LIT];
+#pragma unroll
+          for (int i = 0; i < LIT; ++i) {
+            const int c = (i * 64 + lane) * 4;
+            v[i] = c < BN ? *reinterpret_cast<const f32x4*>(img + r * RSL + c) : f32x4{0.f, 0.f, 0.f, 0.f};
+          }
+          float mean, rstd;
+          ln_stats<LIT>(v, lane, p.N, e.eps, mean, rstd);
+#pragma unroll
+          for (int i = 0; i < LIT; ++i) {
+            const int c = (i * 64 + lane) * 4;
+            if (c < p.N) {
+              const f32x4 o = ln_apply(v[i], mean, rstd, *reinterpret_cast<const f32x4*>(e.gamma + c), *reinterpret_cast<const f32x4*>(e.beta + c));
+              *reinterpret_cast<half4_t*>(e.y + (int64_t)m * e.ldy + c) = half4_t{(half_t)o[0], (half_t)o[1], (half_t)o[2], (half_t)o[3]};
+              if (e.x16)
+                *reinterpret_cast<half4_t*>(e.x16 + (int64_t)m * e.ldx + c) = half4_t{(half_t)v[i][0], (half_t)v[i][1], (half_t)v[i][2], (half_t)v[i][3]};
+            }
+          }
+        }
+        __builtin_amdgcn_s_barrier();
+      }
     } else {
       float* t32 = reinterpret_cast<float*>(my);
       constexpr int RS = 68;
@@ -374,7 +465,9 @@
     using T = std::true_type;
     using F = std::false_type;
     const int act = p.act;
-    if (p.scale) {
+    if constexpr (LN != 0) {
+      epilogue(std::integral_constant<int, LMX_ACT_NONE>{}, F{});
+    } else if (p.scale) {
       if (act == LMX_ACT_NONE) epilogue(std::integral_constant<int, LMX_ACT_NONE>{}, T{});
       else if (act == LMX_ACT_SILU) epilogue(std::integral_constant<int, LMX_ACT_SILU>{}, T{});
       else if (act == LMX_ACT_GELU) epilogue(std::integral_constant<int, LMX_ACT_GELU>{}, T{});
@@ -388,6 +481,7 @@
   }
   __builtin_amdgcn_s_barrier();
   TL(4, wall_clock64());
+  if constexpr (LN != 0) break;
   }
 }
 
@@ -413,10 +507,25 @@
   }
   if (persist > 0 && grid > 256 * persist) grid = 256 * persist;
   if (d.out_dtype == LMX_F16)
-    hipLaunchKernelGGL((gemm2_kernel<LMX_F16, BM, BN, BK, NSTAGE, AMODE, STAG>), dim3(grid), dim3(BM * BN / 64), smem, st, d, ntiles, nt_ok);
+    hipLaunchKernelGGL((gemm2_kernel<LMX_F16, BM, BN, BK, NSTAGE, AMODE, STAG>), dim3(grid), dim3(BM * BN / 64), smem, st, d, ntiles, nt_ok, ln_epi{});
   else
-    hipLaunchKernelGGL((gemm2_kernel<LMX_F32, BM, BN, BK, NSTAGE, AMODE, STAG>), dim3(grid), dim3(BM * BN / 64), smem, st, d, ntiles, nt_ok);
+    hipLaunchKernelGGL((gemm2_kernel<LMX_F32, BM, BN, BK, NSTAGE, AMODE, STAG>), dim3(grid), dim3(BM * BN / 64), smem, st, d, ntiles, nt_ok, ln_epi{});
   return lmx_launch_check("gemm2_kernel");
+}
+
+int launch_ln(const lmx_gemm_desc& d, const ln_epi& e, hipStream_t st) {
+  constexpr int BM = 128, BN = 448, BK = 64, NSTAGE = 2;
+  const size_t smem = smem_bytes(BM, BN, BK, NSTAGE);
+  static_assert(smem_bytes(BM, BN, BK, NSTAGE) <= 160 * 1024 && 64 * (BN + 4) * 4 <= NSTAGE * (BM + BN) * BK * 2, "LDS budget");
+  static bool attr_set = false;
+  if (!attr_set) {
+    LMX_HIP(hipFuncSetAttribute(reinterpret_cast<const void*>(&gemm2_kernel<LMX_F32, BM, BN, BK, NSTAGE, 0, 0, 1>),
+                                hipFuncAttributeMaxDynamicSharedMemorySize, (int)smem));
+    attr_set = true;
+  }
+  const int ntiles = (d.M + BM - 1) / BM;
+  hipLaunchKernelGGL((gemm2_kernel<LMX_F32, BM, BN, BK, NSTAGE, 0, 0, 1>), dim3(ntiles), dim3(BM * BN / 64), smem, st, d, ntiles, 1, e);
+  return lmx_launch_check("gemm2_kernel (LayerNorm epilogue)");
 }
 
 }
@@ -470,3 +579,31 @@
     }
   }
 }
+
+int lmx_gemm_check(const lmx_gemm_desc& d);
+bool lmx_gemm_v1_forced();
+
+extern "C" int lmx_k_gemm_ln(const lmx_gemm_desc* dp, const float* gamma, const float* beta, float eps, void* y16, int64_t ldy,
+                             void* x16, int64_t ldx16, lmx_stream_t stream) {
+  LMX_REQUIRE(dp != nullptr && gamma && beta && y16, "lmx_k_gemm_ln: null descriptor / gamma / beta / y16");
+  const lmx_gemm_desc& d = *dp;
+  const int rc = lmx_gemm_check(d);
+  if (rc != LMX_OK) return rc;
+  LMX_REQUIRE(d.a_mode == 0 && d.out_dtype == LMX_F32 && d.act == LMX_ACT_NONE && !d.scale && d.split_k <= 1 && d.a_rep <= 1 && d.res_rows == 0,
+              "lmx_k_gemm_ln: f32 output, a_mode 0, no activation / scale / split_k / a_rep / res_rows");
+  LMX_REQUIRE(d.N == 448, "lmx_k_gemm_ln: N=%d (the row-complete tile is built for N = 448)", d.N);
+  LMX_REQUIRE(ldy % 4 == 0 && ldy >= d.N && ((((uintptr_t)y16) & 7) == 0), "lmx_k_gemm_ln: y16 stride / alignment");
+  if (x16) LMX_REQUIRE(ldx16 % 4 == 0 && ldx16 >= d.N && ((((uintptr_t)x16) & 7) == 0), "lmx_k_gemm_ln: x16 stride / alignment");
+  LMX_REQUIRE(aligned16(gamma) && aligned16(beta), "lmx_k_gemm_ln: gamma/beta alignment");
+  static int fused = -1;
+  if (fused < 0) fused = (getenv("LMX_GEMM_LN") && getenv("LMX_GEMM_LN")[0] == '0') ? 0 : 1;
+  hipStream_t st = reinterpret_cast<hipStream_t>(stream);
+  if (fused && d.M >= 512 && d.ldc % 8 == 0 && (!d.res || d.ldr % 8 == 0) && aligned16(d.C) && (!d.res || aligned16(d.res)) &&
+      !lmx_gemm_v1_forced())
+    return launch_ln(d, ln_epi{gamma, beta, reinterpret_cast<half_t*>(y16), reinterpret_cast<half_t*>(x16), ldy, ldx16, eps}, st);
+  int r = lmx_k_gemm(dp, stream);
+  if (r == LMX_OK)
+    r = lmx_k_layernorm(d.C, LMX_F32, d.ldc, gamma, beta, y16, LMX_F16, ldy, d.M, d.N, eps, LMX_ACT_NONE, stream);
+  if (r == LMX_OK && x16) r = lmx_k_cast_f32_f16(reinterpret_cast<const float*>(d.C), d.ldc, x16, ldx16, d.M, d.N, stream);
+  return r;
+}
diff --git a/vision-sam3-yolo-lameless_amd/csrc/norm.hip b/vision-sam3-yolo-lameless_amd/csrc/norm.hip
--- a/vision-sam3-yolo-lameless_amd/csrc/norm.hip
+++ b/vision-sam3-yolo-lameless_amd/csrc/norm.hip
@@ -56,7 +56,6 @@
   const int row = blockIdx.x * 4 + (threadIdx.x >> 6);
   if (row >= rows) return;
   f32x4 v[ITERS];
-  float s = 0.f;
 #pragma unroll
   for (int i = 0; i < ITERS; ++i) {
     const int c = (i * 64 + lane) * 4;
@@ -67,27 +66,17 @@
         const half4_t hv = *reinterpret_cast<const half4_t*>(reinterpret_cast<const half_t*>(xv) + (int64_t)row * ldx + c);
         v[i] = f32x4{(float)hv[0], (float)hv[1], (float)hv[2], (float)hv[3]};
       }
-      s += (v[i][0] + v[i][1]) + (v[i][2] + v[i][3]);
-    }
-  }
-  const float mean = wave_sum(s) / (float)D;
-  float q = 0.f;
-#pragma unroll
-  for (int i = 0; i < ITERS; ++i) {
-    const int c = (i * 64 + lane) * 4;
-    if (c < D) {
-      const f32x4 dlt = v[i] - mean;
-      q += (dlt[0] * dlt[0] + dlt[1] * dlt[1]) + (dlt[2] * dlt[2] + dlt[3] * dlt[3]);
-    }
-  }
-  const float rstd = 1.0f / sqrtf(wave_sum(q) / (float)D + eps);
+    }
+  }
+  float mean, rstd;
+  ln_stats<ITERS>(v, lane, D, eps, mean, rstd);
 #pragma unroll
   for (int i = 0; i < ITERS; ++i) {
     const int c = (i * 64 + lane) * 4;
     if (c < D) {
       const f32x4 g = *reinterpret_cast<const f32x4*>(gamma + c);
       const f32x4 b = *reinterpret_cast<const f32x4*>(beta + c);
-      f32x4 o = (v[i] - mean) * rstd * g + b;
+      f32x4 o = ln_apply(v[i], mean, rstd, g, b);
       if (act == LMX_ACT_GELU) {
 #pragma unroll
         for (int e = 0; e < 4; ++e) o[e] = 0.5f * o[e] * (1.0f + erff(o[e] * 0.70710678118654752440f));
@@ -137,24 +126,13 @@
   while (row < rows) {
     const int nrow = row + nw;
     if (nrow < rows) load(nrow, vn);
-    float s = 0.f;
-#pragma unroll
-    for (int i = 0; i < ITERS; ++i)
-      if ((i * 64 + lane) * 4 < D) s += (v[i][0] + v[i][1]) + (v[i][2] + v[i][3]);
-    const float mean = wave_sum(s) / (float)D;
-    float q = 0.f;
-#pragma unroll
-    for (int i = 0; i < ITERS; ++i)
-      if ((i * 64 + lane) * 4 < D) {
-        const f32x4 dlt = v[i] - mean;
-        q += (dlt[0] * dlt[0] + dlt[1] * dlt[1]) + (dlt[2] * dlt[2] + dlt[3] * dlt[3]);
-      }
-    const float rstd = 1.0f / sqrtf(wave_sum(q) / (float)D + eps);
+    float mean, rstd;
+    ln_stats<ITERS>(v, lane, D, eps, mean, rstd);
 #pragma unroll
     for (int i = 0; i < ITERS; ++i) {
       const int c = (i * 64 + lane) * 4;
       if (c < D) {
-        const f32x4 o = (v[i] - mean) * rstd * g[i] + b[i];
+        const f32x4 o = ln_apply(v[i], mean, rstd, g[i], b[i]);
         if (OUT_DT == LMX_F32) {
           *reinterpret_cast<f32x4*>(reinterpret_cast<float*>(yv) + (int64_t)row * ldy + c) = o;
         } else {
diff --git a/vision-sam3-yolo-lameless_amd/lmx/_lib.py b/vision-sam3-yolo-lameless_amd/lmx/_lib.py
--- a/vision-sam3-yolo-lameless_amd/lmx/_lib.py
+++ b/vision-sam3-yolo-lameless_amd/lmx/_lib.py
@@ -39,6 +39,7 @@
     "lmx_last_error": (C.c_char_p, []),
     "lmx_device_count": (_I, []),
     "lmx_k_gemm": (_I, [C.POINTER(GemmDesc), _VP]),
+    "lmx_k_gemm_ln": (_I, [C.POINTER(GemmDesc), _VP, _VP, _F, _VP, _I64, _VP, _I64, _VP]),
     "lmx_dbg_set_gemm2_variant": (None, [_I]),
     "lmx_k_pose_gather": (_I, [_VP, _VP, _VP, _I64, _VP, _VP, _VP, _VP, _I, _I, _I, _I, _F, _F, _F, _F, _F, _VP, _VP]),
     "lmx_k_pack_bits": (_I, [_VP, _I64, _I, _VP, _VP]),
diff --git a/vision-sam3-yolo-lameless_amd/lmx/kernels.py b/vision-sam3-yolo-lameless_amd/lmx/kernels.py
--- a/vision-sam3-yolo-lameless_amd/lmx/kernels.py
+++ b/vision-sam3-yolo-lameless_amd/lmx/kernels.py
@@ -51,8 +51,12 @@
     return M >= 512 and N >= 96 and N % 8 == 0
 
 
-def gemm(a, w, bias=None, act=ACT_NONE, scale=None, res=None, out=None, out_dtype=torch.float16, res_rows=0, pool_hw=None, a_rep=1):
-    dev = _dev(a, w, bias, scale, res, out)
+GEMM_LN_WIDTHS = (448,)
+
+
+def gemm(a, w, bias=None, act=ACT_NONE, scale=None, res=None, out=None, out_dtype=torch.float16, res_rows=0, pool_hw=None, a_rep=1,
+         ln=None, x16=None):
+    dev = _dev(a, w, bias, scale, res, out, x16, *(ln[:2] + ln[3:] if ln else ()))
     M, K, lda = _rows(a, "gemm A")
     N, K2, ldw = _rows(w, "gemm W")
     if K2 != a_rep * K or ldw != K2:
@@ -84,7 +88,26 @@
     d.act, d.out_dtype, d.a_mode, d.a_rep = act, _DT[out.dtype], 0, a_rep
     if pool_hw:
         d.a_mode, d.H, d.W_ = 2, int(pool_hw[0]), int(pool_hw[1])
-    check(_lib.load().lmx_k_gemm(C.byref(d), _stream(dev)), "lmx_k_gemm")
+    if ln is None:
+        if x16 is not None:
+            raise LmxError("gemm: x16 is written by the LayerNorm epilogue only (ln=...)")
+        check(_lib.load().lmx_k_gemm(C.byref(d), _stream(dev)), "lmx_k_gemm")
+        return out
+    gamma, beta, eps, y = ln
+    for t, nm in ((gamma, "gamma"), (beta, "beta")):
+        if t.dtype != torch.float32 or t.numel() != N or not t.is_contiguous():
+            raise LmxError(f"gemm ln: {nm} must be contiguous float32 [N]")
+    My, Ny, ldy = _rows(y, "gemm ln y")
+    if (My, Ny) != (M, N) or y.dtype != torch.float16:
+        raise LmxError("gemm ln: y must be float16 [M, N]")
+    x16p, ldx = None, 0
+    if x16 is not None:
+        Mx, Nx, ldx = _rows(x16, "gemm x16")
+        if (Mx, Nx) != (M, N) or x16.dtype != torch.float16:
+            raise LmxError("gemm ln: x16 must be float16 [M, N]")
+        x16p = x16.data_ptr()
+    check(_lib.load().lmx_k_gemm_ln(C.byref(d), gamma.data_ptr(), beta.data_ptr(), float(eps), y.data_ptr(), ldy, x16p, ldx,
+                                    _stream(dev)), "lmx_k_gemm_ln")
     return out
 
 
@@ -743,6 +766,10 @@
         fl = 2.0 * M * N * Kd
         key = f"gemm M={M} N={N} K={Kd} out={'f32' if osz == 4 else 'f16'} conv3x3={d.a_mode} act={d.act} res={int(bool(d.res))}"
         return ("gemm/mfma-bound" if fl / by >= RIDGE_FLOP_PER_BYTE else "gemm/hbm-bound"), fl, by, key
+    if name == "lmx_k_gemm_ln":
+        cls, fl, by, key = _work("lmx_k_gemm", args[:1])
+        M, N = args[0]._obj.M, args[0]._obj.N
+        return cls, fl, by + 2 * M * N * (2 if args[6] else 1), key + f" ln=1 x16={int(bool(args[6]))}"
     if name == "lmx_k_attention":
         d = args[0]._obj
         fl = 4.0 * d.B * d.H * d.Tq * d.Tk * d.hd
diff --git a/vision-sam3-yolo-lameless_amd/lmx/sam.py b/vision-sam3-yolo-lameless_amd/lmx/sam.py
--- a/vision-sam3-yolo-lameless_amd/lmx/sam.py
+++ b/vision-sam3-yolo-lameless_amd/lmx/sam.py
@@ -335,6 +335,8 @@
         for i, B in enumerate(self.blocks):
             dim, D, heads, qs = B["dim"], B["dim_out"], B["heads"], B["qs"]
             rows = n * H * W
+            ln_epi = D in K.GEMM_LN_WIDTHS and not (D in K.FUSED_MLP_WIDTHS and self.fused_mlp)
+            h2 = None
             if self._attn8(i, H, W):
                 if B["attn8_ln"]:
                     K.hiera_attn8(x, B["attn8"], n, H, W, heads, ln=(B["g1"], B["b1"], cfg.eps))
@@ -359,7 +361,7 @@
                     res = sc
                 else:
                     res = x
-                x, H, W = self._attention_half(B, h, x, res, n, H, W)
+                x, H, W, h2 = self._attention_half(B, h, x, res, n, H, W, ln2=ln_epi)
             h_next = None
             x16 = None
             if D in K.FUSED_MLP_WIDTHS and self.fused_mlp:
@@ -374,9 +376,16 @@
                 else:
                     K.ln_mlp(x, B["g2"], B["b2"], B["w1"], B["bb1"], B["w2"], B["bb2"], cfg.eps, x16=x16, next_ln=nxt)
             else:
-                h2 = K.layernorm(x, B["g2"], B["b2"], cfg.eps)
+                if h2 is None:
+                    h2 = K.layernorm(x, B["g2"], B["b2"], cfg.eps)
                 u = K.gemm(h2, B["w1"], bias=B["bb1"], act=K.ACT_GELU)
-                K.gemm(u, B["w2"], bias=B["bb2"], res=x, out=x)
+                if ln_epi and i + 1 < len(self.blocks) and not (self._attn8(i + 1, H, W) and self.blocks[i + 1]["attn8_ln"]):
+                    h_next = torch.empty((n * H * W, D), dtype=torch.float16, device=dev)
+                    if i in stage_ends:
+                        x16 = torch.empty((n * H * W, D), dtype=torch.float16, device=dev)
+                    K.gemm(u, B["w2"], bias=B["bb2"], res=x, out=x, ln=(self.blocks[i + 1]["g1"], self.blocks[i + 1]["b1"], cfg.eps, h_next), x16=x16)
+                else:
+                    K.gemm(u, B["w2"], bias=B["bb2"], res=x, out=x)
             if i in stage_ends:
                 stages.append(x.view(n, H, W, D))
                 stages16.append(x16)
@@ -388,7 +397,7 @@
         B = self.blocks[i]
         return "attn8" in B and B["dim"] == B["dim_out"] and K.hiera_attn8_ok(B["dim_out"], B["heads"], B["win"], H, W, B["qs"])
 
-    def _attention_half(self, B, h, x, res, n, H, W):
+    def _attention_half(self, B, h, x, res, n, H, W, ln2=False):
         D, heads, win, qs = B["dim_out"], B["heads"], B["win"], B["qs"]
         hd = D // heads
         rows = n * H * W
@@ -417,8 +426,9 @@
         else:
             K.attention(q, k, v, a, n, heads, Hq * Wq, H * W, hd, hd ** -0.5)
         xo = torch.empty((n * Hq * Wq, D), dtype=torch.float32, device=dev) if res is not x else x
-        K.gemm(a, B["wo"], bias=B["bo"], res=res, out=xo)
-        return xo, Hq, Wq
+        h2 = torch.empty((n * Hq * Wq, D), dtype=torch.float16, device=dev) if ln2 else None
+        K.gemm(a, B["wo"], bias=B["bo"], res=res, out=xo, ln=(B["g2"], B["b2"], self.cfg.eps, h2) if ln2 else None)
+        return xo, Hq, Wq, h2
 
     def fpn(self, stages, stages16=None):
         cfg = self.cfg
```
